# kspalaiologos/bzip3

Measured on AMD Instinct MI355X. Metric: MiB/s encode+decode round-trip, 8 MiB blocks, higher is better.
Workload: dtype u8

## Files before the change

bzip3_amd/__init__.py:

```python
import ctypes as C
import os

_HERE = os.path.dirname(os.path.abspath(__file__))
LIB_PATH = os.path.join(_HERE, "lib", "libbzip3.so")

BZ3_OK = 0
BZ3_ERR_OUT_OF_BOUNDS = -1
BZ3_ERR_BWT = -2
BZ3_ERR_CRC = -3
BZ3_ERR_MALFORMED_HEADER = -4
BZ3_ERR_TRUNCATED_DATA = -5
BZ3_ERR_DATA_TOO_BIG = -6
BZ3_ERR_INIT = -7
BZ3_ERR_DATA_SIZE_TOO_SMALL = -8

T_NAMES = ["crc", "rle", "lzp", "bwt", "cm", "copy", "_6", "_7"]

_lib = None


def _declare(L, strict=True):
    vp, i32, u32, sz = C.c_void_p, C.c_int32, C.c_uint32, C.c_size_t
    sig = {
        "bz3_version": (C.c_char_p, []),
        "bz3_last_error": (C.c_int8, [vp]),
        "bz3_strerror": (C.c_char_p, [vp]),
        "bz3_new": (vp, [i32]),
        "bz3_free": (None, [vp]),
        "bz3_bound": (sz, [sz]),
        "bz3_compress": (C.c_int, [u32, vp, vp, sz, C.POINTER(sz)]),
        "bz3_decompress": (C.c_int, [vp, vp, sz, C.POINTER(sz)]),
        "bz3_min_memory_needed": (sz, [i32]),
        "bz3_encode_block": (i32, [vp, vp, i32]),
        "bz3_decode_block": (i32, [vp, vp, sz, i32, i32]),
        "bz3_encode_blocks": (None, [vp, vp, vp, i32]),
        "bz3_decode_blocks": (None, [vp, vp, vp, vp, vp, i32]),
        "bz3_orig_size_sufficient_for_decode": (C.c_int, [vp, sz, i32]),
        "bz3_hip_device_count": (C.c_int, []),
        "bz3_hip_bind_device": (C.c_int, [C.c_int]),
        "bz3_hip_state_device": (C.c_int, [vp]),
        "bz3_hip_set_cm_mode": (C.c_int, [C.c_int]),
        "bz3_hip_cm_blocks_given_up": (C.c_uint, []),
        "bz3_hip_cm_blocks_routed_full": (C.c_uint, []),
        "bz3_hip_debug_bwt_big_rounds": (None, [C.c_int]),
        "bz3_hip_debug_set_unbwt_log_stride": (None, [C.c_int]),
        "bz3_hip_debug_peak_concurrent_groups": (C.c_int, [C.c_int]),
        "bz3_hip_debug_front_end_ring": (C.c_int, []),
        "bz3_hip_debug_arena_swap_buffers": (C.c_int, [C.c_int]),
        "bz3_hip_cm_variant_for": (C.c_int, [C.c_int, C.c_int, C.c_int]),
        "bz3_hip_set_lean_states": (C.c_int, [C.c_int]),
        "bz3_hip_release_cached_memory": (None, []),
        "bz3_hip_set_keep_workspace": (C.c_int, [C.c_int]),
        "bz3_hip_set_front_end_duo": (C.c_int, [C.c_int]),
        "bz3_hip_set_workspace_headroom": (None, [C.c_longlong]),
        "bz3_hip_workspace_headroom": (sz, []),
        "bz3_hip_debug_headroom_events": (C.c_uint, [C.c_int, C.POINTER(C.c_uint)]),
        "bz3_hip_debug_ring_contexts": (sz, [sz, sz, sz, sz, sz, sz, C.c_int, sz]),
        "bz3_hip_debug_arena_slack": (sz, [sz]),
        "bz3_hip_debug_cm_launches": (C.c_uint, [C.c_int]),
        "bz3_hip_debug_workspace_bytes": (sz, [sz, C.c_int]),
        "bz3_hip_debug_cached_bytes": (sz, [C.c_int]),
        "bz3_hip_encode_block_device": (i32, [vp, vp, i32]),
        "bz3_hip_decode_block_device": (i32, [vp, vp, sz, i32, i32]),
        "bz3_hip_encode_blocks_device": (None, [vp, vp, vp, i32]),
        "bz3_hip_decode_blocks_device": (None, [vp, vp, vp, vp, vp, i32]),
        "bz3_hip_compress_device": (C.c_int, [u32, vp, vp, sz, C.POINTER(sz)]),
        "bz3_hip_decompress_device": (C.c_int, [vp, vp, sz, C.POINTER(sz)]),
        "bz3_hip_frame_decoded_size_device": (C.c_int, [vp, sz, C.POINTER(sz)]),
        "bz3_hip_compress_device_many": (C.c_int, [u32, i32, C.POINTER(vp), C.POINTER(sz), C.POINTER(vp), C.POINTER(sz), C.POINTER(C.c_int)]),
        "bz3_hip_decompress_device_many": (C.c_int, [i32, C.POINTER(vp), C.POINTER(sz), C.POINTER(vp), C.POINTER(sz), C.POINTER(C.c_int)]),
        "bz3_hip_frame_decoded_sizes_device": (C.c_int, [i32, C.POINTER(vp), C.POINTER(sz), C.POINTER(sz), C.POINTER(C.c_int)]),
        "bz3_hip_debug_copy_segments": (i32, [vp, vp, C.POINTER(C.c_uint64), i32]),
        "bz3_hip_compress_device_planes": (C.c_int, [u32, u32, vp, vp, sz, C.POINTER(sz)]),
        "bz3_hip_decompress_device_planes": (C.c_int, [u32, vp, vp, sz, C.POINTER(sz)]),
        "bz3_hip_compress_device_planes_many": (C.c_int, [u32, i32, C.POINTER(u32), C.POINTER(vp), C.POINTER(sz), C.POINTER(vp), C.POINTER(sz), C.POINTER(C.c_int)]),
        "bz3_hip_decompress_device_planes_many": (C.c_int, [i32, C.POINTER(u32), C.POINTER(vp), C.POINTER(sz), C.POINTER(vp), C.POINTER(sz), C.POINTER(C.c_int)]),
        "bz3_hip_debug_planes": (i32, [vp, vp, C.POINTER(C.c_uint64), i32]),
        "bz3_hip_compress_device_delta": (C.c_int, [u32, u32, vp, vp, vp, sz, C.POINTER(sz)]),
        "bz3_hip_decompress_device_delta": (C.c_int, [u32, vp, vp, sz, vp, sz, C.POINTER(sz)]),
        "bz3_hip_compress_device_delta_many": (C.c_int, [u32, i32, C.POINTER(u32), C.POINTER(vp), C.POINTER(vp), C.POINTER(sz), C.POINTER(vp), C.POINTER(sz), C.POINTER(C.c_int)]),
        "bz3_hip_decompress_device_delta_many": (C.c_int, [i32, C.POINTER(u32), C.POINTER(vp), C.POINTER(sz), C.POINTER(vp), C.POINTER(sz), C.POINTER(vp), C.POINTER(sz), C.POINTER(C.c_int)]),
        "bz3_hip_crc32c_device": (C.c_int, [vp, sz, u32, C.POINTER(u32)]),
        "bz3_hip_crc32c_device_many": (C.c_int, [i32, C.POINTER(vp), C.POINTER(sz), C.POINTER(u32), C.POINTER(u32)]),
        "bz3_hip_debug_crc_launches": (C.c_uint, [C.c_int]),
        "bz3_hip_debug_delta": (i32, [vp, vp, vp, C.POINTER(C.c_uint64), i32]),
        "bz3_hip_decompress_device_range": (C.c_int, [u32, vp, sz, C.c_uint64, vp, sz, vp, C.POINTER(sz)]),
        "bz3_hip_decompress_device_range_many": (C.c_int, [i32, C.POINTER(u32), C.POINTER(vp), C.POINTER(sz), C.POINTER(C.c_uint64), C.POINTER(vp), C.POINTER(sz),
                                                           C.POINTER(vp), C.POINTER(sz), C.POINTER(C.c_int)]),
        "bz3_hip_debug_range": (i32, [vp, vp, vp, C.POINTER(C.c_uint64), i32]),
        "bz3_hip_decompress_device_strided": (C.c_int, [u32, vp, sz, C.c_uint64, C.c_uint64, C.c_uint64, C.c_uint64, vp, sz, vp, C.POINTER(sz)]),
        "bz3_hip_decompress_device_strided_many": (C.c_int, [i32, C.POINTER(u32), C.POINTER(vp), C.POINTER(sz), C.POINTER(C.c_uint64), C.POINTER(vp), C.POINTER(sz),
                                                             C.POINTER(vp), C.POINTER(sz), C.POINTER(C.c_int)]),
        "bz3_hip_debug_strided": (i32, [vp, vp, vp, C.POINTER(C.c_uint64), i32]),
        "bz3_hip_decompress_device_select": (C.c_int, [u32, vp, sz, C.c_uint64, C.c_uint64, C.c_uint64, C.c_uint64, C.POINTER(C.c_uint64), vp, sz, vp, C.POINTER(sz)]),
        "bz3_hip_decompress_device_select_many": (C.c_int, [i32, C.POINTER(u32), C.POINTER(vp), C.POINTER(sz), C.POINTER(C.c_uint64), C.POINTER(C.POINTER(C.c_uint64)),
                                                            C.POINTER(vp), C.POINTER(sz), C.POINTER(vp), C.POINTER(sz), C.POINTER(C.c_int)]),
        "bz3_hip_debug_select": (i32, [vp, vp, vp, C.POINTER(C.c_uint64), i32, C.POINTER(C.c_uint64), C.c_uint64]),
        "bz3_hip_update_device_range": (C.c_int, [u32, vp, sz, C.c_uint64, vp, sz, vp, vp, C.POINTER(sz)]),
        "bz3_hip_update_device_range_many": (C.c_int, [i32, C.POINTER(u32), C.POINTER(vp), C.POINTER(sz), C.POINTER(C.c_uint64), C.POINTER(vp), C.POINTER(sz), C.POINTER(vp),
                                                       C.POINTER(vp), C.POINTER(sz), C.POINTER(C.c_int)]),
        "bz3_hip_debug_patch": (i32, [vp, vp, vp, C.POINTER(C.c_uint64), i32]),
        "bz3_hip_last_timings": (None, [vp, C.POINTER(C.c_float)]),
        "bz3_hip_last_bwt_stats": (None, [vp, C.POINTER(i32), C.POINTER(i32), C.POINTER(C.c_uint64)]),
        "bz3_hip_stage_crc32c": (u32, [vp, sz, u32]),
        "bz3_hip_stage_mrle_encode": (i32, [vp, i32, vp]),
        "bz3_hip_stage_mrle_decode": (C.c_int, [vp, vp, i32, i32]),
        "bz3_hip_stage_lzp_encode": (i32, [vp, i32, vp]),
        "bz3_hip_stage_lzp_decode": (i32, [vp, i32, vp, i32]),
        "bz3_hip_stage_bwt": (i32, [vp, vp, i32]),
        "bz3_hip_stage_unbwt": (i32, [vp, vp, i32, i32]),
        "bz3_hip_stage_last_ms": (C.c_float, []),
        "bz3_hip_debug_sort_u32": (i32, [vp, u32, C.c_int, C.c_int, vp, vp]),
        "bz3_hip_debug_scan_u32": (i32, [vp, u32, vp]),
        "bz3_hip_debug_cu_masks": (i32, [C.c_int, C.c_int, vp, vp]),
        "bz3_hip_set_collect_window_us": (None, [C.c_int]),
        "bz3_hip_debug_collected_batches": (C.c_uint, [C.c_int, C.POINTER(C.c_uint)]),
        "bz3_hip_stage_cm_encode": (i32, [vp, i32, vp]),
        "bz3_hip_stage_cm_decode": (None, [vp, i32, vp, i32]),
        "bz3_hip_stage_cm_decode_many": (C.c_float, [vp, i32, vp, i32, i32, vp]),
        "bz3_hip_stage_cm_encode_many": (C.c_float, [vp, i32, vp, C.POINTER(i32), i32]),
        "bz3_hip_encode_stream": (C.c_int, [C.c_int, C.c_int, i32, i32]),
        "bz3_hip_decode_stream": (C.c_int, [C.c_int, C.c_int, i32]),
    }
    for name, (res, args) in sig.items():
        if not strict and not hasattr(L, name):
            continue
        fn = getattr(L, name)
        fn.restype = res
        fn.argtypes = args
    return L


EXPORTED_SYMBOLS = None


def _share_hip_runtime_with_torch():
    if os.environ.get("BZ3_HIP_SYSTEM_RUNTIME") == "1":
        return
    try:
        import importlib.util

        spec = importlib.util.find_spec("torch")
        if spec is None or not spec.origin:
            return
        cand = os.path.join(os.path.dirname(spec.origin), "lib", "libamdhip64.so")
        if os.path.exists(cand):
            C.CDLL(cand, mode=C.RTLD_GLOBAL)
    except Exception:
        pass


def load(path=None):
    global _lib
    if _lib is not None and path is None:
        return _lib
    if path is None:
        _share_hip_runtime_with_torch()
    p = path or LIB_PATH
    if not os.path.exists(p):
        raise RuntimeError(
            f"{p} is missing: the HIP extension has not been built (python -m bzip3_amd.build). "
            "bzip3_amd has no CPU or PyTorch fallback by design."
        )
    L = _declare(C.CDLL(p), strict=path is None)
    if path is None:
        _lib = L
    return L


def _cbuf(data, cap):
    cap = max(1, cap)
    if len(data) == cap:
        return (C.c_uint8 * cap).from_buffer_copy(data)
    buf = (C.c_uint8 * cap)()
    if len(data):
        C.memmove(buf, data if isinstance(data, bytes) else bytes(data), len(data))
    return buf


class StageApi:

    def __init__(self, lib=None):
        self.lib = lib or load()

    def crc32c(self, data, init=1):
        return self.lib.bz3_hip_stage_crc32c(_cbuf(data, len(data)), len(data), init)

    def mrle_encode(self, data):
        out = (C.c_uint8 * (len(data) + 64))()
        n = self.lib.bz3_hip_stage_mrle_encode(_cbuf(data, len(data)), len(data), out)
        return C.string_at(out, n)

    def mrle_decode(self, data, outlen, maxin=None):
        maxin = len(data) if maxin is None else maxin
        out = (C.c_uint8 * max(1, outlen))()
        rc = self.lib.bz3_hip_stage_mrle_decode(_cbuf(data, len(data)), out, outlen, maxin)
        return rc, C.string_at(out, outlen)

    def lzp_encode(self, data):
        out = (C.c_uint8 * (len(data) + 64))()
        n = self.lib.bz3_hip_stage_lzp_encode(_cbuf(data, len(data)), len(data), out)
        return n, (C.string_at(out, n) if n > 0 else b"")

    def lzp_decode(self, data, maxout):
        out = (C.c_uint8 * max(8, maxout))()
        n = self.lib.bz3_hip_stage_lzp_decode(_cbuf(data, len(data)), len(data), out, maxout)
        return n, (C.string_at(out, n) if n > 0 else b"")

    def bwt(self, data):
        out = (C.c_uint8 * max(1, len(data)))()
        idx = self.lib.bz3_hip_stage_bwt(_cbuf(data, len(data)), out, len(data))
        return idx, C.string_at(out, len(data))

    def unbwt(self, data, idx):
        out = (C.c_uint8 * max(1, len(data)))()
        rc = self.lib.bz3_hip_stage_unbwt(_cbuf(data, len(data)), out, len(data), idx)
        return rc, C.string_at(out, len(data))

    def cm_encode(self, data):
        out = (C.c_uint8 * (len(data) + len(data) // 50 + 64))()
        n = self.lib.bz3_hip_stage_cm_encode(_cbuf(data, len(data)), len(data), out)
        return C.string_at(out, n)

    def cm_decode(self, data, n):
        out = (C.c_uint8 * max(1, n))()
        self.lib.bz3_hip_stage_cm_decode(_cbuf(data, len(data)), len(data), out, n)
        return C.string_at(out, n)


class State:

    def __init__(self, block_size, lib=None):
        self.lib = lib or load()
        self.block_size = block_size
        self.ptr = self.lib.bz3_new(block_size)
        if not self.ptr:
            raise RuntimeError(f"bz3_new({block_size}) returned NULL (invalid size, no HIP device, or out of device memory)")

    def close(self):
        if self.ptr:
            self.lib.bz3_free(self.ptr)
            self.ptr = None

    def __del__(self):
        try:
            self.close()
        except Exception:
            pass

    def __enter__(self):
        return self

    def __exit__(self, *a):
        self.close()

    @property
    def last_error(self):
        return self.lib.bz3_last_error(self.ptr)

    def strerror(self):
        return self.lib.bz3_strerror(self.ptr).decode()

    def timings(self):
        t = (C.c_float * 8)()
        self.lib.bz3_hip_last_timings(self.ptr, t)
        return {T_NAMES[i]: t[i] for i in range(6)}

    def bwt_stats(self):
        r, p, e = C.c_int32(), C.c_int32(), C.c_uint64()
        self.lib.bz3_hip_last_bwt_stats(self.ptr, C.byref(r), C.byref(p), C.byref(e))
        return {"rounds": r.value, "radix_passes": p.value, "sorted_elements": e.value}

    def encode_block(self, data):
        cap = self.lib.bz3_bound(max(len(data), self.block_size)) + 64
        buf = _cbuf(data, cap)
        n = self.lib.bz3_encode_block(self.ptr, buf, len(data))
        return n, self.last_error, (C.string_at(buf, n) if n > 0 else b"")

    def decode_block(self, data, orig_size, buffer_size=None, comp_size=None):
        cap = self.lib.bz3_bound(self.block_size) + 64
        buffer_size = cap if buffer_size is None else buffer_size
        comp_size = len(data) if comp_size is None else comp_size
        buf = _cbuf(data, max(cap, buffer_size, len(data) + 1))
        n = self.lib.bz3_decode_block(self.ptr, buf, buffer_size, comp_size, orig_size)
        return n, self.last_error, (C.string_at(buf, n) if n > 0 else b"")


def encode_block(data, block_size, lib=None):
    with State(block_size, lib) as st:
        return st.encode_block(data)


def decode_block(data, orig_size, block_size, lib=None, **kw):
    with State(block_size, lib) as st:
        return st.decode_block(data, orig_size, **kw)


class Bz3Error(RuntimeError):

    def __init__(self, code, what, out=None, index=None, codes=None, outs=None):
        super().__init__(f"{what} failed with {code} ({_ERR_NAMES.get(code, 'unknown error')})" + ("" if index is None else f" at frame {index}"))
        self.code = code
        self.out = out
        self.index = index
        self.codes = codes
        self.outs = outs


_ERR_NAMES = {v: k for k, v in globals().items() if k.startswith("BZ3_ERR_")}


def _device_u8(x, what):
    import torch

    if not isinstance(x, torch.Tensor) or x.device.type != "cuda" or x.dtype != torch.uint8 or not x.is_contiguous():
        raise TypeError(f"{what} must be a contiguous torch.uint8 tensor on a GPU")
    return x


def _planes_arg(planes, n):
    ks = [int(planes)] * n if isinstance(planes, int) else [int(k) for k in planes]
    if len(ks) != n:
        raise ValueError(f"planes: {len(ks)} element sizes for {n} tensors")
    for k in ks:
        if k not in (1, 2, 4, 8):
            raise ValueError(f"planes must be 1, 2, 4 or 8, not {k}")
    return ks


def _base_u8(base, x, what, same_size=True):
    if base is None:
        return None
    base = _device_u8(base, what)
    if base.device != x.device:
        raise ValueError(f"{what} is on {base.device}, the tensor on {x.device}")
    if same_size and base.numel() != x.numel():
        raise ValueError(f"{what} holds {base.numel()} bytes, the tensor {x.numel()}")
    return base


def _bases_arg(bases, n):
    bases = [None] * n if bases is None else list(bases)
    if len(bases) != n:
        raise ValueError(f"bases: {len(bases)} entries for {n} tensors")
    return bases


def _ptrs_or_null(ts):
    return (C.c_void_p * len(ts))(*[None if t is None else t.data_ptr() for t in ts])


def compress_tensor(x, block_size=16 << 20, lib=None, planes=1, base=None):
    import torch

    x = _device_u8(x, "x")
    (k,) = _planes_arg(planes, 1)
    base = _base_u8(base, x, "base")
    L = lib or load()
    n = x.numel()
    out = torch.empty(L.bz3_bound(n), dtype=torch.uint8, device=x.device)
    size = C.c_size_t(out.numel())
    torch.cuda.synchronize(x.device)
    rc = L.bz3_hip_compress_device_delta(block_size, k, C.c_void_p(x.data_ptr()), None if base is None else C.c_void_p(base.data_ptr()),
                                         C.c_void_p(out.data_ptr()), n, C.byref(size))
    if rc != BZ3_OK:
        raise Bz3Error(rc, "bz3_hip_compress_device_delta")
    return out[: size.value]


def decompress_tensor(frame, out=None, lib=None, planes=1, base=None):
    import torch

    frame = _device_u8(frame, "frame")
    (k,) = _planes_arg(planes, 1)
    base = _base_u8(base, frame, "base", same_size=False)
    L = lib or load()
    torch.cuda.synchronize(frame.device)
    if out is None:
        need = C.c_size_t(0)
        L.bz3_hip_frame_decoded_size_device(C.c_void_p(frame.data_ptr()), frame.numel(), C.byref(need))
        out = torch.empty(need.value, dtype=torch.uint8, device=frame.device)
    else:
        out = _device_u8(out, "out")
    size = C.c_size_t(out.numel())
    rc = L.bz3_hip_decompress_device_delta(k, C.c_void_p(frame.data_ptr()), None if base is None else C.c_void_p(base.data_ptr()),
                                           0 if base is None else base.numel(), C.c_void_p(out.data_ptr()), frame.numel(), C.byref(size))
    if rc != BZ3_OK:
        raise Bz3Error(rc, "bz3_hip_decompress_device_delta", out[: size.value])
    return out[: size.value]


def _same_device(ts, what):
    dev = ts[0].device
    for t in ts:
        if t.device != dev:
            raise ValueError(f"{what}: all tensors must be on one GPU ({dev} and {t.device})")
    return dev


def _ptrs(ts):
    return (C.c_void_p * len(ts))(*[t.data_ptr() for t in ts])


def _carve(total, sizes, device):
    import torch

    offs, o = [], 0
    for n in sizes:
        offs.append(o)
        o += (n + 15) & ~15
    buf = torch.empty(max(o, 1), dtype=torch.uint8, device=device)
    return [buf[a : a + n] for a, n in zip(offs, sizes)]


def _compress_many(L, xs, block_sizes, ks, dev, slack=False, bases=None):
    import torch

    n = len(xs)
    bases = _bases_arg(bases, n)
    caps = [L.bz3_bound(x.numel()) + ((13 + 8 * (x.numel() // _KiB65 + 2) + 15) & ~15 if slack else 0) for x in xs]
    outs = _carve(sum(caps), caps, dev)
    frames, codes = [None] * n, [BZ3_OK] * n
    torch.cuda.synchronize(dev)
    for bs in sorted(set(block_sizes)):
        idx = [i for i in range(n) if block_sizes[i] == bs]
        g = len(idx)
        out_sizes = (C.c_size_t * g)(*[caps[i] for i in idx])
        rcs = (C.c_int * g)()
        L.bz3_hip_compress_device_delta_many(bs, g, (C.c_uint32 * g)(*[ks[i] for i in idx]), _ptrs([xs[i] for i in idx]), _ptrs_or_null([bases[i] for i in idx]),
                                             (C.c_size_t * g)(*[xs[i].numel() for i in idx]), _ptrs([outs[i] for i in idx]), out_sizes, rcs)
        for j, i in enumerate(idx):
            frames[i], codes[i] = outs[i][: out_sizes[j]], rcs[j]
    if any(c != BZ3_OK for c in codes):
        idx = next(i for i, c in enumerate(codes) if c != BZ3_OK)
        raise Bz3Error(codes[idx], "bz3_hip_compress_device_delta_many", index=idx, codes=codes, outs=frames)
    return frames


def compress_tensors(xs, block_size=16 << 20, lib=None, planes=1, bases=None):
    xs = [_device_u8(x, f"xs[{i}]") for i, x in enumerate(xs)]
    if not xs:
        return []
    ks = _planes_arg(planes, len(xs))
    bases = [_base_u8(b, x, f"bases[{i}]") for i, (b, x) in enumerate(zip(_bases_arg(bases, len(xs)), xs))]
    dev = _same_device(xs, "compress_tensors")
    return _compress_many(lib or load(), xs, [block_size] * len(xs), ks, dev, bases=bases)


def decompress_tensors(frames, outs=None, lib=None, planes=1, bases=None):
    import torch

    frames = [_device_u8(f, f"frames[{i}]") for i, f in enumerate(frames)]
    if not frames:
        return []
    ks = _planes_arg(planes, len(frames))
    bases = [_base_u8(b, f, f"bases[{i}]", same_size=False) for i, (b, f) in enumerate(zip(_bases_arg(bases, len(frames)), frames))]
    dev = _same_device(frames, "decompress_tensors")
    L = lib or load()
    n = len(frames)
    in_ptrs = _ptrs(frames)
    in_sizes = (C.c_size_t * n)(*[f.numel() for f in frames])
    torch.cuda.synchronize(dev)
    if outs is None:
        need = (C.c_size_t * n)()
        rcs = (C.c_int * n)()
        L.bz3_hip_frame_decoded_sizes_device(n, in_ptrs, in_sizes, need, rcs)
        outs = _carve(sum(need), list(need), dev)
    else:
        outs = [_device_u8(o, f"outs[{i}]") for i, o in enumerate(outs)]
        if len(outs) != n:
            raise ValueError(f"decompress_tensors: {n} frames and {len(outs)} outputs")
        _same_device(frames + outs, "decompress_tensors")
    out_sizes = (C.c_size_t * n)(*[o.numel() for o in outs])
    rcs = (C.c_int * n)()
    rc = L.bz3_hip_decompress_device_delta_many(n, (C.c_uint32 * n)(*ks), in_ptrs, in_sizes, _ptrs_or_null(bases),
                                                (C.c_size_t * n)(*[0 if b is None else b.numel() for b in bases]), _ptrs(outs), out_sizes, rcs)
    res = [o[: out_sizes[i]] for i, o in enumerate(outs)]
    if rc != BZ3_OK:
        codes = list(rcs)
        idx = next(i for i, c in enumerate(codes) if c != BZ3_OK)
        raise Bz3Error(rc, "bz3_hip_decompress_device_delta_many", index=idx, codes=codes, outs=res)
    return res


def _decompress_partial(name, frames, request, outs, planes, bases, lib):
    import torch

    frames = [_device_u8(f, f"frames[{i}]") for i, f in enumerate(frames)]
    n = len(frames)
    nbytes, entry, params = request(n)
    if not frames:
        return []
    ks = _planes_arg(planes, n)
    bases = [_base_u8(b, f, f"bases[{i}]", same_size=False) for i, (b, f) in enumerate(zip(_bases_arg(bases, n), frames))]
    dev = _same_device(frames, name)
    L = lib or load()
    if outs is None:
        outs = _carve(sum(nbytes), nbytes, dev)
    else:
        outs = [_device_u8(o, f"outs[{i}]") for i, o in enumerate(outs)]
        if len(outs) != n:
            raise ValueError(f"{name}: {n} frames and {len(outs)} outputs")
        _same_device(frames + outs, name)
    for i, (o, b, w) in enumerate(zip(outs, bases, nbytes)):
        if o.numel() < w or (b is not None and b.numel() < w):
            raise ValueError(f"{name}: outs[{i}] / bases[{i}] hold fewer than the {w} bytes asked for")
    torch.cuda.synchronize(dev)
    out_sizes = (C.c_size_t * n)(*nbytes)
    rcs = (C.c_int * n)()
    rc = getattr(L, entry)(n, (C.c_uint32 * n)(*ks), _ptrs(frames), (C.c_size_t * n)(*[f.numel() for f in frames]), *params, _ptrs_or_null(bases),
                           (C.c_size_t * n)(*[0 if b is None else w for b, w in zip(bases, nbytes)]), _ptrs(outs), out_sizes, rcs)
    res = [o[: out_sizes[i]] for i, o in enumerate(outs)]
    if rc != BZ3_OK:
        codes = list(rcs)
        idx = next(i for i, c in enumerate(codes) if c != BZ3_OK)
        raise Bz3Error(rc, entry, index=idx, codes=codes, outs=res)
    return res


def decompress_tensors_range(frames, offsets, nbytes, outs=None, planes=1, bases=None, lib=None):
    def request(n):
        offs, sizes = [int(o) for o in offsets], [int(w) for w in nbytes]
        if len(offs) != n or len(sizes) != n:
            raise ValueError(f"decompress_tensors_range: {n} frames, {len(offs)} offsets and {len(sizes)} sizes")
        if any(o < 0 for o in offs) or any(w < 0 for w in sizes):
            raise ValueError("decompress_tensors_range: offsets and sizes must not be negative")
        return sizes, "bz3_hip_decompress_device_range_many", [(C.c_uint64 * n)(*offs)]

    return _decompress_partial("decompress_tensors_range", frames, request, outs, planes, bases, lib)


def decompress_tensor_range(frame, offset, nbytes, out=None, planes=1, base=None, lib=None):
    try:
        return decompress_tensors_range([frame], [offset], [nbytes], None if out is None else [out], planes=planes, bases=None if base is None else [base], lib=lib)[0]
    except Bz3Error as e:
        raise Bz3Error(e.code, "bz3_hip_decompress_device_range", e.outs[0]) from None


def update_tensors_range(frames, offsets, datas, planes=1, bases=None, lib=None, block_sizes=None):
    import torch

    frames = [_device_u8(f, f"frames[{i}]") for i, f in enumerate(frames)]
    n = len(frames)
    offs = [int(o) for o in offsets]
    datas = [_device_u8(d, f"datas[{i}]") for i, d in enumerate(datas)]
    if len(offs) != n or len(datas) != n:
        raise ValueError(f"update_tensors_range: {n} frames, {len(offs)} offsets and {len(datas)} data tensors")
    if any(o < 0 for o in offs):
        raise ValueError("update_tensors_range: offsets must not be negative")
    if not frames:
        return []
    ks = _planes_arg(planes, n)
    bases = [_base_u8(b, d, f"bases[{i}]") for i, (b, d) in enumerate(zip(_bases_arg(bases, n), datas))]
    dev = _same_device(frames + datas, "update_tensors_range")
    L = lib or load()
    if block_sizes is None:
        heads = torch.stack([torch.nn.functional.pad(f[:13], (0, 13 - min(13, f.numel()))) for f in frames]).cpu().numpy()
        block_sizes = [int.from_bytes(bytes(h[5:9]), "little") for h in heads]
    bss = [min(max(int(b), _KiB65), _MiB511) for b in block_sizes]
    if len(bss) != n:
        raise ValueError(f"update_tensors_range: {n} frames and {len(bss)} block sizes")
    caps = [f.numel() + (d.numel() // bs + 2) * L.bz3_bound(bs) for f, d, bs in zip(frames, datas, bss)]
    outs = _carve(sum(caps), caps, dev)
    out_sizes = (C.c_size_t * n)(*caps)
    rcs = (C.c_int * n)()
    torch.cuda.synchronize(dev)
    rc = L.bz3_hip_update_device_range_many(n, (C.c_uint32 * n)(*ks), _ptrs(frames), (C.c_size_t * n)(*[f.numel() for f in frames]), (C.c_uint64 * n)(*offs), _ptrs(datas),
                                            (C.c_size_t * n)(*[d.numel() for d in datas]), _ptrs_or_null(bases), _ptrs(outs), out_sizes, rcs)
    res = [o[: out_sizes[i]] for i, o in enumerate(outs)]
    if rc != BZ3_OK:
        codes = list(rcs)
        idx = next(i for i, c in enumerate(codes) if c != BZ3_OK)
        raise Bz3Error(codes[idx], "bz3_hip_update_device_range_many", index=idx, codes=codes, outs=res)
    return res


def update_tensor_range(frame, offset, data, planes=1, base=None, lib=None, block_size=None):
    try:
        return update_tensors_range([frame], [offset], [data], planes=planes, bases=None if base is None else [base], lib=lib,
                                    block_sizes=None if block_size is None else [block_size])[0]
    except Bz3Error as e:
        raise Bz3Error(e.code, "bz3_hip_update_device_range") from None


def decompress_tensors_strided(frames, offsets, runs, strides, counts, outs=None, planes=1, bases=None, lib=None):
    def request(n):
        cols = [[int(v) for v in col] for col in (offsets, runs, strides, counts)]
        if any(len(col) != n for col in cols):
            raise ValueError(f"decompress_tensors_strided: {n} frames and {[len(col) for col in cols]} offsets, runs, strides and counts")
        params = list(zip(*cols))
        for i, (o, r, s, c) in enumerate(params):
            if min(o, r, s, c) < 0:
                raise ValueError("decompress_tensors_strided: offsets, runs, strides and counts must not be negative")
            if r and c and ((c > 1 and s < r) or c * r >= 1 << 64 or o + (c - 1) * s + r >= 1 << 64):
                raise ValueError(f"decompress_tensors_strided: ({o}, {r}, {s}, {c}) of frame {i} is no strided range")
        return [r * c for _, r, _, c in params], "bz3_hip_decompress_device_strided_many", [(C.c_uint64 * (4 * n))(*[v for p in params for v in p])]

    return _decompress_partial("decompress_tensors_strided", frames, request, outs, planes, bases, lib)


def decompress_tensor_strided(frame, offset, run, stride, count, out=None, planes=1, base=None, lib=None):
    try:
        return decompress_tensors_strided([frame], [offset], [run], [stride], [count], None if out is None else [out], planes=planes, bases=None if base is None else [base],
                                          lib=lib)[0]
    except Bz3Error as e:
        raise Bz3Error(e.code, "bz3_hip_decompress_device_strided", e.outs[0]) from None


def decompress_tensors_select(frames, offsets, strides, counts, pieces, outs=None, planes=1, bases=None, lib=None):
    def request(n):
        cols = [[int(v) for v in col] for col in (offsets, strides, counts)]
        lists = [[(int(a), int(l)) for a, l in pl] for pl in pieces]
        if any(len(col) != n for col in cols) or len(lists) != n:
            raise ValueError(f"decompress_tensors_select: {n} frames and {[len(col) for col in cols]} offsets, strides and counts, {len(lists)} piece lists")
        params = list(zip(*cols))
        nbytes = []
        for i, ((o, s, c), pl) in enumerate(zip(params, lists)):
            if min(o, s, c) < 0 or any(a < 0 or l < 0 for a, l in pl):
                raise ValueError("decompress_tensors_select: offsets, strides, counts and pieces must not be negative")
            if any(a + l >= 1 << 64 for a, l in pl) or any(a + l > b for (a, l), (b, _) in zip(pl, pl[1:])):
                raise ValueError(f"decompress_tensors_select: the pieces of frame {i} do not ascend")
            L, end = sum(l for _, l in pl), pl[-1][0] + pl[-1][1] if pl else 0
            if L and c and ((c > 1 and s < end) or c * L >= 1 << 64 or o + (c - 1) * s + end >= 1 << 64):
                raise ValueError(f"decompress_tensors_select: ({o}, {s}, {c}) and the pieces of frame {i} are no index set")
            nbytes.append(c * L)
        arrs = [(C.c_uint64 * max(1, 2 * len(pl)))(*[v for p in pl for v in p]) for pl in lists]
        ptrs = (C.POINTER(C.c_uint64) * n)(*[C.cast(a, C.POINTER(C.c_uint64)) for a in arrs])
        ptrs.arrays = arrs
        return nbytes, "bz3_hip_decompress_device_select_many", [(C.c_uint64 * (4 * n))(*[v for p, pl in zip(params, lists) for v in (*p, len(pl))]), ptrs]

    return _decompress_partial("decompress_tensors_select", frames, request, outs, planes, bases, lib)


def decompress_tensor_select(frame, offset, stride, count, pieces, out=None, planes=1, base=None, lib=None):
    try:
        return decompress_tensors_select([frame], [offset], [stride], [count], [pieces], None if out is None else [out], planes=planes, bases=None if base is None else [base],
                                         lib=lib)[0]
    except Bz3Error as e:
        raise Bz3Error(e.code, "bz3_hip_decompress_device_select", e.outs[0]) from None


DEFAULT_PLANES = {
    "float32": 4,
    "float64": 8,
    "int64": 8,
    "complex64": 4,
    "complex128": 8,
    "bfloat16": 1,
    "float16": 1,
    "int32": 1,
    "int16": 1,
    "int8": 1,
    "uint8": 1,
    "bool": 1,
}
DELTA_PLANES = {"float64": 8}
_KiB65, _MiB511 = 65 * 1024, 511 << 20


def default_planes(dtype):
    return DEFAULT_PLANES.get(str(dtype).replace("torch.", ""), 1)


def delta_default_planes(dtype):
    return DELTA_PLANES.get(str(dtype).replace("torch.", ""), 1)


def _lossless_block_size(nbytes, block_size, planes):
    if planes not in (1, 2, 4, 8):
        raise ValueError(f"planes must be 1, 2, 4 or 8, not {planes}")

    def ok(bs):
        eff = max(_KiB65, bs if bs <= nbytes else nbytes + nbytes // 50 + 32)
        return eff <= _MiB511 and (nbytes == 0 or bs > nbytes or nbytes % bs != 0)

    start = min(max(int(block_size), _KiB65), _MiB511)
    start -= start % planes
    bs = start
    if bs > nbytes > 0 and not ok(bs):
        bs = nbytes - nbytes % planes
    while bs >= _KiB65:
        if ok(bs):
            return bs
        bs -= planes
    bs = start + planes
    while not ok(bs):
        bs += planes
    return bs


class PackedTensor:

    __slots__ = ("frame", "dtype", "shape", "planes", "block_size", "nbytes", "delta", "base_crc", "crc")

    def __init__(self, frame, dtype, shape, planes, block_size, nbytes, delta=False, base_crc=None, crc=None):
        self.frame, self.dtype, self.shape, self.planes, self.block_size, self.nbytes = frame, dtype, shape, planes, block_size, nbytes
        self.delta, self.base_crc, self.crc = delta, base_crc, crc

    def __repr__(self):
        d = f", delta against a base of crc {self.base_crc:#010x}" if self.delta and self.base_crc is not None else (", delta" if self.delta else "")
        return f"PackedTensor({self.dtype}, {tuple(self.shape)}, planes={self.planes}, block_size={self.block_size}{d}, {self.frame.numel()} of {self.nbytes} bytes)"


def _as_bytes(x, what):
    import torch

    if not isinstance(x, torch.Tensor) or x.device.type != "cuda":
        raise TypeError(f"{what} must be a torch tensor on a GPU")
    x = x.detach().contiguous()
    if x.is_complex():
        x = torch.view_as_real(x)
    return x.reshape(-1).view(torch.uint8)


def _from_bytes(raw, dtype, shape):
    import torch

    if dtype.is_complex:
        return torch.view_as_complex(raw.view(torch.empty(0, dtype=dtype).real.dtype).reshape(tuple(shape) + (2,)))
    return raw.view(dtype).reshape(shape)


def _base_bytes(base, nbytes, device, what):
    if base is None:
        return None
    b = _as_bytes(base, what)
    if b.device != device:
        raise ValueError(f"{what} is on {b.device}, the tensor on {device}")
    if b.numel() != nbytes:
        raise ValueError(f"{what} holds {b.numel()} bytes, the tensor {nbytes}")
    return b


def base_crc(raw, lib=None):
    import torch

    raw = _device_u8(raw, "raw")
    torch.cuda.synchronize(raw.device)
    crc = C.c_uint32(0)
    rc = (lib or load()).bz3_hip_crc32c_device(C.c_void_p(raw.data_ptr()), raw.numel(), 1, C.byref(crc))
    if rc != BZ3_OK:
        raise Bz3Error(rc, "bz3_hip_crc32c_device")
    return crc.value


def crc32c_tensors(ts, inits=None, lib=None):
    import torch

    ts = [_device_u8(t, f"ts[{i}]") for i, t in enumerate(ts)]
    if not ts:
        return []
    n = len(ts)
    if inits is not None:
        inits = [int(v) for v in inits]
        if len(inits) != n:
            raise ValueError(f"crc32c_tensors: {len(inits)} start states for {n} tensors")
    dev = _same_device(ts, "crc32c_tensors")
    torch.cuda.synchronize(dev)
    crcs = (C.c_uint32 * n)()
    rc = (lib or load()).bz3_hip_crc32c_device_many(n, (C.c_void_p * n)(*[t.data_ptr() if t.numel() else None for t in ts]), (C.c_size_t * n)(*[t.numel() for t in ts]),
                                                    None if inits is None else (C.c_uint32 * n)(*inits), crcs)
    if rc != BZ3_OK:
        raise Bz3Error(rc, "bz3_hip_crc32c_device_many")
    return list(crcs)


def _crcs_where(ts, lib):
    idx = [i for i, t in enumerate(ts) if t is not None]
    out = [None] * len(ts)
    for i, c in zip(idx, crc32c_tensors([ts[i] for i in idx], lib=lib)):
        out[i] = c
    return out


def _pack_many(xs, block_size, planes, lib, bases=None, checksum=True):
    raws = [_as_bytes(x, f"tensor {i}") for i, x in enumerate(xs)]
    braws = [_base_bytes(b, r.numel(), r.device, f"base {i}") for i, (b, r) in enumerate(zip(_bases_arg(bases, len(xs)), raws))]
    ks = [default_planes(x.dtype) if b is None else delta_default_planes(x.dtype) for x, b in zip(xs, braws)] if planes is None else _planes_arg(planes, len(xs))
    bss = [_lossless_block_size(r.numel(), block_size, k) for r, k in zip(raws, ks)]
    if any(bs % k for bs, k in zip(bss, ks)):
        raise AssertionError("a lossless block size must be a multiple of the element size")
    dev = _same_device(raws, "pack")
    L = lib or load()
    frames = _compress_many(L, raws, bss, ks, dev, slack=True, bases=braws)
    crcs = _crcs_where(braws + (raws if checksum else []), L)
    own = crcs[len(xs) :] if checksum else [None] * len(xs)
    return [PackedTensor(f, x.dtype, x.shape, k, bs, r.numel(), b is not None, c, o) for f, x, k, bs, r, b, c, o in zip(frames, xs, ks, bss, raws, braws, crcs, own)]


def _check_bases(ps, braws, labels, lib):
    got = _crcs_where([b if b is not None and p.base_crc is not None else None for p, b in zip(ps, braws)], lib)
    for p, g, label in zip(ps, got, labels):
        if g is not None and g != p.base_crc:
            raise ValueError(f"unpack: base {label} is not the tensor this frame was packed against (its checksum differs)")


def _unpack_many(ps, outs, lib, bases=None, check_base=True, verify=False, names=None):
    import torch

    for p in ps:
        if not isinstance(p, PackedTensor):
            raise TypeError("unpack: a PackedTensor is expected")
    bases = _bases_arg(bases, len(ps))
    braws = []
    for i, (p, b) in enumerate(zip(ps, bases)):
        if p.delta and b is None:
            raise ValueError(f"unpack: tensor {i} was packed against a base, which is needed to restore it")
        if not p.delta:
            b = None
        braws.append(_base_bytes(b, p.nbytes, p.frame.device, f"base {i}"))
    L = lib or load()
    if check_base:
        _check_bases(ps, braws, range(len(ps)), L)
    if outs is None:
        dev = _same_device([p.frame for p in ps], "unpack")
        raws = _carve(0, [p.nbytes for p in ps], dev)
        res = None
    else:
        res = outs
        raws = []
        for p, o in zip(ps, outs):
            if not isinstance(o, torch.Tensor) or o.dtype != p.dtype or o.shape != p.shape or not o.is_contiguous():
                raise TypeError("unpack: `out` must be a contiguous tensor of the packed dtype and shape")
            raws.append(_as_bytes(o, "out"))
    got = decompress_tensors([p.frame for p in ps], raws, lib=lib, planes=[p.planes for p in ps], bases=braws)
    for p, g in zip(ps, got):
        if g.numel() != p.nbytes:
            raise ValueError(f"unpack: the frame decodes to {g.numel()} bytes, the tensor has {p.nbytes}")
    if verify:
        got = _crcs_where([r if p.crc is not None else None for p, r in zip(ps, raws)], L)
        for i, (p, g) in enumerate(zip(ps, got)):
            if g is not None and g != p.crc:
                raise ValueError(f"unpack: the decoded bytes of tensor {i if names is None else repr(names[i])} do not have the checksum recorded when it was packed")
    return res if res is not None else [_from_bytes(r, p.dtype, p.shape) for r, p in zip(raws, ps)]


def pack_tensor(x, block_size=16 << 20, planes=None, lib=None, base=None, checksum=True):
    return _pack_many([x], block_size, None if planes is None else [planes], lib, [base], checksum)[0]


def unpack_tensor(p, out=None, lib=None, base=None, check_base=True, verify=False):
    return _unpack_many([p], None if out is None else [out], lib, [base], check_base, verify)[0]


def _row_bytes(p, what):
    if not isinstance(p, PackedTensor):
        raise TypeError("unpack: a PackedTensor is expected")
    if len(p.shape) == 0:
        raise ValueError(f"{what}: a 0-d tensor has no rows")
    return p.nbytes // p.shape[0] if p.shape[0] else 0


def _unpack_rows_many(ps, rows, outs, lib, bases):
    shapes, spans = [], []
    for i, (p, r) in enumerate(zip(ps, rows)):
        if not isinstance(p, PackedTensor):
            raise TypeError("unpack: a PackedTensor is expected")
        if r is None:
            shapes.append(tuple(p.shape))
            spans.append((0, p.nbytes))
            continue
        rb = _row_bytes(p, f"tensor {i}")
        start, stop = int(r[0]), int(r[1])
        if not 0 <= start <= stop <= p.shape[0]:
            raise ValueError(f"rows ({start}, {stop}) of a tensor of {p.shape[0]} rows")
        shapes.append((stop - start, *p.shape[1:]))
        spans.append((start * rb, (stop - start) * rb))
    frames, planes, sizes = [p.frame for p in ps], [p.planes for p in ps], [w for _, w in spans]
    return _unpack_parts_many(ps, shapes, sizes, [], outs, lib, bases, "rows",
                              lambda raws, braws: decompress_tensors_range(frames, [o for o, _ in spans], sizes, raws, planes=planes, bases=braws, lib=lib))



def unpack_tensor_rows(p, start, stop, out=None, base=None, lib=None):
    return _unpack_rows_many([p], [(start, stop)], None if out is None else [out], lib, [base])[0]


def _update_rows_many(ps, rows, bases, lib):
    import torch

    offs, raws, braws = [], [], []
    for i, (p, (start, values), b) in enumerate(zip(ps, rows, _bases_arg(bases, len(ps)))):
        rb = _row_bytes(p, f"tensor {i}")
        start = int(start)
        if not isinstance(values, torch.Tensor) or values.device.type != "cuda":
            raise TypeError(f"update: the rows of tensor {i} must be a torch tensor on a GPU")
        if values.dtype != p.dtype or values.dim() != len(p.shape) or tuple(values.shape[1:]) != tuple(p.shape[1:]):
            raise TypeError(f"update: the rows of tensor {i} must be {p.dtype} of shape (rows, {', '.join(map(str, p.shape[1:]))})")
        if not 0 <= start <= start + values.shape[0] <= p.shape[0]:
            raise ValueError(f"update: rows ({start}, {start + values.shape[0]}) of a tensor of {p.shape[0]} rows")
        if p.delta and b is None:
            raise ValueError(f"update: tensor {i} was packed against a base, whose rows are needed to code the new ones")
        if not p.delta:
            b = None
        elif not isinstance(b, torch.Tensor) or b.dtype != p.dtype or tuple(b.shape) != tuple(values.shape):
            raise ValueError(f"update: base {i} must hold the same rows of the base: {p.dtype} {tuple(values.shape)}")
        raw = _as_bytes(values, f"rows {i}")
        offs.append(start * rb)
        raws.append(raw)
        braws.append(_base_bytes(b, raw.numel(), p.frame.device, f"base {i}"))
    frames = update_tensors_range([p.frame for p in ps], offs, raws, planes=[p.planes for p in ps], bases=braws, lib=lib, block_sizes=[p.block_size for p in ps])
    return [PackedTensor(f, p.dtype, p.shape, p.planes, p.block_size, p.nbytes, p.delta, p.base_crc, None) for f, p in zip(frames, ps)]


def update_tensor_rows(p, start, values, base=None, lib=None):
    return _update_rows_many([p], [(start, values)], [base], lib)[0]


def _slice_of(p, sl, what):
    if not isinstance(p, PackedTensor):
        raise TypeError("unpack: a PackedTensor is expected")
    shape = tuple(p.shape)
    if sl is None:
        return shape, (0, p.nbytes, p.nbytes, 1)
    dim, start, stop = (int(v) for v in sl)
    if not shape:
        raise ValueError(f"{what}: a 0-d tensor has no dimension to slice")
    if not -len(shape) <= dim < len(shape):
        raise ValueError(f"{what}: dimension {dim} of a tensor of {len(shape)} dimensions")
    dim %= len(shape)
    if not 0 <= start <= stop <= shape[dim]:
        raise ValueError(f"{what}: ({start}, {stop}) of a dimension of {shape[dim]}")
    numel, inner, count = 1, 1, 1
    for d, v in enumerate(shape):
        numel *= v
        if d > dim:
            inner *= v
        if d < dim:
            count *= v
    inner *= p.nbytes // numel if numel else 0
    return shape[:dim] + (stop - start,) + shape[dim + 1 :], (start * inner, (stop - start) * inner, shape[dim] * inner, count)


def _unpack_parts_many(ps, shapes, sizes, whole, outs, lib, bases, what, decode):
    import torch

    bases = _bases_arg(bases, len(ps))
    braws = []
    for i, (p, b, w, shape) in enumerate(zip(ps, bases, sizes, shapes)):
        if p.delta and b is None:
            raise ValueError(f"unpack: tensor {i} was packed against a base, which is needed to restore it")
        if not p.delta:
            b = None
        elif not isinstance(b, torch.Tensor) or b.dtype != p.dtype or tuple(b.shape) != shape:
            raise ValueError(f"unpack: base {i} must hold the same {what} of the base: {p.dtype} {shape}")
        braws.append(_base_bytes(b, w, p.frame.device, f"base {i}"))
    dev = _same_device([p.frame for p in ps], "unpack")
    if outs is None:
        raws = _carve(0, sizes, dev)
    else:
        raws = []
        for p, o, shape in zip(ps, outs, shapes):
            if not isinstance(o, torch.Tensor) or o.dtype != p.dtype or tuple(o.shape) != shape or not o.is_contiguous():
                raise TypeError(f"unpack: `out` must be a contiguous tensor of the packed dtype and of the {what}'{'' if what.endswith('s') else 's'} shape")
            raws.append(_as_bytes(o, "out"))
    got = decode(raws, braws)
    for i, (g, w) in enumerate(zip(got, sizes)):
        if g.numel() != w:
            raise Bz3Error(BZ3_ERR_TRUNCATED_DATA, f"unpack: the frame of tensor {i} holds {g.numel()} of the {w} bytes of its {what};", g)
    if whole:
        n = len(whole)
        need, rcs = (C.c_size_t * n)(), (C.c_int * n)()
        (lib or load()).bz3_hip_frame_decoded_sizes_device(n, _ptrs([ps[i].frame for i in whole]), (C.c_size_t * n)(*[ps[i].frame.numel() for i in whole]), need, rcs)
        for i, d in zip(whole, need):
            if d != ps[i].nbytes:
                raise Bz3Error(BZ3_ERR_DATA_TOO_BIG if d > ps[i].nbytes else BZ3_ERR_TRUNCATED_DATA, f"unpack: the frame of tensor {i} decodes to {d} bytes, the tensor has {ps[i].nbytes};")
    return list(outs) if outs is not None else [_from_bytes(r, p.dtype, shape) for r, p, shape in zip(raws, ps, shapes)]


def _unpack_slices_many(ps, slices, outs, lib, bases):
    shapes, params = [], []
    for i, (p, sl) in enumerate(zip(ps, slices)):
        shape, q = _slice_of(p, sl, f"tensor {i}")
        shapes.append(shape)
        params.append(q)
    frames, planes = [p.frame for p in ps], [p.planes for p in ps]
    return _unpack_parts_many(ps, shapes, [q[1] * q[3] for q in params], [i for i, sl in enumerate(slices) if sl is None], outs, lib, bases, "slice",
                              lambda raws, braws: decompress_tensors_strided(frames, *zip(*params), raws, planes=planes, bases=braws, lib=lib))


def unpack_tensor_slice(p, dim, start, stop, out=None, base=None, lib=None):
    return _unpack_slices_many([p], [(dim, start, stop)], None if out is None else [out], lib, [base])[0]


def _index_list(index, what):
    if hasattr(index, "detach") and hasattr(index, "cpu"):
        if index.dim() != 1 or index.is_floating_point() or index.is_complex() or str(index.dtype) == "torch.bool":
            raise ValueError(f"{what}: the index must be a 1-D integer tensor")
        return [int(v) for v in index.detach().cpu().tolist()]
    if hasattr(index, "ndim") and hasattr(index, "tolist"):
        if index.ndim != 1 or index.dtype.kind not in "iu":
            raise ValueError(f"{what}: the index must be a 1-D integer array")
        return [int(v) for v in index.tolist()]
    out = []
    for v in index:
        if isinstance(v, bool) or int(v) != v:
            raise ValueError(f"{what}: the index must hold integers")
        out.append(int(v))
    return out


def _index_of(p, sel, what):
    if sel is None or len(sel) == 3:
        shape, (o, r, s, c) = _slice_of(p, sel, what)
        return shape, (o, s, c, [(0, r)]), None
    shape, (_, _, stride, count) = _slice_of(p, (sel[0], 0, 0), what)
    dim = int(sel[0]) % len(p.shape)
    size = p.shape[dim]
    inner = stride // size if size else 0
    idx = _index_list(sel[1], what)
    if any(not 0 <= i < size for i in idx):
        raise ValueError(f"{what}: index out of range for a dimension of {size}")
    if any(a >= b for a, b in zip(idx, idx[1:])):
        raise ValueError(f"{what}: the index must be strictly increasing here")
    pieces = []
    for i in idx:
        if pieces and pieces[-1][0] + pieces[-1][1] == i * inner:
            pieces[-1] = (pieces[-1][0], pieces[-1][1] + inner)
        else:
            pieces.append((i * inner, inner))
    return tuple(p.shape[:dim]) + (len(idx),) + tuple(p.shape[dim + 1 :]), (0, stride, count if idx else 0, pieces), idx


def _unpack_index_many(ps, sels, outs, lib, bases):
    shapes, reqs = [], []
    for i, (p, sel) in enumerate(zip(ps, sels)):
        shape, q, _ = _index_of(p, sel, f"tensor {i}")
        shapes.append(shape)
        reqs.append(q)
    frames, planes = [p.frame for p in ps], [p.planes for p in ps]
    return _unpack_parts_many(ps, shapes, [q[2] * sum(l for _, l in q[3]) for q in reqs], [i for i, sel in enumerate(sels) if sel is None], outs, lib, bases, "part",
                              lambda raws, braws: decompress_tensors_select(frames, *zip(*reqs), raws, planes=planes, bases=braws, lib=lib))


def _sorted_unique(index, what):
    idx = _index_list(index, what)
    if all(a < b for a, b in zip(idx, idx[1:])):
        return idx, idx, None
    uniq = sorted(set(idx))
    where = {v: j for j, v in enumerate(uniq)}
    return idx, uniq, [where[v] for v in idx]


def unpack_tensor_index(p, dim, index, out=None, base=None, lib=None):
    import torch

    idx, uniq, where = _sorted_unique(index, "unpack_tensor_index")
    if where is None:
        return _unpack_index_many([p], [(dim, idx)], None if out is None else [out], lib, [base])[0]
    if isinstance(p, PackedTensor) and p.delta:
        raise ValueError("unpack_tensor_index: a tensor packed against a base takes a strictly increasing index (its base is given in the index's order)")
    part = _unpack_index_many([p], [(dim, uniq)], None, lib, [None])[0]
    d = int(dim) % len(p.shape)
    shape = tuple(p.shape[:d]) + (len(idx),) + tuple(p.shape[d + 1 :])
    if out is not None and (not isinstance(out, torch.Tensor) or out.dtype != p.dtype or tuple(out.shape) != shape or not out.is_contiguous()):
        raise TypeError("unpack: `out` must be a contiguous tensor of the packed dtype and of the result's shape")
    order = torch.tensor(where, dtype=torch.int64, device=part.device)
    if out is None:
        return torch.index_select(part, d, order)
    torch.index_select(part, d, order, out=out)
    return out


def pack_state_dict(sd, block_size=16 << 20, planes=None, lib=None, base=None, checksum=True):
    names = list(sd)
    if isinstance(planes, dict):
        planes = [planes[k] for k in names]
    if not names:
        return {}
    bases = None
    if base is not None:
        bases = [base.get(k) for k in names]
        bases = [b if b is not None and getattr(b, "dtype", None) == sd[k].dtype and getattr(b, "shape", None) == sd[k].shape else None for k, b in zip(names, bases)]
    return dict(zip(names, _pack_many([sd[k] for k in names], block_size, planes, lib, bases, checksum)))


def unpack_state_dict(packed, lib=None, base=None, inplace=False, check_base=True, rows=None, verify=False, slices=None, index=None):
    names = list(packed)
    if index is not None or slices is not None or rows is not None:
        arg, part = ("index", "a part of") if index is not None else ("slices", "a slice of") if slices is not None else ("rows", "rows for")
        if verify:
            raise ValueError(f"unpack_state_dict: verify=True and {arg} do not go together (the checksum covers the whole tensor)")
        if inplace:
            raise ValueError(f"unpack_state_dict: {arg} and inplace=True do not go together")
        want = {k: (0, int(r[0]), int(r[1])) for k, r in (rows or {}).items()}
        for k, sl in (slices or {}).items():
            if k in want:
                raise ValueError(f"unpack_state_dict: {k!r} is in both rows and slices")
            want[k] = tuple(sl)
        order = {}
        for k, (dim, idx) in (index or {}).items():
            if k in want:
                raise ValueError(f"unpack_state_dict: {k!r} is in index and in rows or slices")
            if k in packed:
                _, uniq, order[k] = _sorted_unique(idx, repr(k))
                want[k] = (dim, uniq)
            else:
                want[k] = (dim, idx)
        unknown = [k for k in want if k not in packed]
        if unknown:
            raise ValueError(f"unpack_state_dict: {part} {unknown[0]!r}, which is not in the dict")
        if not names:
            return {}
        import torch

        ps = [packed[k] for k in names]
        sels = [want.get(k) for k in names]
        for k, p, sel in zip(names, ps, sels):
            if arg != "rows":
                _index_of(p, sel, repr(k))
            if order.get(k) is not None and p.delta:
                raise ValueError(f"unpack_state_dict: {k!r} was packed against a base and takes a strictly increasing index")
        bases, whole = [], []
        L = lib or load()
        for k, p, sel in zip(names, ps, sels):
            b = base.get(k) if base is not None and p.delta else None
            fits = isinstance(b, torch.Tensor) and b.dtype == p.dtype and tuple(b.shape) == tuple(p.shape)
            whole.append(_base_bytes(b, p.nbytes, p.frame.device, f"base {k!r}") if check_base and fits and p.base_crc is not None else None)
            if fits and sel is not None and len(sel) == 3:
                if arg != "rows" or (len(p.shape) and 0 <= sel[1] <= sel[2] <= p.shape[0]):
                    b = b.narrow(int(sel[0]) % len(p.shape), int(sel[1]), int(sel[2]) - int(sel[1]))
            elif fits and sel is not None:
                b = b.index_select(int(sel[0]) % len(p.shape), torch.tensor(sel[1], dtype=torch.int64, device=b.device))
            bases.append(b)
        _check_bases(ps, whole, [repr(k) for k in names], L)
        if arg == "index":
            parts = _unpack_index_many(ps, sels, None, lib, bases)
        elif arg == "slices":
            parts = _unpack_slices_many(ps, sels, None, lib, bases)
        else:
            parts = _unpack_rows_many(ps, [None if sel is None else sel[1:] for sel in sels], None, lib, bases)
        got = dict(zip(names, parts))
        for k, where in order.items():
            if where is not None:
                got[k] = torch.index_select(got[k], int(index[k][0]) % len(packed[k].shape), torch.tensor(where, dtype=torch.int64, device=got[k].device))
        return got
    if not names:
        return {}
    ps = [packed[k] for k in names]
    bases = [base.get(k) if base is not None and p.delta else None for k, p in zip(names, ps)]
    if not inplace or not any(p.delta for p in ps):
        return dict(zip(names, _unpack_many(ps, None, lib, bases, check_base, verify, names)))
    import torch

    fresh = _carve(0, [0 if p.delta else p.nbytes for p in ps], _same_device([p.frame for p in ps], "unpack"))
    outs = []
    for k, p, b, f in zip(names, ps, bases, fresh):
        if not p.delta:
            outs.append(_from_bytes(f, p.dtype, p.shape))
        elif not isinstance(b, torch.Tensor) or b.dtype != p.dtype or b.shape != p.shape:
            raise ValueError(f"unpack: {k} was packed against a base of {p.dtype} {tuple(p.shape)}, which is needed to restore it")
        else:
            outs.append(b)
    return dict(zip(names, _unpack_many(ps, outs, lib, bases, check_base, verify, names)))


def update_state_dict_rows(packed, rows, base=None, lib=None):
    unknown = [k for k in rows if k not in packed]
    if unknown:
        raise ValueError(f"update_state_dict_rows: rows for {unknown[0]!r}, which is not in the dict")
    names = list(rows)
    out = dict(packed)
    if names:
        out.update(zip(names, _update_rows_many([packed[k] for k in names], [rows[k] for k in names], [None if base is None else base.get(k) for k in names], lib)))
    return out


def check_chain(steps):
    unchecked = []
    for t, step in enumerate(steps):
        for name, p in step.items():
            if not isinstance(p, PackedTensor):
                raise TypeError(f"check_chain: step {t}: {name!r} is not a PackedTensor")
            if not p.delta:
                continue
            if t == 0:
                raise ValueError(f"check_chain: step 0: {name!r} is a delta tensor, and there is no step before it")
            q = steps[t - 1].get(name)
            if q is None:
                raise ValueError(f"check_chain: step {t}: {name!r} is a delta tensor, and step {t - 1} does not hold that name")
            if q.dtype != p.dtype or tuple(q.shape) != tuple(p.shape) or q.nbytes != p.nbytes:
                raise ValueError(f"check_chain: step {t}: {name!r} is {p.dtype} {tuple(p.shape)} of {p.nbytes} bytes, in step {t - 1} it is {q.dtype} {tuple(q.shape)} of {q.nbytes}")
            if p.base_crc is None or q.crc is None:
                unchecked.append((t - 1, name))
            elif p.base_crc != q.crc:
                raise ValueError(f"check_chain: step {t}: {name!r} was packed against a base of checksum {p.base_crc:#010x}, in step {t - 1} it has {q.crc:#010x}")
    return unchecked


def unpack_chain(steps, verify=True, lib=None):
    steps = list(steps)
    if not steps:
        raise ValueError("unpack_chain: no steps")
    check_chain(steps)
    last = len(steps) - 1
    current = unpack_state_dict(steps[0], lib=lib, verify=verify and last == 0)
    for t in range(1, len(steps)):
        current = unpack_state_dict(steps[t], lib=lib, base=current, inplace=True, check_base=False, verify=verify and t == last)
    return current


PACKED_MAGIC = b"BZ3TNSR1"
_ENTRY_KEYS = ("dtype", "shape", "planes", "block_size", "nbytes", "delta", "base_crc", "crc", "offset", "size")


def _opt_int(v):
    return None if v is None else int(v)


def save_packed(path, packed, metadata=None):
    import json

    import torch

    names = list(packed)
    entries, offs, o = {}, [], 0
    for k in names:
        p = packed[k]
        if not isinstance(k, str) or not isinstance(p, PackedTensor):
            raise TypeError("save_packed: a dict of str -> PackedTensor is expected")
        if not isinstance(p.frame, torch.Tensor) or p.frame.dtype != torch.uint8 or p.frame.dim() != 1:
            raise TypeError(f"save_packed: the frame of {k!r} must be a one-dimensional torch.uint8 tensor")
        size = p.frame.numel()
        entries[k] = {"dtype": str(p.dtype).replace("torch.", ""), "shape": [int(d) for d in p.shape], "planes": int(p.planes), "block_size": int(p.block_size),
                      "nbytes": int(p.nbytes), "delta": bool(p.delta), "base_crc": _opt_int(p.base_crc), "crc": _opt_int(p.crc), "offset": o, "size": size}
        offs.append(o)
        o += (size + 15) & ~15
    head = json.dumps({"version": 1, "metadata": {} if metadata is None else metadata, "tensors": entries}, ensure_ascii=False).encode("utf-8")
    head += b" " * ((0 - (16 + len(head))) % 64)
    host = {}
    for dev in {packed[k].frame.device for k in names}:
        mine = [k for k in names if packed[k].frame.device == dev]
        if dev.type == "cpu":
            host.update({k: packed[k].frame.contiguous() for k in mine})
        else:
            parts = torch.cat([packed[k].frame for k in mine]).cpu().split([packed[k].frame.numel() for k in mine])
            host.update(dict(zip(mine, parts)))
    tmp = path + ".tmp"
    try:
        with open(tmp, "wb") as f:
            f.write(PACKED_MAGIC + len(head).to_bytes(8, "little") + head)
            at = 0
            for k, off in zip(names, offs):
                f.write(b"\0" * (off - at))
                f.write(memoryview(host[k].numpy()))
                at = off + host[k].numel()
        os.replace(tmp, path)
    except BaseException:
        if os.path.exists(tmp):
            os.remove(tmp)
        raise


def _read_packed_header(f, path):
    import json
    import math

    import torch

    size = os.fstat(f.fileno()).st_size
    fixed = f.read(16)
    if len(fixed) < 16 or fixed[:8] != PACKED_MAGIC:
        raise ValueError(f"{path}: not a packed tensor file (it does not start with {PACKED_MAGIC!r})")
    hlen = int.from_bytes(fixed[8:], "little")
    if 16 + hlen > size:
        raise ValueError(f"{path}: the header of {hlen} bytes runs past the end of the file")
    try:
        head = json.loads(f.read(hlen).decode("utf-8"))
    except ValueError as e:
        raise ValueError(f"{path}: the header is not JSON: {e}") from None
    if not isinstance(head, dict) or head.get("version") != 1:
        raise ValueError(f"{path}: version {head.get('version') if isinstance(head, dict) else None!r} of the format, this code reads version 1")
    entries, metadata = head.get("tensors"), head.get("metadata", {})
    if not isinstance(entries, dict):
        raise ValueError(f"{path}: the header holds no tensors")
    for k, e in entries.items():
        if not isinstance(e, dict) or any(key not in e for key in _ENTRY_KEYS):
            raise ValueError(f"{path}: the entry of {k!r} is incomplete")
        dtype = getattr(torch, e["dtype"], None) if isinstance(e["dtype"], str) else None
        if not isinstance(dtype, torch.dtype):
            raise ValueError(f"{path}: {k!r} has the unknown dtype {e['dtype']!r}")
        if e["planes"] not in (1, 2, 4, 8):
            raise ValueError(f"{path}: {k!r} has planes = {e['planes']!r}, which must be 1, 2, 4 or 8")
        if not isinstance(e["shape"], list) or any(not isinstance(d, int) or d < 0 for d in e["shape"]):
            raise ValueError(f"{path}: {k!r} has the shape {e['shape']!r}")
        if e["nbytes"] != math.prod(e["shape"]) * torch.empty(0, dtype=dtype).element_size():
            raise ValueError(f"{path}: {k!r} has nbytes = {e['nbytes']!r}, which is not what {e['dtype']} {e['shape']} holds")
        if any(not isinstance(e[key], int) or isinstance(e[key], bool) or e[key] < 0 for key in ("offset", "size", "block_size")):
            raise ValueError(f"{path}: {k!r} has a bad offset, size or block size")
    return entries, metadata, 16 + hlen, size


def packed_index(path):
    with open(path, "rb") as f:
        entries, metadata, _, _ = _read_packed_header(f, path)
    return entries, metadata


def load_packed(path, device, names=None):
    import torch

    with open(path, "rb") as f:
        entries, _, data_at, size = _read_packed_header(f, path)
        names = list(entries) if names is None else list(names)
        for k in names:
            if k not in entries:
                raise KeyError(k)
            if data_at + entries[k]["offset"] + entries[k]["size"] > size:
                raise ValueError(f"{path}: the frame of {k!r} runs past the end of the file")
        offs, o = [], 0
        for k in names:
            offs.append(o)
            o += (entries[k]["size"] + 15) & ~15
        host = torch.zeros(max(o, 1), dtype=torch.uint8)
        view = memoryview(host.numpy())
        for k, a in zip(names, offs):
            f.seek(data_at + entries[k]["offset"])
            if f.readinto(view[a : a + entries[k]["size"]]) != entries[k]["size"]:
                raise ValueError(f"{path}: the frame of {k!r} could not be read whole")
    buf = host.to(device)
    out = {}
    for k, a in zip(names, offs):
        e = entries[k]
        out[k] = PackedTensor(buf[a : a + e["size"]], getattr(torch, e["dtype"]), torch.Size(e["shape"]), e["planes"], e["block_size"], e["nbytes"], bool(e["delta"]),
                              e["base_crc"], e["crc"])
    return out


def shard_blocks(n_blocks, world_size, rank):
    return [k for k in range(n_blocks) if k % world_size == rank]
```

bzip3_amd/csrc/api_decode.hip:

```cpp
#include "api_internal.hpp"

using namespace bz3;
using namespace bz3::api;

namespace {

__global__ void __launch_bounds__(128) k_unstore_small(u8 * __restrict__ b, u32 n) {
    const u32 t = threadIdx.x;
    const u8 v = t < n ? b[8 + t] : (u8)0;
    __syncthreads();
    if (t < n) b[t] = v;
}

void decode_front(bz3_state * st, u8 * buf, size_t buffer_size, s32 compressed_size, s32 orig_size, const u8 * hdr) {
    st->pending = bz3_state::FAILED;
    st->result = -1;
    if (st->skip) return;
    if (buffer_size < 9 || buffer_size < (size_t)compressed_size) {
        st->last_error = BZ3_ERR_DATA_SIZE_TOO_SMALL;
        return;
    }
    const u32 crc = rd_le32(hdr);
    const s32 bwt_idx = (s32)rd_le32(hdr + 4);
    const size_t bound = bz3_bound((size_t)st->block_size);
    if (compressed_size < 0 || (size_t)compressed_size > bound) {
        st->last_error = BZ3_ERR_MALFORMED_HEADER;
        return;
    }
    hipStream_t s = st->xs;
    for (float & x : st->t) x = 0.f;
    st->user = buf;
    st->buffer_size = buffer_size;
    st->crc = crc;
    if (bwt_idx == -1) {
        if (compressed_size - 8 > 64 || compressed_size < 8) {
            st->last_error = BZ3_ERR_MALFORMED_HEADER;
            return;
        }
        if ((size_t)(compressed_size - 8) > buffer_size) {
            st->last_error = BZ3_ERR_DATA_SIZE_TOO_SMALL;
            return;
        }
        st->size = compressed_size - 8;
        launch(k_unstore_small, dim3(1), dim3(128), 0, s, buf, (u32)st->size);
        crc32c_device(buf, (u64)st->size, 1u, st->ctx->d_crc, st->d_words, s);
        st->pending = bz3_state::DEC_STORED;
        return;
    }
    const s32 model = (s8)hdr[8];
    const size_t need = 9 + (size_t)((model & 2) * 4) + (size_t)((model & 4) * 4);
    if (buffer_size < need) {
        st->last_error = BZ3_ERR_DATA_SIZE_TOO_SMALL;
        return;
    }
    s32 lzp_size = -1, rle_size = -1, p = 0;
    if (model & 2) lzp_size = (s32)rd_le32(hdr + 9 + 4 * p++);
    if (model & 4) rle_size = (s32)rd_le32(hdr + 9 + 4 * p++);
    p += 2;
    compressed_size -= p * 4 + 1;
    if (((model & 2) && (lzp_size < 0 || (size_t)lzp_size > bound)) || ((model & 4) && (rle_size < 0 || (size_t)rle_size > bound))) {
        st->last_error = BZ3_ERR_MALFORMED_HEADER;
        return;
    }
    if (orig_size < 0 || (size_t)orig_size > bound) {
        st->last_error = BZ3_ERR_MALFORMED_HEADER;
        return;
    }
    const s32 size_before_bwt = (model & 2) ? lzp_size : (model & 4) ? rle_size : orig_size;
    if (!sizes_fit(buffer_size, lzp_size, rle_size, orig_size)) {
        st->last_error = BZ3_ERR_DATA_SIZE_TOO_SMALL;
        return;
    }
    st->bwt_idx = bwt_idx;
    st->model = model;
    st->lzp_size = lzp_size;
    st->rle_size = rle_size;
    st->orig_size = orig_size;
    st->size_before_bwt = size_before_bwt;
    st->cm_in = buf + p * 4 + 1;
    st->cm_in_size = (u32)(compressed_size < 0 ? 0 : compressed_size);
    st->pending = bz3_state::DEC_CODED;
}

bool decode_unbwt(bz3_state * st, Arena & arena, float cm_ms, u32 lanes) {
    hipStream_t s = st->xs;
    st->t[BZ3_HIP_T_CM] = cm_ms;
    const s32 n = st->size_before_bwt;
    if (st->bwt_idx > n) {
        st->last_error = BZ3_ERR_MALFORMED_HEADER;
        return false;
    }
    u8 *b1 = st->d_swap, *b2 = st->user;
    if (st->lean) {
        b1 = st->user;
        b2 = st->d_swap;
    }
    const double t0 = now_ms();
    if (n <= 1) {
        if (st->bwt_idx != n) { st->last_error = BZ3_ERR_BWT; return false; }
        if (n == 1) HIP_CHECK(hipMemcpyAsync(b2, b1, 1, hipMemcpyDeviceToDevice, s));
    } else {
        if (st->bwt_idx <= 0) { st->last_error = BZ3_ERR_BWT; return false; }
        bwt_inverse(b1, (u32)n, (u32)st->bwt_idx, b2, arena, s, lanes);
        HIP_CHECK(hipStreamSynchronize(s));
    }
    st->b1 = b2;
    st->b2 = b1;
    st->size_src = n;
    st->t[BZ3_HIP_T_BWT] = (float)(now_ms() - t0);
    return true;
}

void decode_finish(bz3_state * st, Arena & arena) {
    hipStream_t s = st->xs;
    const size_t bound = bz3_bound((size_t)st->block_size);
    (void)bound;
    u8 *b1 = st->b1, *b2 = st->b2;
    s32 size_src = st->size_src;
    if (st->model & 2) {
        size_src = (s32)read_word(s, st->d_words + 5);
        if (size_src == -1) { st->last_error = BZ3_ERR_CRC; return; }
        if ((size_t)size_src > st->buffer_size) { st->last_error = BZ3_ERR_DATA_SIZE_TOO_SMALL; return; }
        u8 * tmp = b1; b1 = b2; b2 = tmp;
    }
    if (st->model & 4) {
        const double t0 = now_ms();
        bool bad = size_src < 32;
        if (!bad) {
            mrle_decode(b1, (u32)size_src, b2, (u32)st->orig_size, st->d_words + 4, arena, s);
            bad = read_word(s, st->d_words + 4) != (u32)st->orig_size;
        }
        st->t[BZ3_HIP_T_RLE] = (float)(now_ms() - t0);
        if (bad) { st->last_error = BZ3_ERR_CRC; return; }
        size_src = st->orig_size;
        u8 * tmp = b1; b1 = b2; b2 = tmp;
    }
    st->last_error = BZ3_OK;
    if (size_src > st->block_size || size_src < 0) {
        st->last_error = BZ3_ERR_MALFORMED_HEADER;
        return;
    }
    if (b1 != st->user) {
        const double t0 = now_ms();
        HIP_CHECK(hipMemcpyAsync(st->user, b1, (size_t)size_src, hipMemcpyDeviceToDevice, s));
        HIP_CHECK(hipStreamSynchronize(s));
        st->t[BZ3_HIP_T_COPY] += (float)(now_ms() - t0);
    }
    const double t0 = now_ms();
    crc32c_device(st->user, (u64)size_src, 1u, st->ctx->d_crc, st->d_words, s);
    const u32 got = read_word(s, st->d_words + 1);
    st->t[BZ3_HIP_T_CRC] = (float)(now_ms() - t0);
    if (got != st->crc) {
        st->last_error = BZ3_ERR_CRC;
        return;
    }
    st->result = size_src;
}

}

namespace bz3 {
namespace api {

void decode_group(bz3_state ** sts, u8 ** bufs, const size_t * buffer_sizes, const s32 * sizes, const s32 * orig_sizes, const u8 * hdrs, s32 n) {
    if (n <= 0) return;
    bz3_state * lead = sts[0];
    DeviceGuard g(lead->device);
    std::lock_guard<std::mutex> lk(lead->ctx->mu);
    hipStream_t s = lead->stream;
    for (s32 i = 0; i < n; i++) sts[i]->xs = s;
    size_t need = 0;
    bool any_lean = false;
    for (s32 i = 0; i < n; i++) {
        const size_t w = workspace_bytes_for(bz3_bound((size_t)sts[i]->block_size) + 64);
        if (w > need) need = w;
        any_lean = any_lean || sts[i]->lean;
    }
    std::vector<s32> coded;
    for (s32 i = 0; i < n; i++) {
        decode_front(sts[i], bufs[i], buffer_sizes[i], sizes[i], orig_sizes[i], hdrs + 17 * (size_t)i);
        if (sts[i]->pending == bz3_state::DEC_CODED) coded.push_back(i);
    }
    auto stage_bytes = [&](s32 i) { return sts[i]->lean ? (((size_t)sts[i]->cm_in_size + 64 + 255) & ~(size_t)255) : (size_t)0; };
    size_t stage_budget = (size_t)48 << 30;
    {
        size_t free_b = 0, total_b = 0;
        if (any_lean && hipMemGetInfo(&free_b, &total_b) == hipSuccess) {
            const size_t have = lead->ctx->ws_cap;
            const size_t aside = need + ws_headroom() + ((size_t)577 << 20);
            const size_t room = free_b + have > aside ? free_b + have - aside : 0;
            stage_budget = room - room / 4;
        }
    }
    std::vector<size_t> round_end;
    size_t max_round = 0;
    for (size_t k = 0; k < coded.size();) {
        size_t bytes = 0, e = k;
        while (e < coded.size() && (e == k || bytes + stage_bytes(coded[e]) <= stage_budget)) bytes += stage_bytes(coded[e++]);
        round_end.push_back(e);
        if (bytes > max_round) max_round = bytes;
        k = e;
    }
    s32 tail_slots = n >= 128 ? 4 : 2;
    s32 tail_window = tail_slots == 4 ? 16 : 32;
    if (tail_slots == 4) {
        size_t cap_max = 0;
        for (s32 i = 0; i < n; i++)
            if (sts[i]->lean && sts[i]->cap > cap_max) cap_max = sts[i]->cap;
        const size_t cap_al = (cap_max + 255) & ~(size_t)255;
        size_t free_b = 0, total_b = 0;
        const bool have_info = hipMemGetInfo(&free_b, &total_b) == hipSuccess;
        for (s32 w : {30, 25, 20}) {
            if (n < 4 * w || lead->ctx->reserved_cus_wanted() < 64) continue;
            const size_t bufs = (size_t)4 * (size_t)w;
            const bool from_arena = keep_workspace() && any_lean && lead->ctx->ws_cap >= need + need / 16 + bufs * cap_al + ((size_t)64 << 20);
            if (!any_lean || from_arena || (have_info && free_b >= bufs * cap_max + ws_headroom() + ((size_t)2 << 30) + max_round)) {
                tail_window = w;
                break;
            }
        }
    }
    lead->ctx->ensure_aux();
    if (const char * e = getenv("BZ3_HIP_TAIL_PIPE")) {
        int w = 0, q = 0;
        if (sscanf(e, "%d,%d", &w, &q) == 2 && w >= 1 && q >= 2 && q <= DeviceCtx::AUX) {
            tail_window = w;
            tail_slots = q;
        }
    }
    if (tail_window > n) tail_window = n;
    size_t lzp_in_window = 0;
    for (s32 w0 = 0; w0 < n; w0 += tail_window) {
        size_t c = 0;
        for (s32 i = w0; i < n && i < w0 + tail_window; i++)
            if (sts[i]->pending == bz3_state::DEC_CODED && (sts[i]->model & 2)) c++;
        if (c > lzp_in_window) lzp_in_window = c;
    }
    Arena arena = lead->ctx->arena_for(need + (size_t)tail_slots * lzp_in_window * (LZP_LUT_WORDS * 4 + sizeof(LzpDecodeJob) + 256) + (size_t)n * 256 + cm_scratch_bytes(coded.size()) + max_round + 65536);
    float cm_ms = 0.f;
    for (size_t r = 0, k0 = 0; r < round_end.size(); k0 = round_end[r++]) {
        const size_t mk = arena.mark();
        std::vector<CmDecodeJob> cm_jobs;
        std::vector<char> to_full;
        for (size_t k = k0; k < round_end[r]; k++) {
            bz3_state * st = sts[coded[k]];
            to_full.push_back((u64)st->cm_in_size * 10u >= (u64)(u32)st->size_before_bwt * 9u ? 1 : 0);
            const u8 * in = st->cm_in;
            if (st->lean) {
                u8 * stage = arena.take<u8>(stage_bytes(coded[k]));
                if (st->cm_in_size) HIP_CHECK(hipMemcpyAsync(stage, st->cm_in, st->cm_in_size, hipMemcpyDeviceToDevice, s));
                in = stage;
            }
            cm_jobs.push_back(CmDecodeJob{dev_addr(in), dev_addr(st->lean ? st->user : st->d_swap), st->cm_in_size, (u32)st->size_before_bwt, 0u, 0u});
        }
        CmDecodeJob * d_jobs = arena.take<CmDecodeJob>(cm_jobs.size());
        cm_ms += run_cm_jobs(lead->ctx, arena, cm_jobs, d_jobs, s, lead->ev0, lead->ev1,
                             [](const CmDecodeJob * j, u32 nj, hipStream_t st, int variant) { cm_decode_batch(j, nj, st, variant); }, &to_full);
        arena.release(mk);
    }
    struct TailWindow {
        s32 w0 = 0, w1 = 0;
        std::vector<LzpDecodeJob> lz_jobs;
        std::vector<s32> lz_owner;
        std::vector<char> alive;
        LzpDecodeJob * d_lz = nullptr;
        u32 * luts = nullptr;
    } tw[DeviceCtx::AUX];
    for (int k = 0; k < tail_slots; k++) {
        tw[k].d_lz = lzp_in_window ? arena.take<LzpDecodeJob>(lzp_in_window) : nullptr;
        tw[k].luts = lzp_in_window ? arena.take<u32>(lzp_in_window * LZP_LUT_WORDS) : nullptr;
    }
    std::vector<u8 *> arena_swaps;
    size_t swap_cap = 0;
    if (keep_workspace() && any_lean) {
        for (s32 i = 0; i < n; i++)
            if (sts[i]->lean && sts[i]->cap > swap_cap) swap_cap = sts[i]->cap;
        const size_t want = (size_t)tail_slots * (size_t)tail_window;
        const size_t step = (swap_cap + 255) & ~(size_t)255;
        const size_t keep_free = need + need / 32 + 65536;
        while (swap_cap && arena_swaps.size() < want && arena.cap - arena.used >= keep_free + step) arena_swaps.push_back(arena.take<u8>(swap_cap));
    }
    std::vector<char> from_arena((size_t)n, 0);
    auto borrow = [&](s32 i) {
        bz3_state * st = sts[i];
        if (st->lean && !st->d_swap && !arena_swaps.empty() && st->cap <= swap_cap) {
            st->d_swap = arena_swaps.back();
            arena_swaps.pop_back();
            from_arena[(size_t)i] = 1;
            g_arena_swaps.fetch_add(1);
        } else {
            lean_borrow(st);
        }
    };
    auto give_back = [&](s32 i) {
        bz3_state * st = sts[i];
        if (from_arena[(size_t)i]) {
            if (st->d_swap) arena_swaps.push_back(st->d_swap);
            st->d_swap = nullptr;
            from_arena[(size_t)i] = 0;
        } else {
            lean_return(st);
        }
    };
    lead->ctx->ensure_aux();
    DrainOnUnwind drain{s, lead->ctx->aux, DeviceCtx::AUX};
    hipStream_t s_cm = s;
    hipStream_t * side_streams = lead->ctx->aux;
    static const s32 part_min = [] { const char * e = getenv("BZ3_HIP_CU_PARTITION_MIN_BLOCKS"); return e && atoi(e) > 0 ? (s32)atoi(e) : (s32)128; }();
    if (lead->ctx->rest && n >= part_min && tail_slots <= DeviceCtx::RING_SLOTS) {
        side_streams = lead->ctx->aux_m;
        HIP_CHECK(hipStreamSynchronize(s));
        s = lead->ctx->rest;
        for (s32 i = 0; i < n; i++) sts[i]->xs = s;
    }
    const u32 unbwt_lanes = s != s_cm && lead->ctx->real_cus > lead->ctx->reserved_cus ? (u32)(lead->ctx->real_cus - lead->ctx->reserved_cus) * UNBWT_LANES_PER_CU : 0u;
    DrainOnUnwind drain_rest{s == s_cm ? nullptr : s, side_streams == lead->ctx->aux ? nullptr : side_streams, side_streams == lead->ctx->aux ? 0 : DeviceCtx::AUX};
    const s32 nwin = (n + tail_window - 1) / tail_window;
    const s32 lag = tail_slots - 1;
    static const bool trace_rings = getenv("BZ3_HIP_TRACE_RINGS") != nullptr;
    double tr_unbwt = 0, tr_wait = 0, tr_finish = 0, tr_t0 = now_ms();
    for (s32 k = 0; k < nwin + lag; k++) {
        const double tr_a = now_ms();
        if (k < nwin) {
            const int q = (int)(k % tail_slots);
            hipStream_t s2 = side_streams[q];
            TailWindow & w = tw[q];
            w.w0 = k * tail_window;
            w.w1 = (w.w0 + tail_window < n) ? w.w0 + tail_window : n;
            w.lz_jobs.clear();
            w.lz_owner.clear();
            w.alive.assign((size_t)(w.w1 - w.w0), 0);
            for (s32 i = w.w0; i < w.w1; i++) {
                bz3_state * st = sts[i];
                if (st->pending == bz3_state::DEC_STORED) {
                    HIP_CHECK(hipStreamSynchronize(st->xs));
                    if (read_word(st->xs, st->d_words + 1) != st->crc) st->last_error = BZ3_ERR_CRC;
                    else st->result = st->size;
                    continue;
                }
                if (st->pending != bz3_state::DEC_CODED) continue;
                borrow(i);
                if (!decode_unbwt(st, arena, cm_ms, unbwt_lanes)) continue;
                w.alive[(size_t)(i - w.w0)] = 1;
                if (st->model & 2) {
                    if (st->lzp_size < 4) {
                        st->last_error = BZ3_ERR_CRC;
                        w.alive[(size_t)(i - w.w0)] = 0;
                        continue;
                    }
                    const size_t bound = bz3_bound((size_t)st->block_size);
                    const size_t room = st->lean && st->buffer_size < bound ? st->buffer_size : bound;
                    w.lz_jobs.push_back(LzpDecodeJob{dev_addr(st->b1), dev_addr(st->b2), dev_addr(w.luts + w.lz_jobs.size() * LZP_LUT_WORDS), dev_addr(st->d_words + 5),
                                                     (u32)st->lzp_size, (u32)room});
                    w.lz_owner.push_back(i);
                }
            }
            if (!w.lz_jobs.empty()) {
                HIP_CHECK(hipEventRecord(lead->ctx->ev_prep, s));
                HIP_CHECK(hipStreamWaitEvent(s2, lead->ctx->ev_prep, 0));
                HIP_CHECK(hipEventRecord(lead->ctx->ev_d0[q], s2));
                lzp_decode_batch(w.lz_jobs.data(), w.d_lz, (u32)w.lz_jobs.size(), s2);
                HIP_CHECK(hipEventRecord(lead->ctx->ev_d1[q], s2));
            }
        }
        const double tr_b = now_ms();
        tr_unbwt += tr_b - tr_a;
        if (k >= lag) {
            const int q = (int)((k - lag) % tail_slots);
            TailWindow & w = tw[q];
            if (!w.lz_jobs.empty()) {
                HIP_CHECK(hipEventSynchronize(lead->ctx->ev_d1[q]));
                tr_wait += now_ms() - tr_b;
                float ms = 0.f;
                (void)hipEventElapsedTime(&ms, lead->ctx->ev_d0[q], lead->ctx->ev_d1[q]);
                for (s32 i : w.lz_owner) sts[i]->t[BZ3_HIP_T_LZP] = ms;
                for (size_t j = 0; j < w.lz_jobs.size(); j++) {
                    bz3_state * st = sts[w.lz_owner[j]];
                    const size_t bound = bz3_bound((size_t)st->block_size);
                    if (!st->lean || st->buffer_size >= bound || read_word(s, st->d_words + 5) != w.lz_jobs[j].max_out) continue;
                    u8 * big = st->ctx->temp_get(st->cap);
                    LzpDecodeJob again = w.lz_jobs[j];
                    again.out = dev_addr(big);
                    again.max_out = (u32)bound;
                    again.lut = dev_addr(w.luts);
                    lzp_decode_batch(&again, w.d_lz, 1u, s);
                    HIP_CHECK(hipStreamSynchronize(s));
                    st->ctx->temp_put(big);
                }
            }
            for (s32 i = w.w0; i < w.w1; i++) {
                if (w.alive[(size_t)(i - w.w0)]) decode_finish(sts[i], arena);
                give_back(i);
            }
        }
        tr_finish += now_ms() - tr_b;
    }
    if (trace_rings)
        fprintf(stderr, "[bz3 rings] decode tail: %d blocks, %d windows of %d x %d slots: %.1f ms = inverse BWTs + LZP launches %.1f + waiting for a window's LZP decoders %.1f + mRLE / CRC / hand-back %.1f\n",
                (int)n, (int)nwin, (int)tail_window, (int)tail_slots, now_ms() - tr_t0, tr_unbwt, tr_wait, tr_finish - tr_wait);
    for (s32 i = 0; i < n; i++) sts[i]->pending = bz3_state::NONE;
    if (s != s_cm) (void)hipStreamSynchronize(s);
    enforce_headroom(lead->ctx, s_cm);
}

}
}
```

bzip3_amd/csrc/api_hooks.hip:

```cpp
#include "api_internal.hpp"

using namespace bz3;
using namespace bz3::api;

namespace {

struct StageEnv {
    DeviceCtx * ctx = nullptr;
    hipStream_t s = nullptr;
    std::vector<void *> allocs;
    std::unique_lock<std::mutex> lock;
    StageEnv() {
        int dev = pick_device();
        if (dev < 0) {
            fprintf(stderr, "bzip3_amd: no HIP device available -- this library has no CPU code path\n");
            abort();
        }
        ctx = get_ctx(dev);
        HIP_CHECK(hipSetDevice(dev));
        HIP_CHECK(hipStreamCreateWithFlags(&s, hipStreamNonBlocking));
        lock = std::unique_lock<std::mutex>(ctx->mu);
    }
    ~StageEnv() {
        (void)hipStreamSynchronize(s);
        for (void * p : allocs) (void)hipFree(p);
        (void)hipStreamDestroy(s);
    }
    u8 * dev(size_t bytes, const void * init = nullptr, size_t init_bytes = 0) {
        void * p = nullptr;
        HIP_CHECK(hipMalloc(&p, bytes + 4096));
        allocs.push_back(p);
        if (init && init_bytes) HIP_CHECK(hipMemcpy(p, init, init_bytes, hipMemcpyHostToDevice));
        return (u8 *)p;
    }
    void down(void * host, const void * d, size_t bytes) {
        HIP_CHECK(hipStreamSynchronize(s));
        if (bytes) HIP_CHECK(hipMemcpy(host, d, bytes, hipMemcpyDeviceToHost));
    }
    u32 word(const u32 * d) {
        u32 v = 0;
        down(&v, d, 4);
        return v;
    }
};

template <typename F>
auto stage_guard(F && f) -> decltype(f()) {
    try {
        return f();
    } catch (const HipError & e) {
        fprintf(stderr, "bzip3_amd: HIP failure '%s' at %s:%d\n", e.what, e.file, e.line);
        abort();
    }
}

}

extern "C" {

BZIP3_API uint32_t bz3_hip_stage_crc32c(const uint8_t * data, size_t n, uint32_t init) {
    return stage_guard([&]() -> u32 {
        StageEnv e;
        u8 * d = e.dev(n + 16, data, n);
        u32 * w = (u32 *)e.dev(64);
        crc32c_device(d, n, init, e.ctx->d_crc, w, e.s);
        return e.word(w + 1);
    });
}

BZIP3_API int32_t bz3_hip_stage_mrle_encode(const uint8_t * in, int32_t n, uint8_t * out) {
    return stage_guard([&]() -> s32 {
        StageEnv e;
        u8 * d = e.dev((size_t)n + 16, in, (size_t)n);
        u8 * o = e.dev((size_t)n + 64);
        Arena a = e.ctx->arena_for(workspace_bytes_for((u64)n + 64));
        MrleEncScratch sc;
        mrle_encode_size(d, (u32)n, sc, a, e.s);
        const s32 size = (s32)(32u + e.word(sc.total));
        mrle_encode_write(d, (u32)n, sc, o, e.s);
        e.down(out, o, (size_t)size);
        return size;
    });
}

BZIP3_API int bz3_hip_stage_mrle_decode(const uint8_t * in, uint8_t * out, int32_t outlen, int32_t maxin) {
    return stage_guard([&]() -> int {
        if (maxin < 32) return 1;
        StageEnv e;
        u8 * d = e.dev((size_t)maxin + 16, in, (size_t)maxin);
        u8 * o = e.dev((size_t)outlen + 64);
        u32 * w = (u32 *)e.dev(64);
        Arena a = e.ctx->arena_for(workspace_bytes_for((u64)maxin + 64));
        mrle_decode(d, (u32)maxin, o, (u32)outlen, w, a, e.s);
        const u32 got = e.word(w);
        e.down(out, o, (size_t)(got < (u32)outlen ? got : (u32)outlen));
        return got != (u32)outlen;
    });
}

BZIP3_API int32_t bz3_hip_stage_lzp_encode(const uint8_t * in, int32_t n, uint8_t * out) {
    return stage_guard([&]() -> s32 {
        StageEnv e;
        u8 * d = e.dev((size_t)n + 64, in, (size_t)n);
        u8 * o = e.dev((size_t)n + 64);
        Arena a = e.ctx->arena_for(workspace_bytes_for((u64)n + 64));
        const s32 r = lzp_encode(d, (u32)n, o, a, e.s);
        if (r > 0) e.down(out, o, (size_t)r);
        return r;
    });
}

BZIP3_API int32_t bz3_hip_stage_lzp_decode(const uint8_t * in, int32_t n, uint8_t * out, int32_t max) {
    return stage_guard([&]() -> s32 {
        StageEnv e;
        u8 * d = e.dev((size_t)n + 64, in, (size_t)n);
        u8 * o = e.dev((size_t)max + 64);
        Arena a = e.ctx->arena_for(workspace_bytes_for((u64)n + 64));
        if (n < 4) return -1;
        u32 * d_result = a.take<u32>(4);
        LzpDecodeJob job{dev_addr(d), dev_addr(o), dev_addr(a.take<u32>(LZP_LUT_WORDS)), dev_addr(d_result), (u32)n, (u32)max};
        LzpDecodeJob * d_job = a.take<LzpDecodeJob>(1);
        lzp_decode_batch(&job, d_job, 1, e.s);
        const s32 r = (s32)e.word(d_result);
        if (r > 0) e.down(out, o, (size_t)r);
        return r;
    });
}

static std::atomic<float> g_stage_ms{0.f};
BZIP3_API float bz3_hip_stage_last_ms(void) { return g_stage_ms.load(); }

BZIP3_API int32_t bz3_hip_stage_bwt(const uint8_t * in, uint8_t * out, int32_t n) {
    return stage_guard([&]() -> s32 {
        StageEnv e;
        u8 * d = e.dev((size_t)n + 64, in, (size_t)n);
        u8 * o = e.dev((size_t)n + 64);
        Arena a = e.ctx->arena_for(workspace_bytes_for((u64)n + 64));
        HIP_CHECK(hipStreamSynchronize(e.s));
        const auto t0 = std::chrono::steady_clock::now();
        const s32 idx = bwt_forward(d, (u32)n, o, a, e.s, nullptr);
        g_stage_ms.store(std::chrono::duration<float, std::milli>(std::chrono::steady_clock::now() - t0).count());
        e.down(out, o, (size_t)n);
        return idx;
    });
}

BZIP3_API int32_t bz3_hip_stage_unbwt(const uint8_t * in, uint8_t * out, int32_t n, int32_t idx) {
    return stage_guard([&]() -> s32 {
        if (n < 0) return -1;
        if (n <= 1) {
            if (idx != n) return -1;
            if (n == 1) out[0] = in[0];
            return 0;
        }
        if (idx <= 0 || idx > n) return -1;
        StageEnv e;
        u8 * d = e.dev((size_t)n + 64, in, (size_t)n);
        u8 * o = e.dev((size_t)n + 64);
        Arena a = e.ctx->arena_for(workspace_bytes_for((u64)n + 64));
        HIP_CHECK(hipStreamSynchronize(e.s));
        const auto t0 = std::chrono::steady_clock::now();
        bwt_inverse(d, (u32)n, (u32)idx, o, a, e.s);
        HIP_CHECK(hipStreamSynchronize(e.s));
        g_stage_ms.store(std::chrono::duration<float, std::milli>(std::chrono::steady_clock::now() - t0).count());
        e.down(out, o, (size_t)n);
        return 0;
    });
}

BZIP3_API int32_t bz3_hip_debug_cu_masks(int cus, int reserve, uint32_t * side, uint32_t * rest) {
    if (cus < 32 || cus > 1024 || reserve < 8 || !side || !rest) return -1;
    std::vector<uint32_t> a, b;
    DeviceCtx::cu_masks(cus, reserve, a, b);
    for (size_t k = 0; k < a.size(); k++) {
        side[k] = a[k];
        rest[k] = b[k];
    }
    return (int32_t)a.size();
}

BZIP3_API int32_t bz3_hip_debug_scan_u32(uint32_t * data, uint32_t n, uint32_t * total) {
    return stage_guard([&]() -> s32 {
        if (n == 0) return -1;
        StageEnv e;
        u32 * d = (u32 *)e.dev((size_t)n * 4 + 64, data, (size_t)n * 4);
        u32 * t = (u32 *)e.dev(64);
        Arena a = e.ctx->arena_for(scan_temp_words(n) * 4 + (1u << 20));
        exclusive_scan_u32(d, n, t, a, e.s);
        e.down(data, d, (size_t)n * 4);
        if (total) *total = e.word(t);
        return 0;
    });
}

BZIP3_API int32_t bz3_hip_debug_sort_u32(const uint32_t * keys, uint32_t n, int key_bits, int digit_bits, uint32_t * sorted_keys, uint32_t * sorted_index) {
    return stage_guard([&]() -> s32 {
        if ((digit_bits != 8 && digit_bits != 9) || key_bits < 1 || key_bits > 32 || n == 0) return -1;
        StageEnv e;
        u32 * k[2] = {(u32 *)e.dev((size_t)n * 4 + 64, keys, (size_t)n * 4), (u32 *)e.dev((size_t)n * 4 + 64)};
        u32 * v[2] = {(u32 *)e.dev((size_t)n * 4 + 64), (u32 *)e.dev((size_t)n * 4 + 64)};
        Arena a = e.ctx->arena_for(radix_temp_bytes(n, digit_bits) + (1u << 20));
        int cur = 0, passes = 0;
        for (int shift = 0; shift < key_bits; shift += digit_bits, passes++) {
            const u32 * vin = passes ? v[cur] : nullptr;
            if (digit_bits == 9) radix_pass_bits<u32, 9>(k[cur], k[cur ^ 1], vin, v[cur ^ 1], n, shift, 0xFFFFFFFFu, 0u, a, e.s);
            else radix_pass<u32>(k[cur], k[cur ^ 1], vin, v[cur ^ 1], n, shift, 0xFFFFFFFFu, 0u, a, e.s);
            cur ^= 1;
        }
        e.down(sorted_keys, k[cur], (size_t)n * 4);
        e.down(sorted_index, v[cur], (size_t)n * 4);
        return passes;
    });
}

extern "C++" template <class Job, class Launch>
void stage_cm_job(StageEnv & e, Job job, Launch && go) {
    const int variant = cm_variant_for(e.ctx, 1, std::is_same<Job, CmEncodeJob>::value);
    u32 * status = nullptr;
    if (cm_variant_has_rows(variant)) {
        job.spill = dev_addr(e.dev(CM_SPILL_BYTES));
        status = (u32 *)e.dev(64);
        HIP_CHECK(hipMemsetAsync(status, 0, 64, e.s));
        job.status = dev_addr(status);
        job.miss_base = cm_variant_is_test(variant) ? 64u : CM_MISS_BASE;
        job.miss_shift = cm_variant_is_test(variant) ? 3u : CM_MISS_SHIFT;
    }
    Job * d_job = (Job *)e.dev(sizeof job, &job, sizeof job);
    go(d_job, 1u, e.s, variant);
    if (cm_variant_has_rows(variant) && e.word(status) != 0u) {
        g_cm_given_up.fetch_add(1u);
        go(d_job, 1u, e.s, (int)CM_VARIANT_FULL);
    }
}

BZIP3_API int32_t bz3_hip_stage_cm_encode(const uint8_t * in, int32_t n, uint8_t * out) {
    return stage_guard([&]() -> s32 {
        StageEnv e;
        u8 * d = e.dev((size_t)n + 64, in, (size_t)n);
        u8 * o = e.dev(bz3_bound((size_t)n) + 64);
        u32 * w = (u32 *)e.dev(64);
        const char * dbg = getenv("BZ3_CM_DEBUG");
        CmEncodeJob job{dev_addr(d), dev_addr(o), dev_addr(w), (u32)n, dbg ? (u32)atoi(dbg) : 0u};
        const char * tg = getenv("BZ3_CM_TEST_GAP");
        u8 * side = nullptr;
        if (tg) {
            const size_t g = (size_t)atol(tg);
            const char * ts = getenv("BZ3_CM_TEST_SIDE");
            const size_t side_cap = ts ? (size_t)atol(ts) : CM_SIDE_BYTES;
            u8 * both = e.dev(g + (size_t)n + 64);
            HIP_CHECK(hipMemcpy(both + g, d, (size_t)n, hipMemcpyDeviceToDevice));
            side = e.dev(side_cap + 64);
            o = both;
            job.in = dev_addr(both + g);
            job.out = dev_addr(both);
            job.gap = (u32)g;
            job.side = dev_addr(side);
            job.side_cap = (u32)side_cap;
        }
        stage_cm_job(e, job, [](const CmEncodeJob * j, u32 nj, hipStream_t st, int variant) { cm_encode_batch(j, nj, st, variant); });
        const u32 coded = e.word(w), sw = e.word(w + 1);
        if (coded == 0xFFFFFFFFu) return -1;
        const u32 head = (tg && sw < coded) ? sw : coded;
        e.down(out, o, (size_t)head);
        if (head < coded) e.down(out + head, side, (size_t)(coded - head));
        return (s32)coded;
    });
}

BZIP3_API void bz3_hip_stage_cm_decode(const uint8_t * in, int32_t in_size, uint8_t * out, int32_t n) {
    stage_guard([&]() -> int {
        StageEnv e;
        u8 * d = e.dev((size_t)in_size + 64, in, (size_t)in_size);
        u8 * o = e.dev((size_t)n + 64);
        const char * dbg = getenv("BZ3_CM_DEBUG");
        CmDecodeJob job{dev_addr(d), dev_addr(o), (u32)in_size, (u32)n, dbg ? (u32)atoi(dbg) : 0u, 0u};
        stage_cm_job(e, job, [](const CmDecodeJob * j, u32 nj, hipStream_t st, int variant) { cm_decode_batch(j, nj, st, variant); });
        e.down(out, o, (size_t)n);
        return 0;
    });
}

BZIP3_API float bz3_hip_stage_cm_decode_many(const uint8_t * in, int32_t in_size, uint8_t * out, int32_t n, int32_t copies, uint64_t * counters) {
    return stage_guard([&]() -> float {
        StageEnv e;
        if (copies < 1 || n < 256) return -1.f;
        u8 * d = e.dev((size_t)in_size + 64, in, (size_t)in_size);
        const size_t stride = ((size_t)n + 64 + 255) & ~(size_t)255;
        u8 * o = e.dev(stride * (size_t)copies);
        const char * dbg = getenv("BZ3_CM_DEBUG");
        const u32 debug = dbg ? (u32)atoi(dbg) : 0u;
        const int variant = cm_variant_for(e.ctx, (size_t)copies, false);
        u8 * spill = cm_variant_has_rows(variant) ? e.dev(CM_SPILL_BYTES * (size_t)copies) : nullptr;
        u32 * status = (u32 *)e.dev(4 * (size_t)copies + 64);
        HIP_CHECK(hipMemsetAsync(status, 0, 4 * (size_t)copies, e.s));
        std::vector<CmDecodeJob> jobs;
        for (int32_t k = 0; k < copies; k++) {
            CmDecodeJob j{dev_addr(d), dev_addr(o + stride * (size_t)k), (u32)in_size, (u32)n, debug, 0u};
            if (spill) {
                j.spill = dev_addr(spill + CM_SPILL_BYTES * (size_t)k);
                j.status = dev_addr(status + k);
                j.miss_base = CM_MISS_BASE;
                j.miss_shift = CM_MISS_SHIFT;
            }
            jobs.push_back(j);
        }
        CmDecodeJob * d_jobs = (CmDecodeJob *)e.dev(sizeof(CmDecodeJob) * jobs.size(), jobs.data(), sizeof(CmDecodeJob) * jobs.size());
        hipEvent_t e0, e1;
        HIP_CHECK(hipEventCreate(&e0));
        HIP_CHECK(hipEventCreate(&e1));
        HIP_CHECK(hipEventRecord(e0, e.s));
        cm_decode_batch(d_jobs, (u32)copies, e.s, variant, (debug & 15u) == 3u);
        HIP_CHECK(hipEventRecord(e1, e.s));
        HIP_CHECK(hipStreamSynchronize(e.s));
        float ms = 0.f;
        (void)hipEventElapsedTime(&ms, e0, e1);
        (void)hipEventDestroy(e0);
        (void)hipEventDestroy(e1);
        e.down(out, o, (size_t)n);
        if (counters)
            for (int32_t k = 0; k < copies; k++) e.down(counters + 16 * (size_t)k, o + stride * (size_t)k, 128);
        if (getenv("BZ3_CM_MANY_CHECK")) {
            std::vector<u8> other((size_t)n);
            for (int32_t k = 1; k < copies; k++) {
                e.down(other.data(), o + stride * (size_t)k, (size_t)n);
                if (memcmp(other.data(), out, (size_t)n) != 0) return -2.f;
            }
        }
        return ms;
    });
}

BZIP3_API float bz3_hip_stage_cm_encode_many(const uint8_t * in, int32_t n, uint8_t * out, int32_t * coded, int32_t copies) {
    return stage_guard([&]() -> float {
        StageEnv e;
        if (copies < 1 || n < 1) return -1.f;
        u8 * d = e.dev((size_t)n + 64, in, (size_t)n);
        const size_t stride = (bz3_bound((size_t)n) + 64 + 255) & ~(size_t)255;
        u8 * o = e.dev(stride * (size_t)copies);
        u32 * w = (u32 *)e.dev(16 * (size_t)copies + 64);
        const char * dbg = getenv("BZ3_CM_DEBUG");
        const u32 debug = dbg ? (u32)atoi(dbg) : 0u;
        const int variant = cm_variant_for(e.ctx, (size_t)copies, true);
        u8 * spill = cm_variant_has_rows(variant) ? e.dev(CM_SPILL_BYTES * (size_t)copies) : nullptr;
        u32 * status = (u32 *)e.dev(4 * (size_t)copies + 64);
        HIP_CHECK(hipMemsetAsync(status, 0, 4 * (size_t)copies, e.s));
        u32 * claim = getenv("BZ3_CM_NO_CLAIM") ? nullptr : (u32 *)e.dev(CM_CLAIM_WORDS * 4);
        if (claim) HIP_CHECK(hipMemsetAsync(claim, 0, CM_CLAIM_WORDS * 4, e.s));
        std::vector<CmEncodeJob> jobs;
        for (int32_t k = 0; k < copies; k++) {
            CmEncodeJob j{dev_addr(d), dev_addr(o + stride * (size_t)k), dev_addr(w + 4 * (size_t)k), (u32)n, debug};
            j.claim = claim ? dev_addr(claim) : 0;
            if (spill) {
                j.spill = dev_addr(spill + CM_SPILL_BYTES * (size_t)k);
                j.status = dev_addr(status + k);
                j.miss_base = CM_MISS_BASE;
                j.miss_shift = CM_MISS_SHIFT;
            }
            jobs.push_back(j);
        }
        CmEncodeJob * d_jobs = (CmEncodeJob *)e.dev(sizeof(CmEncodeJob) * jobs.size(), jobs.data(), sizeof(CmEncodeJob) * jobs.size());
        hipEvent_t e0, e1;
        HIP_CHECK(hipEventCreate(&e0));
        HIP_CHECK(hipEventCreate(&e1));
        HIP_CHECK(hipEventRecord(e0, e.s));
        cm_encode_batch(d_jobs, (u32)copies, e.s, variant);
        HIP_CHECK(hipEventRecord(e1, e.s));
        HIP_CHECK(hipStreamSynchronize(e.s));
        float ms = 0.f;
        (void)hipEventElapsedTime(&ms, e0, e1);
        (void)hipEventDestroy(e0);
        (void)hipEventDestroy(e1);
        const u32 got = e.word(w);
        if (coded) *coded = (int32_t)got;
        if (got != 0xFFFFFFFFu && got <= bz3_bound((size_t)n) && !(debug & 15u)) {
            e.down(out, o, (size_t)got);
            if (getenv("BZ3_CM_MANY_CHECK")) {
                std::vector<u8> other((size_t)got);
                for (int32_t k = 1; k < copies; k++) {
                    if (e.word(w + 4 * (size_t)k) != got) return -2.f;
                    e.down(other.data(), o + stride * (size_t)k, (size_t)got);
                    if (memcmp(other.data(), out, (size_t)got) != 0) return -2.f;
                }
            }
        }
        return ms;
    });
}

}
```

bzip3_amd/csrc/sort.hip:

```cpp
#include "prims.hpp"
#include "sort.hpp"

namespace bz3 {

constexpr int SC_BLOCK = 256;
constexpr int SC_ITEMS = 8;
constexpr int SC_TILE = SC_BLOCK * SC_ITEMS;

__device__ __forceinline__ void scan_load_items(const u32 * __restrict__ data, u64 n, u64 base, u32 (&v)[SC_ITEMS]) {
    static_assert(SC_ITEMS == 8, "two uint4 per thread");
    if (base + SC_ITEMS <= n && (reinterpret_cast<uintptr_t>(data) & 15u) == 0) {
        const uint4 a = *reinterpret_cast<const uint4 *>(data + base);
        const uint4 b = *reinterpret_cast<const uint4 *>(data + base + 4);
        v[0] = a.x; v[1] = a.y; v[2] = a.z; v[3] = a.w;
        v[4] = b.x; v[5] = b.y; v[6] = b.z; v[7] = b.w;
    } else {
        const u64 last = n - 1;
#pragma unroll
        for (int k = 0; k < SC_ITEMS; k++) v[k] = data[base + k < n ? base + k : last];
#pragma unroll
        for (int k = 0; k < SC_ITEMS; k++) v[k] = base + k < n ? v[k] : 0u;
    }
}

__global__ void __launch_bounds__(SC_BLOCK) k_scan_reduce(const u32 * __restrict__ data, u64 n, u32 * __restrict__ sums) {
    __shared__ u32 lds[SC_BLOCK / WAVE + 1];
    const u64 base = (u64)blockIdx.x * SC_TILE + (u64)threadIdx.x * SC_ITEMS;
    u32 v[SC_ITEMS];
    scan_load_items(data, n, base, v);
    u32 acc = 0;
#pragma unroll
    for (int k = 0; k < SC_ITEMS; k++) acc += v[k];
    u32 tot = block_sum<SC_BLOCK>(acc, lds);
    if (threadIdx.x == 0) sums[blockIdx.x] = tot;
}

__global__ void __launch_bounds__(SC_BLOCK) k_scan_apply(u32 * __restrict__ data, u64 n, const u32 * __restrict__ sums,
                                                         u32 * __restrict__ total_out) {
    __shared__ u32 lds[SC_BLOCK / WAVE + 1];
    const u64 base = (u64)blockIdx.x * SC_TILE + (u64)threadIdx.x * SC_ITEMS;
    u32 v[SC_ITEMS];
    scan_load_items(data, n, base, v);
    u32 acc = 0;
#pragma unroll
    for (int k = 0; k < SC_ITEMS; k++) acc += v[k];
    u32 tot;
    u32 pre = block_excl_add<SC_BLOCK>(acc, lds, tot);
    if (sums) pre += sums[blockIdx.x];
    if (base + SC_ITEMS <= n && (reinterpret_cast<uintptr_t>(data) & 15u) == 0) {
        uint4 a, b;
        a.x = pre; a.y = a.x + v[0]; a.z = a.y + v[1]; a.w = a.z + v[2];
        b.x = a.w + v[3]; b.y = b.x + v[4]; b.z = b.y + v[5]; b.w = b.z + v[6];
        *reinterpret_cast<uint4 *>(data + base) = a;
        *reinterpret_cast<uint4 *>(data + base + 4) = b;
    } else {
#pragma unroll
        for (int k = 0; k < SC_ITEMS; k++) {
            if (base + k < n) data[base + k] = pre;
            pre += v[k];
        }
    }
    if (total_out && gridDim.x == 1 && threadIdx.x == 0) *total_out = tot;
}

__global__ void k_add_last(const u32 * __restrict__ sums_excl, const u32 * __restrict__ last_tile_total, u32 * out) {
    *out = *sums_excl + *last_tile_total;
}

constexpr int SC1_BLOCK = 1024;
constexpr u64 SC1_MAX = 262144;
__global__ void __launch_bounds__(SC1_BLOCK) k_scan_single(u32 * __restrict__ data, u64 n, u32 * __restrict__ total_out) {
    __shared__ u32 lds[SC1_BLOCK / WAVE + 1];
    const u64 quads = (n + 3) / 4;
    const u64 per = (quads + SC1_BLOCK - 1) / SC1_BLOCK;
    const u64 q0 = (u64)threadIdx.x * per, q1 = q0 + per < quads ? q0 + per : quads;
    const bool vec = (reinterpret_cast<uintptr_t>(data) & 15u) == 0;
    auto load4 = [&](u64 q, u32 (&v)[4]) {
        if (vec && 4 * q + 4 <= n) {
            const uint4 a = *reinterpret_cast<const uint4 *>(data + 4 * q);
            v[0] = a.x; v[1] = a.y; v[2] = a.z; v[3] = a.w;
        } else {
#pragma unroll
            for (int k = 0; k < 4; k++) v[k] = 4 * q + k < n ? data[4 * q + k] : 0u;
        }
    };
    u32 acc = 0;
    for (u64 q = q0; q < q1; q++) {
        u32 v[4];
        load4(q, v);
        acc += v[0] + v[1] + v[2] + v[3];
    }
    u32 tot;
    u32 run = block_excl_add<SC1_BLOCK>(acc, lds, tot);
    for (u64 q = q0; q < q1; q++) {
        u32 v[4];
        load4(q, v);
        u32 o[4];
        o[0] = run; o[1] = o[0] + v[0]; o[2] = o[1] + v[1]; o[3] = o[2] + v[2];
        run = o[3] + v[3];
        if (vec && 4 * q + 4 <= n) {
            *reinterpret_cast<uint4 *>(data + 4 * q) = make_uint4(o[0], o[1], o[2], o[3]);
        } else {
#pragma unroll
            for (int k = 0; k < 4; k++)
                if (4 * q + k < n) data[4 * q + k] = o[k];
        }
    }
    if (total_out && threadIdx.x == 0) *total_out = tot;
}

static void scan_rec(u32 * d, u64 n, u32 * d_total, Arena & tmp, hipStream_t s) {
    if (n == 0) {
        if (d_total) HIP_CHECK(hipMemsetAsync(d_total, 0, 4, s));
        return;
    }
    if (n <= SC_TILE) {
        launch(k_scan_apply, dim3(1), dim3(SC_BLOCK), 0, s, d, n, (const u32 *)nullptr, d_total);
        return;
    }
    static const bool no_single = getenv("BZ3_SCAN_NO_SINGLE") != nullptr;
    if (n <= SC1_MAX && !no_single) {
        launch(k_scan_single, dim3(1), dim3(SC1_BLOCK), 0, s, d, n, d_total);
        return;
    }
    const u64 tiles = (n + SC_TILE - 1) / SC_TILE;
    size_t m = tmp.mark();
    u32 * sums = tmp.take<u32>(tiles + 1);
    launch(k_scan_reduce, dim3((u32)tiles), dim3(SC_BLOCK), 0, s, (const u32 *)d, n, sums);
    scan_rec(sums, tiles, d_total, tmp, s);
    launch(k_scan_apply, dim3((u32)tiles), dim3(SC_BLOCK), 0, s, d, n, (const u32 *)sums, (u32 *)nullptr);
    tmp.release(m);
}

void exclusive_scan_u32(u32 * d_data, u64 n, u32 * d_total, Arena & tmp, hipStream_t s) { scan_rec(d_data, n, d_total, tmp, s); }

constexpr int RS_WAVES = RS_BLOCK / WAVE;
constexpr int RS_ROUNDS = RS_TILE / RS_BLOCK;
constexpr int RS_WAVE_SPAN = RS_TILE / RS_WAVES;

__device__ __forceinline__ u32 rs_tile_of_block(u32 b, u32 tiles, bool xcd) {
    if (!xcd) return b;
    const u32 per = (tiles + 7u) / 8u;
    return (b & 7u) * per + (b >> 3);
}
inline u32 rs_grid(u32 tiles, bool xcd) { return xcd ? 8u * ((tiles + 7u) / 8u) : tiles; }

template <typename K, int BITS>
__device__ __forceinline__ u32 rs_digit(K key, int shift) {
    return (u32)(key >> shift) & ((1u << BITS) - 1u);
}

template <typename K, int BITS>
__global__ void __launch_bounds__(RS_BLOCK) k_rs_hist(const K * __restrict__ keys, u64 n, int shift, u32 * __restrict__ hist, u32 tiles, u32 xcd) {
    constexpr int RADIX = 1 << BITS;
    __shared__ u32 bins[RADIX];
    const u32 tile = rs_tile_of_block(blockIdx.x, tiles, xcd != 0u);
    if (tile >= tiles) return;
#pragma unroll
    for (int d = threadIdx.x; d < RADIX; d += RS_BLOCK) bins[d] = 0;
    __syncthreads();
    const u64 tile_base = (u64)tile * RS_TILE;
    const u64 wbase = tile_base + (u64)wave_id() * RS_WAVE_SPAN + lane_id();
    const u64 last = n - 1;
    K key[RS_ROUNDS];
#pragma unroll
    for (int r = 0; r < RS_ROUNDS; r++) {
        const u64 i = wbase + (u64)r * WAVE;
        key[r] = keys[i < n ? i : last];
    }
#pragma unroll
    for (int r = 0; r < RS_ROUNDS; r++) {
        const u64 i = wbase + (u64)r * WAVE;
        if (i < n) atomicAdd(&bins[rs_digit<K, BITS>(key[r], shift)], 1u);
    }
    __syncthreads();
#pragma unroll
    for (int d = threadIdx.x; d < RADIX; d += RS_BLOCK) hist[(u64)d * tiles + tile] = bins[d];
}

template <typename K, bool IOTA, bool WKEYS, int BITS, bool RAW>
__global__ void __launch_bounds__(RS_BLOCK) k_rs_scatter(const K * __restrict__ kin, K * __restrict__ kout, const u32 * __restrict__ vin,
                                                               u32 * __restrict__ vout, u64 n, int shift, const u32 * __restrict__ offs, u32 tiles,
                                                               u32 iota_split, u32 out_base, u32 xcd) {
    constexpr int RADIX = 1 << BITS;
    constexpr int DPT = RADIX / RS_BLOCK;
    static_assert(RADIX % RS_BLOCK == 0 && DPT >= 1, "a thread owns whole digits");
    __shared__ u32 cnt[RS_WAVES][RADIX];
    __shared__ u32 dstart[RADIX];
    __shared__ u32 gdelta[RADIX];
    __shared__ u32 scan_lds[RS_BLOCK / WAVE + 1];
    __shared__ K skey[RS_TILE];
    __shared__ u32 sval[RS_TILE];
    const u32 tile = rs_tile_of_block(blockIdx.x, tiles, xcd != 0u);
    if (tile >= tiles) return;
    const int w = wave_id(), l = lane_id();
#pragma unroll
    for (int k = 0; k < RS_WAVES; k++)
#pragma unroll
        for (int d = threadIdx.x; d < RADIX; d += RS_BLOCK) cnt[k][d] = 0;
    __syncthreads();

    const u64 tile_base = (u64)tile * RS_TILE;
    const u64 wbase = tile_base + (u64)w * RS_WAVE_SPAN + l;
    K key[RS_ROUNDS];
    u32 local[RS_ROUNDS];
    const u64 lt = lanemask_lt();
    const u64 last = n - 1;
#pragma unroll
    for (int r = 0; r < RS_ROUNDS; r++) {
        const u64 i = wbase + (u64)r * WAVE;
        key[r] = kin[i < n ? i : last];
    }
    u32 row_total[DPT], row_before[DPT];
    if (RAW) {
#pragma unroll
        for (int j = 0; j < DPT; j++) {
            const u32 * __restrict__ row = offs + (u64)(DPT * threadIdx.x + j) * tiles;
            u32 tot = 0, bef = 0;
#pragma unroll 4
            for (u32 t = 0; t < tiles; t++) {
                const u32 c = row[t];
                tot += c;
                bef += t < tile ? c : 0u;
            }
            row_total[j] = tot;
            row_before[j] = bef;
        }
    }
#pragma unroll
    for (int r = 0; r < RS_ROUNDS; r++) {
        const u64 i = wbase + (u64)r * WAVE;
        const bool valid = i < n;
        const u32 d = rs_digit<K, BITS>(key[r], shift);
        u64 peers = __ballot(valid);
#pragma unroll
        for (int b = 0; b < BITS; b++) {
            const bool bit = (d >> b) & 1u;
            const u64 bal = __ballot(bit);
            peers &= bit ? bal : ~bal;
        }
        const u32 below = (u32)__popcll(peers & lt);
        const u32 pre = valid ? cnt[w][d] : 0u;
        wave_sync();
        if (valid && below == 0) cnt[w][d] = pre + (u32)__popcll(peers);
        wave_sync();
        local[r] = pre + below;
    }
    u32 val[RS_ROUNDS];
#pragma unroll
    for (int r = 0; r < RS_ROUNDS; r++) {
        const u64 i = wbase + (u64)r * WAVE;
        val[r] = IOTA ? (u32)i + ((u32)i >= iota_split ? 1u : 0u) : vin[i < n ? i : last];
    }
    __syncthreads();
    {
        u32 run[DPT];
        u32 mine = 0;
#pragma unroll
        for (int j = 0; j < DPT; j++) {
            const u32 d = DPT * threadIdx.x + j;
            u32 acc = 0;
#pragma unroll
            for (int k = 0; k < RS_WAVES; k++) {
                u32 c = cnt[k][d];
                cnt[k][d] = acc;
                acc += c;
            }
            run[j] = acc;
            mine += acc;
        }
        u32 total;
        u32 start = block_excl_add<RS_BLOCK>(mine, scan_lds, total);
        u32 gbase = 0;
        if (RAW) {
            u32 rt = 0;
#pragma unroll
            for (int j = 0; j < DPT; j++) rt += row_total[j];
            u32 all;
            gbase = block_excl_add<RS_BLOCK>(rt, scan_lds, all);
        }
#pragma unroll
        for (int j = 0; j < DPT; j++) {
            const u32 d = DPT * threadIdx.x + j;
            dstart[d] = start;
            if (RAW) {
                gdelta[d] = gbase + row_before[j] + out_base - start;
                gbase += row_total[j];
            } else {
                gdelta[d] = offs[(u64)d * tiles + tile] + out_base - start;
            }
            start += run[j];
        }
    }
    __syncthreads();
#pragma unroll
    for (int r = 0; r < RS_ROUNDS; r++) {
        const u32 d = rs_digit<K, BITS>(key[r], shift);
        local[r] += dstart[d] + cnt[w][d];
    }
#pragma unroll
    for (int r = 0; r < RS_ROUNDS; r++) {
        const u64 i = wbase + (u64)r * WAVE;
        if (i < n) {
            skey[local[r]] = key[r];
            sval[local[r]] = val[r];
        }
    }
    __syncthreads();
    const u64 left = n - tile_base;
    const u32 count = left < (u64)RS_TILE ? (u32)left : (u32)RS_TILE;
#pragma unroll
    for (int q = 0; q < RS_ROUNDS; q++) {
        const u32 j = (u32)q * RS_BLOCK + threadIdx.x;
        if (j < count) {
            const K k = skey[j];
            const u32 pos = gdelta[rs_digit<K, BITS>(k, shift)] + j;
            if (WKEYS) kout[pos] = k;
            vout[pos] = sval[j];
        }
    }
}

constexpr u32 RS_RAW_TILES = 128;

template <typename K, int BITS>
void radix_pass_bits(const K * kin, K * kout, const u32 * vin, u32 * vout, u64 n, int shift, u32 iota_split, u32 out_base, Arena & tmp,
                     hipStream_t s) {
    if (n == 0) return;
    constexpr int RADIX = 1 << BITS;
    const u32 tiles = (u32)((n + RS_TILE - 1) / RS_TILE);
    size_t m = tmp.mark();
    u32 * hist = tmp.take<u32>((size_t)tiles * RADIX);
    const u32 xcd = 1u;
    const dim3 sgrid(rs_grid(tiles, xcd != 0u));
    launch(k_rs_hist<K, BITS>, sgrid, dim3(RS_BLOCK), 0, s, kin, n, shift, hist, tiles, xcd);
    static const bool no_raw = getenv("BZ3_RS_NO_RAW") != nullptr;
    const bool raw = tiles <= RS_RAW_TILES && !no_raw;
    if (!raw) exclusive_scan_u32(hist, (u64)tiles * RADIX, nullptr, tmp, s);
    const bool iota = vin == nullptr, wkeys = kout != nullptr;
#define BZ3_RS_LAUNCH(I, W, R) \
    launch(k_rs_scatter<K, I, W, BITS, R>, sgrid, dim3(RS_BLOCK), 0, s, kin, kout, vin, vout, n, shift, (const u32 *)hist, tiles, iota_split, out_base, xcd)
#define BZ3_RS_DISPATCH(R)                                   \
    do {                                                     \
        if (iota && wkeys) BZ3_RS_LAUNCH(true, true, R);     \
        else if (iota) BZ3_RS_LAUNCH(true, false, R);        \
        else if (wkeys) BZ3_RS_LAUNCH(false, true, R);       \
        else BZ3_RS_LAUNCH(false, false, R);                 \
    } while (0)
    if (raw) BZ3_RS_DISPATCH(true);
    else BZ3_RS_DISPATCH(false);
#undef BZ3_RS_DISPATCH
#undef BZ3_RS_LAUNCH
    tmp.release(m);
}

void radix_hist_bits9(const u32 * keys, u64 n, int shift, u32 * hist, u32 tiles, hipStream_t s) {
    launch(k_rs_hist<u32, 9>, dim3(rs_grid(tiles, true)), dim3(RS_BLOCK), 0, s, keys, n, shift, hist, tiles, 1u);
}

template <typename K>
void radix_pass(const K * kin, K * kout, const u32 * vin, u32 * vout, u64 n, int shift, u32 iota_split, u32 out_base, Arena & tmp,
                hipStream_t s) {
    radix_pass_bits<K, 8>(kin, kout, vin, vout, n, shift, iota_split, out_base, tmp, s);
}

template <typename K>
int radix_sort_pairs(K * k0, K * k1, u32 * v0, u32 * v1, u64 n, int bit_lo, int bit_hi, Arena & tmp, hipStream_t s) {
    int cur = 0;
    for (int shift = bit_lo; shift < bit_hi; shift += 8) {
        if (cur == 0)
            radix_pass<K>(k0, k1, v0, v1, n, shift, 0xFFFFFFFFu, 0u, tmp, s);
        else
            radix_pass<K>(k1, k0, v1, v0, n, shift, 0xFFFFFFFFu, 0u, tmp, s);
        cur ^= 1;
    }
    return cur;
}

template void radix_pass<u8>(const u8 *, u8 *, const u32 *, u32 *, u64, int, u32, u32, Arena &, hipStream_t);
template void radix_pass<u32>(const u32 *, u32 *, const u32 *, u32 *, u64, int, u32, u32, Arena &, hipStream_t);
template void radix_pass<u64>(const u64 *, u64 *, const u32 *, u32 *, u64, int, u32, u32, Arena &, hipStream_t);
template void radix_pass_bits<u32, 9>(const u32 *, u32 *, const u32 *, u32 *, u64, int, u32, u32, Arena &, hipStream_t);
template int radix_sort_pairs<u32>(u32 *, u32 *, u32 *, u32 *, u64, int, int, Arena &, hipStream_t);
template int radix_sort_pairs<u64>(u64 *, u64 *, u32 *, u32 *, u64, int, int, Arena &, hipStream_t);

}
```

bzip3_amd/csrc/sort.hpp:

```cpp
#pragma once
#include "hipx.hpp"

namespace bz3 {

struct Arena {
    char * base = nullptr;
    size_t cap = 0, used = 0;
    template <typename T>
    T * take(size_t count) {
        size_t bytes = (count * sizeof(T) + 255) & ~(size_t)255;
        if (used + bytes > cap) throw HipError{hipErrorUnknown, "device workspace exhausted", __FILE__, __LINE__};
        T * p = reinterpret_cast<T *>(base + used);
        used += bytes;
        return p;
    }
    size_t mark() const { return used; }
    void release(size_t m) { used = m; }
};

constexpr int RS_TILE = 4096;
constexpr int RS_BLOCK = 256;
constexpr int RS_RADIX = 256;

inline size_t scan_temp_words(u64 n) {
    size_t w = 0;
    while (n > 2048) {
        n = (n + 2047) / 2048;
        w += ((n + 63) & ~(u64)63);
    }
    return w + 64;
}
inline size_t radix_temp_bytes(u64 n, int bits = 8) {
    u64 tiles = (n + RS_TILE - 1) / RS_TILE;
    u64 hist = tiles << bits;
    return (hist + scan_temp_words(hist) + 256) * 4 + 4096;
}

void exclusive_scan_u32(u32 * d_data, u64 n, u32 * d_total, Arena & tmp, hipStream_t s);

template <typename K>
void radix_pass(const K * kin, K * kout, const u32 * vin, u32 * vout, u64 n, int shift, u32 iota_split, u32 out_base,
                Arena & tmp, hipStream_t s);

template <typename K, int BITS>
void radix_pass_bits(const K * kin, K * kout, const u32 * vin, u32 * vout, u64 n, int shift, u32 iota_split, u32 out_base,
                     Arena & tmp, hipStream_t s);

void radix_hist_bits9(const u32 * keys, u64 n, int shift, u32 * hist, u32 tiles, hipStream_t s);

template <typename K>
int radix_sort_pairs(K * k0, K * k1, u32 * v0, u32 * v1, u64 n, int bit_lo, int bit_hi, Arena & tmp, hipStream_t s);

}
```

bzip3_amd/csrc/stages.hpp:

```cpp
#pragma once
#include "hipx.hpp"
#include "sort.hpp"

namespace bz3 {

struct CrcTables {
    u32 pow2[64];
    u32 lane[64];
    u32 row;
    u32 pad[3];
};
void crc_build_tables(CrcTables & t);
void crc32c_device(const u8 * d_data, u64 n, u32 init, const CrcTables * d_tables, u32 * d_scratch, hipStream_t s);
struct CrcBuf {
    u64 ptr;
    u64 size;
    u32 init;
    u32 first_seg;
};
u64 crc_many_segments(const void * ptr, u64 size);
unsigned crc32c_device_many(const CrcBuf * d_bufs, u32 n, u32 total_seg, const CrcTables * d_tables, u32 * d_crcs, hipStream_t s);

struct MrleEncScratch {
    u32 tiles = 0;
    u32 * carry = nullptr;
    u32 * tile_sum = nullptr;
    s32 * gain = nullptr;
    u32 * total = nullptr;
};
void mrle_encode_size(const u8 * d_in, u32 n, MrleEncScratch & sc, Arena & tmp, hipStream_t s);
void mrle_encode_write(const u8 * d_in, u32 n, const MrleEncScratch & sc, u8 * d_out, hipStream_t s);
void mrle_decode(const u8 * d_enc, u32 m, u8 * d_out, u32 outlen, u32 * d_total, Arena & tmp, hipStream_t s);

struct LzDriverOut {
    u32 end_pos;
    u32 n_matches;
    u32 iterations;
    u32 evaluated;
};
struct LzpEncodeCtx {
    bool active = false;
    const u8 * in = nullptr;
    u32 n = 0, nwords = 0;
    u32 *prev = nullptr, *next = nullptr, *skip = nullptr, *mstart = nullptr, *cand_bits = nullptr, *mpos = nullptr, *mlen = nullptr;
    LzDriverOut * d_res = nullptr;
};
struct LzpDriverJob {
    u64 in;
    u64 prev, next, cand_bits, skip, mstart, mpos, mlen;
    u64 result;
    u32 n, nwords;
};
size_t lzp_encode_ctx_bytes(u64 n);
void lzp_encode_prepare(const u8 * d_in, u32 n, LzpEncodeCtx & c, Arena & tmp, hipStream_t s);
void lzp_encode_prepare(const u8 * d_in, u32 n, LzpEncodeCtx & c, Arena & ctx, Arena & tmp, hipStream_t s);
LzpDriverJob lzp_driver_job(const LzpEncodeCtx & c);
void lzp_driver_batch(const LzpDriverJob * h_jobs, LzpDriverJob * d_jobs, u32 njobs, hipStream_t s);
s32 lzp_encode_finish(const LzpEncodeCtx & c, u8 * d_out, Arena & tmp, hipStream_t s);
s32 lzp_encode(const u8 * d_in, u32 n, u8 * d_out, Arena & tmp, hipStream_t s);
struct LzpDecodeJob {
    u64 in;
    u64 out;
    u64 lut;
    u64 result;
    u32 n, max_out;
};
constexpr size_t LZP_LUT_WORDS = (size_t)1 << 18;
void lzp_decode_batch(const LzpDecodeJob * h_jobs, LzpDecodeJob * d_jobs, u32 njobs, hipStream_t s);

struct BwtStats {
    int rounds = 0;
    u64 sorted_elements = 0;
    int radix_passes = 0;
};
constexpr int BWT_ROUTE_KEEP = 40;
s32 bwt_forward(const u8 * d_in, u32 n, u8 * d_out, Arena & tmp, hipStream_t s, BwtStats * stats, u32 * d_idx = nullptr, u32 * d_outside = nullptr);
size_t bwt_workspace_bytes(u64 n);
void bwt_set_big_rounds(int k);

constexpr u32 UNBWT_LANES_PER_CU = 2048;
void bwt_inverse(const u8 * d_in, u32 n, u32 idx, u8 * d_out, Arena & tmp, hipStream_t s, u32 lanes = 0);
size_t unbwt_workspace_bytes(u64 n);
int unbwt_log_stride(u32 rows, u32 lanes);
void unbwt_set_log_stride(int v);

constexpr u32 CM_NO_GAP = 0xFFFFFFFFu;
struct CmEncodeJob {
    u64 in;
    u64 out;
    u64 out_size;
    u32 n;
    u32 debug;
    u64 spill = 0;
    u64 status = 0;
    u32 miss_base = 0, miss_shift = 0;
    u32 gap = CM_NO_GAP, side_cap = 0;
    u64 side = 0;
    u64 claim = 0;
};
constexpr u32 CM_CLAIM_WORDS = 4096;
struct CmDecodeJob {
    u64 in;
    u64 out;
    u32 in_size;
    u32 n;
    u32 debug;
    u32 pad;
    u64 spill = 0, status = 0;
    u32 miss_base = 0, miss_shift = 0;
};
enum { CM_VARIANT_FULL = 0, CM_VARIANT_ROWS = 1, CM_VARIANT_ROWS3 = 2, CM_VARIANT_ROWS_TEST = 9  };
inline bool cm_variant_has_rows(int v) { return v != CM_VARIANT_FULL; }
inline bool cm_variant_is_test(int v) { return v == CM_VARIANT_ROWS_TEST; }
constexpr size_t CM_SPILL_BYTES = 256 * 256 * 2;
constexpr u32 CM_MISS_BASE = 1024, CM_MISS_SHIFT = 5;
void cm_encode_batch(const CmEncodeJob * d_jobs, u32 njobs, hipStream_t s, int variant = CM_VARIANT_FULL);
void cm_decode_batch(const CmDecodeJob * d_jobs, u32 njobs, hipStream_t s, int variant = CM_VARIANT_FULL, bool prof = false);

}
```

bzip3_amd/csrc/unbwt.hip:

```cpp
#include "prims.hpp"
#include "sort.hpp"
#include "stages.hpp"

#include <atomic>

namespace bz3 {

constexpr int UB_BLOCK = 256;
constexpr u32 UB_EVERY_ROW = 1u << 17;
constexpr int UB_MIN_LOG_STRIDE = 3, UB_MAX_LOG_STRIDE = 8;

__device__ __forceinline__ bool ub_is_splitter(u32 row, u32 idx, int log_stride) {
    if (row == 0 || row == idx || log_stride == 0) return true;
    return ((row * 0x9E3779B1u) >> (32 - log_stride)) == 0u;
}

constexpr u32 UB_BOUND_MARGIN = 64;
static inline u32 ub_split_bound(u32 rows, int log_stride) {
    if (log_stride == 0) return rows;
    const u64 b = ((u64)rows >> log_stride) + 2 + UB_BOUND_MARGIN;
    return b < rows ? (u32)b : rows;
}
__device__ __forceinline__ u32 ub_count(const u32 * __restrict__ d_total, u32 bound) {
    const u32 t = *d_total;
    return t < bound ? t : bound;
}
__device__ __forceinline__ u32 ub_sid(const u32 * __restrict__ sid, u32 row, u32 bound) {
    const u32 v = sid[row];
    return v < bound ? v : bound - 1;
}

__global__ void __launch_bounds__(UB_BLOCK) k_ub_hist(const u8 * __restrict__ in, u32 n, u32 * __restrict__ hist) {
    __shared__ u32 bins[256];
    bins[threadIdx.x] = 0;
    __syncthreads();
    const u64 base = (u64)blockIdx.x * (UB_BLOCK * 64);
    const u64 last = (u64)n - 1;
    for (u32 g = 0; g < 4; g++) {
        u8 c[16];
#pragma unroll
        for (u32 k = 0; k < 16; k++) {
            const u64 i = base + (u64)(g * 16 + k) * UB_BLOCK + threadIdx.x;
            c[k] = in[i < n ? i : last];
        }
#pragma unroll
        for (u32 k = 0; k < 16; k++) {
            const u64 i = base + (u64)(g * 16 + k) * UB_BLOCK + threadIdx.x;
            if (i < n) atomicAdd(&bins[c[k]], 1u);
        }
    }
    __syncthreads();
    if (bins[threadIdx.x]) atomicAdd(&hist[threadIdx.x], bins[threadIdx.x]);
}

__global__ void __launch_bounds__(256) k_ub_cum(const u32 * __restrict__ hist, u32 * __restrict__ cum, u32 * __restrict__ psi, u32 idx) {
    __shared__ u32 lds[256 / WAVE + 1];
    u32 tot;
    u32 pre = block_excl_add<256>(hist[threadIdx.x], lds, tot);
    cum[threadIdx.x] = pre + 1;
    if (threadIdx.x == 0) {
        cum[256] = tot + 1;
        psi[0] = idx;
    }
}

__global__ void __launch_bounds__(UB_BLOCK) k_ub_flags(u32 rows, u32 idx, int log_stride, u32 * __restrict__ flags) {
    const u32 r = blockIdx.x * UB_BLOCK + threadIdx.x;
    if (r < rows) flags[r] = ub_is_splitter(r, idx, log_stride) ? 1u : 0u;
}

__global__ void __launch_bounds__(UB_BLOCK) k_ub_collect(u32 rows, u32 idx, int log_stride, const u32 * __restrict__ sid, u32 bound, u32 * __restrict__ split_row) {
    const u32 r = blockIdx.x * UB_BLOCK + threadIdx.x;
    if (r < rows && ub_is_splitter(r, idx, log_stride)) {
        const u32 j = sid[r];
        if (j < bound) split_row[j] = r;
    }
}

__device__ __forceinline__ u32 ub_symbol_lds(const u32 * c, u32 r) {
    u32 lo = 0, hi = 256;
#pragma unroll
    for (int b = 0; b < 8; b++) {
        const u32 mid = (lo + hi) >> 1;
        if (c[mid] <= r) lo = mid; else hi = mid;
    }
    return lo;
}

__global__ void __launch_bounds__(UB_BLOCK) k_ub_walk(const u32 * __restrict__ psi, const u32 * __restrict__ sid, const u32 * __restrict__ split_row,
                                                     const u32 * __restrict__ d_total, u32 bound, u32 idx, int log_stride, u32 rows, const u32 * __restrict__ cum,
                                                     u32 cap, u32 * __restrict__ succ, u32 * __restrict__ dist, u32 * __restrict__ seg_len, u8 * __restrict__ slab,
                                                     u32 * __restrict__ resume) {
    __shared__ u32 c[257];
    for (int k = threadIdx.x; k < 257; k += UB_BLOCK) c[k] = cum[k];
    __syncthreads();
    const u32 j = blockIdx.x * UB_BLOCK + threadIdx.x;
    if (j >= ub_count(d_total, bound)) return;
    u32 r = split_row[j];
    if (r == 0) {
        succ[j] = j;
        dist[j] = 0;
        seg_len[j] = 0;
        return;
    }
    u32 * __restrict__ mine = reinterpret_cast<u32 *>(slab + (size_t)j * cap);
    u32 len = 0, word = 0;
    do {
        const u32 nr = psi[r];
        if (len < cap) {
            word |= ub_symbol_lds(c, r) << (8u * (len & 3u));
            if ((len & 3u) == 3u) {
                mine[len >> 2] = word;
                word = 0;
            }
        } else if (len == cap) {
            resume[j] = r;
        }
        r = nr;
        len++;
    } while (!ub_is_splitter(r, idx, log_stride) && len <= rows);
    if (len < cap && (len & 3u)) mine[len >> 2] = word;
    succ[j] = ub_sid(sid, r, bound);
    dist[j] = len;
    seg_len[j] = len;
}

__global__ void __launch_bounds__(UB_BLOCK) k_ub_jump(const u32 * __restrict__ succ_in, const u32 * __restrict__ dist_in, const u32 * __restrict__ d_total, u32 bound,
                                                     u32 * __restrict__ succ_out, u32 * __restrict__ dist_out) {
    const u32 j = blockIdx.x * UB_BLOCK + threadIdx.x;
    if (j >= ub_count(d_total, bound)) return;
    const u32 sj = succ_in[j];
    u64 d = (u64)dist_in[j] + dist_in[sj];
    dist_out[j] = d > 0xFFFFFFFFull ? 0xFFFFFFFFu : (u32)d;
    succ_out[j] = succ_in[sj];
}

__global__ void __launch_bounds__(UB_BLOCK) k_ub_place(const u8 * __restrict__ slab, const u32 * __restrict__ seg_len, const u32 * __restrict__ dist,
                                                      const u32 * __restrict__ succ, const u32 * __restrict__ sid, u32 idx, u32 cap,
                                                      const u32 * __restrict__ d_total, u32 bound, u32 n, u8 * __restrict__ out) {
    const u32 t = blockIdx.x * UB_BLOCK + threadIdx.x;
    const u32 j = t >> 4, part = t & 15u;
    if (j >= ub_count(d_total, bound)) return;
    if (succ[j] != sid[0]) return;
    const u32 D = dist[ub_sid(sid, idx, bound)];
    const u32 d = dist[j];
    if (d > D) return;
    const u32 len = seg_len[j];
    const u32 m = len < cap ? len : cap;
    const u32 limit = n & ~1u;
    const u64 pos0 = (u64)D - d;
    const u8 * __restrict__ src = slab + (size_t)j * cap;
    for (u32 o = part * 16u; o < m; o += 256u) {
        if (o + 16u <= m && pos0 + o + 16u <= limit) {
            const uint4 q = *reinterpret_cast<const uint4 *>(src + o);
            PackedU128 w;
            w.v[0] = q.x; w.v[1] = q.y; w.v[2] = q.z; w.v[3] = q.w;
            *reinterpret_cast<PackedU128 *>(out + pos0 + o) = w;
        } else {
            for (u32 k = o; k < m && k < o + 16u; k++)
                if (pos0 + k < limit) out[pos0 + k] = src[k];
        }
    }
}

__global__ void __launch_bounds__(UB_BLOCK) k_ub_walk_long(const u32 * __restrict__ psi, const u32 * __restrict__ resume, const u32 * __restrict__ seg_len,
                                                          const u32 * __restrict__ dist, const u32 * __restrict__ succ, const u32 * __restrict__ sid, u32 idx,
                                                          const u32 * __restrict__ cum, u32 cap, const u32 * __restrict__ d_total, u32 bound, u32 n,
                                                          u8 * __restrict__ out) {
    __shared__ u32 c[257];
    for (int k = threadIdx.x; k < 257; k += UB_BLOCK) c[k] = cum[k];
    __syncthreads();
    const u32 j = blockIdx.x * UB_BLOCK + threadIdx.x;
    if (j >= ub_count(d_total, bound)) return;
    const u32 len = seg_len[j];
    if (len <= cap) return;
    if (succ[j] != sid[0]) return;
    const u32 D = dist[ub_sid(sid, idx, bound)];
    const u32 d = dist[j];
    if (d > D) return;
    const u32 limit = n & ~1u;
    u32 r = resume[j];
    u64 pos = (u64)D - d + cap;
    for (u32 t = cap; t < len; t++) {
        const u32 nr = psi[r];
        const u32 sym = ub_symbol_lds(c, r);
        if (pos < limit) out[pos] = (u8)sym;
        pos++;
        r = nr;
    }
}

__device__ __forceinline__ u32 ub_first_symbol(const u32 * __restrict__ cum, u32 r) {
    u32 lo = 0, hi = 256;
    for (int b = 0; b < 8; b++) {
        const u32 mid = (lo + hi) >> 1;
        if (cum[mid] <= r) lo = mid; else hi = mid;
    }
    return lo;
}

__global__ void __launch_bounds__(UB_BLOCK) k_ub_tail(const u8 * __restrict__ in, const u32 * __restrict__ psi, const u32 * __restrict__ cum,
                                                     const u32 * __restrict__ dist, const u32 * __restrict__ sid, u32 idx, u32 bound, u32 n, u8 * __restrict__ out) {
    const u32 D = dist[ub_sid(sid, idx, bound)];
    const u32 limit = n & ~1u;
    const u32 lastc = in[0];
    const u32 E = cum[lastc];
    const u32 gid = blockIdx.x * UB_BLOCK + threadIdx.x;
    u32 start = D;
    if (D < limit && (D & 1u)) {
        int shift = 0;
        while ((n >> shift) > (1u << 17)) shift++;
        const bool same_group = E >= 2 && ((E - 1) >> shift) == (E >> shift);
        if (gid == 0) {
            if (same_group || E + 1 > n) {
                out[D] = 0;
            } else {
                out[D - 1] = (u8)ub_first_symbol(cum, E + 1);
                out[D] = (u8)ub_first_symbol(cum, psi[E + 1]);
            }
        }
        start = D + 1;
    }
    if (start < limit) {
        const u32 q0 = (E == 1) ? 2u : 1u;
        const u32 hi = ub_first_symbol(cum, q0), lo = ub_first_symbol(cum, psi[q0]);
        for (u64 j = (u64)start + gid; j < limit; j += (u64)gridDim.x * UB_BLOCK)
            if (j != n - 1) out[j] = (u8)((j & 1u) ? lo : hi);
    }
    if (gid == 0) out[n - 1] = (u8)lastc;
}

size_t unbwt_workspace_bytes(u64 n) {
    const u64 rows = n + 1;
    const u64 splitters = rows < UB_EVERY_ROW ? rows : (rows >> UB_MIN_LOG_STRIDE) + 2 + UB_BOUND_MARGIN;
    return (n + 64) * 8 + radix_temp_bytes(n) + scan_temp_words(n + 1) * 4 + (splitters + 4096) * 32 + (n + (n >> 3)) * 4 + (1u << 20);
}

static std::atomic<int> g_ub_force_log_stride{-1};
void unbwt_set_log_stride(int v) { g_ub_force_log_stride.store(v >= 0 && v <= UB_MAX_LOG_STRIDE ? v : -1); }

static u32 ub_device_lanes() {
    static std::atomic<u32> cached[64];
    int dev = 0;
    if (hipGetDevice(&dev) != hipSuccess || dev < 0 || dev >= 64) dev = 0;
    u32 v = cached[dev].load();
    if (v == 0) {
        int cus = 0;
#ifndef BZ3_EMU
        if (hipDeviceGetAttribute(&cus, hipDeviceAttributeMultiprocessorCount, dev) != hipSuccess) cus = 0;
#endif
        if (cus <= 0) cus = 256;
        v = (u32)cus * UNBWT_LANES_PER_CU;
        cached[dev].store(v);
    }
    return v;
}

int unbwt_log_stride(u32 rows, u32 lanes) {
    const int forced = g_ub_force_log_stride.load();
    if (forced >= 0) return forced;
    if (rows < UB_EVERY_ROW) return 0;
    int log_stride = UB_MIN_LOG_STRIDE;
    while (log_stride < UB_MAX_LOG_STRIDE && ((u64)rows >> log_stride) > lanes) log_stride++;
    return log_stride;
}

void bwt_inverse(const u8 * d_in, u32 n, u32 idx, u8 * d_out, Arena & tmp, hipStream_t s, u32 lanes) {
    if (n == 0) return;
    if (n == 1) {
        HIP_CHECK(hipMemcpyAsync(d_out, d_in, 1, hipMemcpyDeviceToDevice, s));
        return;
    }
    const size_t mk = tmp.mark();
    const u32 rows = n + 1;
    u32 * psi = tmp.take<u32>(rows);
    u32 * sid = tmp.take<u32>(rows);
    u32 * hist = tmp.take<u32>(256);
    u32 * cum = tmp.take<u32>(257);
    u32 * d_total = tmp.take<u32>(1);

    HIP_CHECK(hipMemsetAsync(hist, 0, 256 * 4, s));
    launch(k_ub_hist, dim3((u32)(((u64)n + UB_BLOCK * 64 - 1) / (UB_BLOCK * 64))), dim3(UB_BLOCK), 0, s, d_in, n, hist);
    launch(k_ub_cum, dim3(1), dim3(256), 0, s, (const u32 *)hist, cum, psi, idx);
    radix_pass<u8>(d_in, (u8 *)nullptr, (const u32 *)nullptr, psi, n, 0, idx, 1u, tmp, s);

    const int log_stride = unbwt_log_stride(rows, lanes ? lanes : ub_device_lanes());
    const u32 bound = ub_split_bound(rows, log_stride);
    const dim3 grows((rows + UB_BLOCK - 1) / UB_BLOCK);
    launch(k_ub_flags, grows, dim3(UB_BLOCK), 0, s, rows, idx, log_stride, sid);
    exclusive_scan_u32(sid, rows, d_total, tmp, s);
    u32 * split_row = tmp.take<u32>(bound);
    u32 * seg_len = tmp.take<u32>(bound);
    u32 * resume = tmp.take<u32>(bound);
    u32 * succ[2] = {tmp.take<u32>(bound), tmp.take<u32>(bound)};
    u32 * dist[2] = {tmp.take<u32>(bound), tmp.take<u32>(bound)};
    const u32 cap = 4u << log_stride;
    u8 * slab = tmp.take<u8>((size_t)bound * cap + 64);
    const dim3 gs((bound + UB_BLOCK - 1) / UB_BLOCK);
    launch(k_ub_collect, grows, dim3(UB_BLOCK), 0, s, rows, idx, log_stride, (const u32 *)sid, bound, split_row);
    launch(k_ub_walk, gs, dim3(UB_BLOCK), 0, s, (const u32 *)psi, (const u32 *)sid, (const u32 *)split_row, (const u32 *)d_total, bound, idx, log_stride, rows,
           (const u32 *)cum, cap, succ[0], dist[0], seg_len, slab, resume);

    int cur = 0;
    for (u64 span = 1; span < bound; span <<= 1) {
        launch(k_ub_jump, gs, dim3(UB_BLOCK), 0, s, (const u32 *)succ[cur], (const u32 *)dist[cur], (const u32 *)d_total, bound, succ[cur ^ 1], dist[cur ^ 1]);
        cur ^= 1;
    }
    launch(k_ub_place, dim3((u32)(((u64)bound * 16 + UB_BLOCK - 1) / UB_BLOCK)), dim3(UB_BLOCK), 0, s, (const u8 *)slab, (const u32 *)seg_len, (const u32 *)dist[cur],
           (const u32 *)succ[cur], (const u32 *)sid, idx, cap, (const u32 *)d_total, bound, n, d_out);
    launch(k_ub_walk_long, gs, dim3(UB_BLOCK), 0, s, (const u32 *)psi, (const u32 *)resume, (const u32 *)seg_len, (const u32 *)dist[cur], (const u32 *)succ[cur],
           (const u32 *)sid, idx, (const u32 *)cum, cap, (const u32 *)d_total, bound, n, d_out);
    launch(k_ub_tail, dim3(256), dim3(UB_BLOCK), 0, s, d_in, (const u32 *)psi, (const u32 *)cum, (const u32 *)dist[cur], (const u32 *)sid, idx, bound, n, d_out);
    tmp.release(mk);
}

}
```

include/bz3_hip.h:

```cpp
#ifndef BZ3_HIP_H
#define BZ3_HIP_H
#include <stddef.h>
#include <stdint.h>
#include "libbz3.h"
#define BZ3_HIP 1

#ifdef __cplusplus
extern "C" {
#endif

BZIP3_API int bz3_hip_device_count(void);
BZIP3_API int bz3_hip_bind_device(int device);
BZIP3_API int bz3_hip_state_device(struct bz3_state * state);

BZIP3_API int bz3_hip_set_cm_mode(int mode);
BZIP3_API void bz3_hip_debug_bwt_big_rounds(int k);
BZIP3_API void bz3_hip_debug_set_unbwt_log_stride(int log_stride);
BZIP3_API unsigned bz3_hip_cm_blocks_given_up(void);
BZIP3_API unsigned bz3_hip_cm_blocks_routed_full(void);

BZIP3_API int bz3_hip_cm_variant_for(int device, int blocks, int encode);

BZIP3_API int bz3_hip_debug_peak_concurrent_groups(int reset);

BZIP3_API int bz3_hip_debug_front_end_ring(void);
BZIP3_API int bz3_hip_set_keep_workspace(int on);
BZIP3_API int bz3_hip_set_front_end_duo(int on);
BZIP3_API void bz3_hip_set_workspace_headroom(long long bytes);
BZIP3_API size_t bz3_hip_workspace_headroom(void);
BZIP3_API unsigned bz3_hip_debug_headroom_events(int reset, unsigned * releases);
BZIP3_API size_t bz3_hip_debug_ring_contexts(size_t free_bytes, size_t have, size_t need, size_t fixed, size_t ctx_bytes, size_t cap, int lean, size_t headroom);
BZIP3_API size_t bz3_hip_debug_arena_slack(size_t bytes);
BZIP3_API unsigned bz3_hip_debug_cm_launches(int reset);
BZIP3_API size_t bz3_hip_debug_workspace_bytes(size_t block_bytes, int which);
BZIP3_API size_t bz3_hip_debug_cached_bytes(int device);
BZIP3_API int bz3_hip_debug_arena_swap_buffers(int reset);

BZIP3_API int bz3_hip_set_lean_states(int on);
BZIP3_API void bz3_hip_release_cached_memory(void);

BZIP3_API int32_t bz3_hip_encode_block_device(struct bz3_state * state, void * buffer, int32_t size);
BZIP3_API int32_t bz3_hip_decode_block_device(struct bz3_state * state, void * buffer, size_t buffer_size, int32_t compressed_size,
                                              int32_t orig_size);
BZIP3_API void bz3_hip_encode_blocks_device(struct bz3_state * states[], void * buffers[], int32_t sizes[], int32_t n);
BZIP3_API void bz3_hip_decode_blocks_device(struct bz3_state * states[], void * buffers[], size_t buffer_sizes[], int32_t sizes[],
                                            int32_t orig_sizes[], int32_t n);

BZIP3_API int bz3_hip_compress_device(uint32_t block_size, const void * in, void * out, size_t in_size, size_t * out_size);
BZIP3_API int bz3_hip_decompress_device(const void * in, void * out, size_t in_size, size_t * out_size);
BZIP3_API int bz3_hip_frame_decoded_size_device(const void * in, size_t in_size, size_t * decoded_size);
BZIP3_API int bz3_hip_compress_device_many(uint32_t block_size, int32_t n, const void * const ins[], const size_t in_sizes[],
                                           void * const outs[], size_t out_sizes[], int rcs[]);
BZIP3_API int bz3_hip_decompress_device_many(int32_t n, const void * const ins[], const size_t in_sizes[],
                                             void * const outs[], size_t out_sizes[], int rcs[]);
BZIP3_API int bz3_hip_frame_decoded_sizes_device(int32_t n, const void * const ins[], const size_t in_sizes[],
                                                 size_t decoded_sizes[], int rcs[]);
BZIP3_API int32_t bz3_hip_debug_copy_segments(const void * src, void * dst, const uint64_t * segs, int32_t n);

BZIP3_API int bz3_hip_compress_device_planes(uint32_t block_size, uint32_t elem_size, const void * in, void * out, size_t in_size,
                                             size_t * out_size);
BZIP3_API int bz3_hip_decompress_device_planes(uint32_t elem_size, const void * in, void * out, size_t in_size, size_t * out_size);
BZIP3_API int bz3_hip_compress_device_planes_many(uint32_t block_size, int32_t n, const uint32_t elem_sizes[], const void * const ins[],
                                                  const size_t in_sizes[], void * const outs[], size_t out_sizes[], int rcs[]);
BZIP3_API int bz3_hip_decompress_device_planes_many(int32_t n, const uint32_t elem_sizes[], const void * const ins[],
                                                    const size_t in_sizes[], void * const outs[], size_t out_sizes[], int rcs[]);
BZIP3_API int32_t bz3_hip_debug_planes(const void * src, void * dst, const uint64_t * segs, int32_t n);

BZIP3_API int bz3_hip_compress_device_delta(uint32_t block_size, uint32_t elem_size, const void * in, const void * base, void * out,
                                            size_t in_size, size_t * out_size);
BZIP3_API int bz3_hip_decompress_device_delta(uint32_t elem_size, const void * in, const void * base, size_t base_size, void * out,
                                              size_t in_size, size_t * out_size);
BZIP3_API int bz3_hip_compress_device_delta_many(uint32_t block_size, int32_t n, const uint32_t elem_sizes[], const void * const ins[],
                                                 const void * const bases[], const size_t in_sizes[], void * const outs[],
                                                 size_t out_sizes[], int rcs[]);
BZIP3_API int bz3_hip_decompress_device_delta_many(int32_t n, const uint32_t elem_sizes[], const void * const ins[],
                                                   const size_t in_sizes[], const void * const bases[], const size_t base_sizes[],
                                                   void * const outs[], size_t out_sizes[], int rcs[]);
BZIP3_API int bz3_hip_crc32c_device(const void * p, size_t n, uint32_t init, uint32_t * crc);
BZIP3_API int bz3_hip_crc32c_device_many(int32_t n, const void * const * ptrs, const size_t * sizes, const uint32_t * inits, uint32_t * crcs);
BZIP3_API unsigned bz3_hip_debug_crc_launches(int reset);
BZIP3_API int32_t bz3_hip_debug_delta(const void * src, const void * base, void * dst, const uint64_t * segs, int32_t n);

BZIP3_API int bz3_hip_decompress_device_range(uint32_t elem_size, const void * in, size_t in_size, uint64_t offset, const void * base,
                                              size_t base_size, void * out, size_t * out_size);
BZIP3_API int bz3_hip_decompress_device_range_many(int32_t n, const uint32_t elem_sizes[], const void * const ins[], const size_t in_sizes[],
                                                   const uint64_t offsets[], const void * const bases[], const size_t base_sizes[],
                                                   void * const outs[], size_t out_sizes[], int rcs[]);
BZIP3_API int32_t bz3_hip_debug_range(const void * src, const void * base, void * dst, const uint64_t * segs, int32_t n);

BZIP3_API int bz3_hip_decompress_device_strided(uint32_t elem_size, const void * in, size_t in_size, uint64_t offset, uint64_t run,
                                                uint64_t stride, uint64_t count, const void * base, size_t base_size, void * out,
                                                size_t * out_size);
BZIP3_API int bz3_hip_decompress_device_strided_many(int32_t n, const uint32_t elem_sizes[], const void * const ins[], const size_t in_sizes[],
                                                     const uint64_t params[], const void * const bases[], const size_t base_sizes[],
                                                     void * const outs[], size_t out_sizes[], int rcs[]);
BZIP3_API int32_t bz3_hip_debug_strided(const void * src, const void * base, void * dst, const uint64_t * segs, int32_t n);

BZIP3_API int bz3_hip_decompress_device_select(uint32_t elem_size, const void * in, size_t in_size, uint64_t offset, uint64_t stride,
                                               uint64_t count, uint64_t m, const uint64_t * pieces, const void * base, size_t base_size,
                                               void * out, size_t * out_size);
BZIP3_API int bz3_hip_decompress_device_select_many(int32_t n, const uint32_t elem_sizes[], const void * const ins[], const size_t in_sizes[],
                                                    const uint64_t params[], const uint64_t * const pieces[], const void * const bases[],
                                                    const size_t base_sizes[], void * const outs[], size_t out_sizes[], int rcs[]);
BZIP3_API int32_t bz3_hip_debug_select(const void * src, const void * base, void * dst, const uint64_t * segs, int32_t n,
                                       const uint64_t * pieces, uint64_t n_pieces);

BZIP3_API int bz3_hip_update_device_range(uint32_t elem_size, const void * in, size_t in_size, uint64_t offset, const void * data, size_t w,
                                          const void * base, void * out, size_t * out_size);
BZIP3_API int bz3_hip_update_device_range_many(int32_t n, const uint32_t elem_sizes[], const void * const ins[], const size_t in_sizes[],
                                               const uint64_t offsets[], const void * const datas[], const size_t ws[],
                                               const void * const bases[], void * const outs[], size_t out_sizes[], int rcs[]);
BZIP3_API int32_t bz3_hip_debug_patch(const void * src, const void * base, void * dst, const uint64_t * segs, int32_t n);

enum {
    BZ3_HIP_T_CRC = 0,
    BZ3_HIP_T_RLE = 1,
    BZ3_HIP_T_LZP = 2,
    BZ3_HIP_T_BWT = 3,
    BZ3_HIP_T_CM = 4,
    BZ3_HIP_T_COPY = 5,
    BZ3_HIP_T_COUNT = 8
};
BZIP3_API void bz3_hip_last_timings(struct bz3_state * state, float ms[BZ3_HIP_T_COUNT]);
BZIP3_API void bz3_hip_last_bwt_stats(struct bz3_state * state, int32_t * rounds, int32_t * radix_passes, uint64_t * sorted_elements);

BZIP3_API void bz3_hip_set_collect_window_us(int us);
BZIP3_API unsigned bz3_hip_debug_collected_batches(int reset, unsigned * largest);

BZIP3_API uint32_t bz3_hip_stage_crc32c(const uint8_t * data, size_t n, uint32_t init);
BZIP3_API int32_t bz3_hip_stage_mrle_encode(const uint8_t * in, int32_t n, uint8_t * out);
BZIP3_API int bz3_hip_stage_mrle_decode(const uint8_t * in, uint8_t * out, int32_t outlen, int32_t maxin);
BZIP3_API int32_t bz3_hip_stage_lzp_encode(const uint8_t * in, int32_t n, uint8_t * out);
BZIP3_API int32_t bz3_hip_stage_lzp_decode(const uint8_t * in, int32_t n, uint8_t * out, int32_t max);
BZIP3_API int32_t bz3_hip_stage_bwt(const uint8_t * in, uint8_t * out, int32_t n);
BZIP3_API int32_t bz3_hip_stage_unbwt(const uint8_t * in, uint8_t * out, int32_t n, int32_t idx);
BZIP3_API int32_t bz3_hip_debug_cu_masks(int cus, int reserve, uint32_t * side, uint32_t * rest);
BZIP3_API int32_t bz3_hip_debug_scan_u32(uint32_t * data, uint32_t n, uint32_t * total);
BZIP3_API int32_t bz3_hip_debug_sort_u32(const uint32_t * keys, uint32_t n, int key_bits, int digit_bits, uint32_t * sorted_keys, uint32_t * sorted_index);
BZIP3_API float bz3_hip_stage_last_ms(void);
BZIP3_API int32_t bz3_hip_stage_cm_encode(const uint8_t * in, int32_t n, uint8_t * out);
BZIP3_API void bz3_hip_stage_cm_decode(const uint8_t * in, int32_t in_size, uint8_t * out, int32_t n);

#define BZ3_HIP_ERR_IO (-100)
BZIP3_API int bz3_hip_encode_stream(int in_fd, int out_fd, int32_t block_size, int32_t blocks_per_batch);
BZIP3_API int bz3_hip_decode_stream(int in_fd, int out_fd, int32_t blocks_per_batch);

BZIP3_API float bz3_hip_stage_cm_decode_many(const uint8_t * in, int32_t in_size, uint8_t * out, int32_t n, int32_t copies, uint64_t * counters);

BZIP3_API float bz3_hip_stage_cm_encode_many(const uint8_t * in, int32_t n, uint8_t * out, int32_t * coded, int32_t copies);

#ifdef __cplusplus
}
#endif
#endif
```

Before: 643.2.

## Batch inverse BWT across blocks in a decode window into shared launches

Decoding no longer runs the inverse BWT one block at a time with a sync after each. Blocks in a window are now gathered and processed together, with every unbwt kernel, the radix pass and the scan taking a second grid dimension indexed by job. This is meant to cut launch and sync overhead and fill the GPU when single 8 MiB blocks underuse it. In exchange, the batch needs workspace for each block and the batch size is limited by free arena space and available lanes, so per-block timing becomes an average.

```diff
diff --git a/bzip3_amd/__init__.py b/bzip3_amd/__init__.py
--- a/bzip3_amd/__init__.py
+++ b/bzip3_amd/__init__.py
@@ -109,6 +109,7 @@
         "bz3_hip_stage_lzp_decode": (i32, [vp, i32, vp, i32]),
         "bz3_hip_stage_bwt": (i32, [vp, vp, i32]),
         "bz3_hip_stage_unbwt": (i32, [vp, vp, i32, i32]),
+        "bz3_hip_debug_unbwt_many": (i32, [vp, vp, vp, vp, i32]),
         "bz3_hip_stage_last_ms": (C.c_float, []),
         "bz3_hip_debug_sort_u32": (i32, [vp, u32, C.c_int, C.c_int, vp, vp]),
         "bz3_hip_debug_scan_u32": (i32, [vp, u32, vp]),
@@ -216,6 +217,17 @@
         out = (C.c_uint8 * max(1, len(data)))()
         rc = self.lib.bz3_hip_stage_unbwt(_cbuf(data, len(data)), out, len(data), idx)
         return rc, C.string_at(out, len(data))
+
+    def unbwt_many(self, jobs):
+        k = len(jobs)
+        ins = [_cbuf(d, len(d)) for d, _ in jobs]
+        outs = [(C.c_uint8 * max(1, len(d)))() for d, _ in jobs]
+        inp = (C.c_void_p * max(1, k))(*[C.cast(b, C.c_void_p) for b in ins])
+        outp = (C.c_void_p * max(1, k))(*[C.cast(b, C.c_void_p) for b in outs])
+        n = (C.c_int32 * max(1, k))(*[len(d) for d, _ in jobs])
+        idx = (C.c_int32 * max(1, k))(*[i for _, i in jobs])
+        rc = self.lib.bz3_hip_debug_unbwt_many(inp, outp, n, idx, k)
+        return rc, [C.string_at(o, len(d)) for o, (d, _) in zip(outs, jobs)]
 
     def cm_encode(self, data):
         out = (C.c_uint8 * (len(data) + len(data) // 50 + 64))()
diff --git a/bzip3_amd/csrc/api_decode.hip b/bzip3_amd/csrc/api_decode.hip
--- a/bzip3_amd/csrc/api_decode.hip
+++ b/bzip3_amd/csrc/api_decode.hip
@@ -82,13 +82,13 @@
     st->pending = bz3_state::DEC_CODED;
 }
 
-bool decode_unbwt(bz3_state * st, Arena & arena, float cm_ms, u32 lanes) {
+int decode_unbwt_check(bz3_state * st, float cm_ms, UbBatchItem & item) {
     hipStream_t s = st->xs;
     st->t[BZ3_HIP_T_CM] = cm_ms;
     const s32 n = st->size_before_bwt;
     if (st->bwt_idx > n) {
         st->last_error = BZ3_ERR_MALFORMED_HEADER;
-        return false;
+        return -1;
     }
     u8 *b1 = st->d_swap, *b2 = st->user;
     if (st->lean) {
@@ -96,19 +96,20 @@
         b2 = st->d_swap;
     }
     const double t0 = now_ms();
+    int queued = 0;
     if (n <= 1) {
-        if (st->bwt_idx != n) { st->last_error = BZ3_ERR_BWT; return false; }
+        if (st->bwt_idx != n) { st->last_error = BZ3_ERR_BWT; return -1; }
         if (n == 1) HIP_CHECK(hipMemcpyAsync(b2, b1, 1, hipMemcpyDeviceToDevice, s));
     } else {
-        if (st->bwt_idx <= 0) { st->last_error = BZ3_ERR_BWT; return false; }
-        bwt_inverse(b1, (u32)n, (u32)st->bwt_idx, b2, arena, s, lanes);
-        HIP_CHECK(hipStreamSynchronize(s));
+        if (st->bwt_idx <= 0) { st->last_error = BZ3_ERR_BWT; return -1; }
+        item = UbBatchItem{b1, b2, (u32)n, (u32)st->bwt_idx};
+        queued = 1;
     }
     st->b1 = b2;
     st->b2 = b1;
     st->size_src = n;
     st->t[BZ3_HIP_T_BWT] = (float)(now_ms() - t0);
-    return true;
+    return queued;
 }
 
 void decode_finish(bz3_state * st, Arena & arena) {
@@ -315,6 +316,9 @@
     }
     const u32 unbwt_lanes = s != s_cm && lead->ctx->real_cus > lead->ctx->reserved_cus ? (u32)(lead->ctx->real_cus - lead->ctx->reserved_cus) * UNBWT_LANES_PER_CU : 0u;
     DrainOnUnwind drain_rest{s == s_cm ? nullptr : s, side_streams == lead->ctx->aux ? nullptr : side_streams, side_streams == lead->ctx->aux ? 0 : DeviceCtx::AUX};
+    std::vector<UbBatchItem> ub_items;
+    std::vector<u32> ub_sizes;
+    std::vector<s32> ub_owner;
     const s32 nwin = (n + tail_window - 1) / tail_window;
     const s32 lag = tail_slots - 1;
     static const bool trace_rings = getenv("BZ3_HIP_TRACE_RINGS") != nullptr;
@@ -330,6 +334,9 @@
             w.lz_jobs.clear();
             w.lz_owner.clear();
             w.alive.assign((size_t)(w.w1 - w.w0), 0);
+            ub_items.clear();
+            ub_sizes.clear();
+            ub_owner.clear();
             for (s32 i = w.w0; i < w.w1; i++) {
                 bz3_state * st = sts[i];
                 if (st->pending == bz3_state::DEC_STORED) {
@@ -340,8 +347,28 @@
                 }
                 if (st->pending != bz3_state::DEC_CODED) continue;
                 borrow(i);
-                if (!decode_unbwt(st, arena, cm_ms, unbwt_lanes)) continue;
+                UbBatchItem item{};
+                const int r = decode_unbwt_check(st, cm_ms, item);
+                if (r < 0) continue;
                 w.alive[(size_t)(i - w.w0)] = 1;
+                if (r > 0) {
+                    ub_items.push_back(item);
+                    ub_sizes.push_back(item.n);
+                    ub_owner.push_back(i);
+                }
+            }
+            for (size_t at = 0; at < ub_items.size();) {
+                const u32 b = unbwt_batch_size(ub_sizes.data() + at, (u32)(ub_items.size() - at), arena.cap - arena.used, unbwt_lanes);
+                const double t0 = now_ms();
+                bwt_inverse_batch(ub_items.data() + at, b, arena, s, unbwt_lanes);
+                HIP_CHECK(hipStreamSynchronize(s));
+                const float each = (float)(now_ms() - t0) / (float)b;
+                for (u32 j = 0; j < b; j++) sts[ub_owner[at + j]]->t[BZ3_HIP_T_BWT] = each;
+                at += b;
+            }
+            for (s32 i = w.w0; i < w.w1; i++) {
+                bz3_state * st = sts[i];
+                if (!w.alive[(size_t)(i - w.w0)]) continue;
                 if (st->model & 2) {
                     if (st->lzp_size < 4) {
                         st->last_error = BZ3_ERR_CRC;
diff --git a/bzip3_amd/csrc/api_hooks.hip b/bzip3_amd/csrc/api_hooks.hip
--- a/bzip3_amd/csrc/api_hooks.hip
+++ b/bzip3_amd/csrc/api_hooks.hip
@@ -164,6 +164,43 @@
         HIP_CHECK(hipStreamSynchronize(e.s));
         g_stage_ms.store(std::chrono::duration<float, std::milli>(std::chrono::steady_clock::now() - t0).count());
         e.down(out, o, (size_t)n);
+        return 0;
+    });
+}
+
+BZIP3_API int32_t bz3_hip_debug_unbwt_many(const uint8_t * const * in, uint8_t * const * out, const int32_t * n, const int32_t * idx, int32_t count) {
+    return stage_guard([&]() -> s32 {
+        if (count < 0 || (count > 0 && (!in || !out || !n || !idx))) return -1;
+        u64 largest = 0;
+        for (s32 k = 0; k < count; k++) {
+            if (n[k] < 0 || (n[k] <= 1 ? idx[k] != n[k] : (idx[k] <= 0 || idx[k] > n[k]))) return -1;
+            if ((u64)n[k] > largest) largest = (u64)n[k];
+        }
+        std::vector<UbBatchItem> items;
+        std::vector<u32> sizes;
+        std::vector<s32> owner;
+        StageEnv e;
+        for (s32 k = 0; k < count; k++) {
+            if (n[k] == 1) out[k][0] = in[k][0];
+            if (n[k] < 2) continue;
+            const u8 * d = e.dev((size_t)n[k] + 64, in[k], (size_t)n[k]);
+            items.push_back(UbBatchItem{d, e.dev((size_t)n[k] + 64), (u32)n[k], (u32)idx[k]});
+            sizes.push_back((u32)n[k]);
+            owner.push_back(k);
+        }
+        if (items.empty()) return 0;
+        const size_t plain = workspace_bytes_for(largest + 64), full = unbwt_batch_workspace_bytes(largest + 64, UB_MAX_BATCH);
+        Arena a = e.ctx->arena_for(plain > full ? plain : full);
+        HIP_CHECK(hipStreamSynchronize(e.s));
+        const auto t0 = std::chrono::steady_clock::now();
+        for (size_t at = 0; at < items.size();) {
+            const u32 b = unbwt_batch_size(sizes.data() + at, (u32)(items.size() - at), a.cap - a.used, 0u);
+            bwt_inverse_batch(items.data() + at, b, a, e.s);
+            HIP_CHECK(hipStreamSynchronize(e.s));
+            at += b;
+        }
+        g_stage_ms.store(std::chrono::duration<float, std::milli>(std::chrono::steady_clock::now() - t0).count());
+        for (size_t j = 0; j < items.size(); j++) e.down(out[owner[j]], items[j].out, (size_t)items[j].n);
         return 0;
     });
 }
diff --git a/bzip3_amd/csrc/sort.hip b/bzip3_amd/csrc/sort.hip
--- a/bzip3_amd/csrc/sort.hip
+++ b/bzip3_amd/csrc/sort.hip
@@ -23,22 +23,25 @@
     }
 }
 
-__global__ void __launch_bounds__(SC_BLOCK) k_scan_reduce(const u32 * __restrict__ data, u64 n, u32 * __restrict__ sums) {
+__device__ __forceinline__ void scan_reduce_body(const u32 * __restrict__ data, u64 n, u32 * __restrict__ sums, u32 bx) {
     __shared__ u32 lds[SC_BLOCK / WAVE + 1];
-    const u64 base = (u64)blockIdx.x * SC_TILE + (u64)threadIdx.x * SC_ITEMS;
+    const u64 base = (u64)bx * SC_TILE + (u64)threadIdx.x * SC_ITEMS;
     u32 v[SC_ITEMS];
     scan_load_items(data, n, base, v);
     u32 acc = 0;
 #pragma unroll
     for (int k = 0; k < SC_ITEMS; k++) acc += v[k];
     u32 tot = block_sum<SC_BLOCK>(acc, lds);
-    if (threadIdx.x == 0) sums[blockIdx.x] = tot;
-}
-
-__global__ void __launch_bounds__(SC_BLOCK) k_scan_apply(u32 * __restrict__ data, u64 n, const u32 * __restrict__ sums,
-                                                         u32 * __restrict__ total_out) {
+    if (threadIdx.x == 0) sums[bx] = tot;
+}
+__global__ void __launch_bounds__(SC_BLOCK) k_scan_reduce(const u32 * __restrict__ data, u64 n, u32 * __restrict__ sums) {
+    scan_reduce_body(data, n, sums, blockIdx.x);
+}
+
+__device__ __forceinline__ void scan_apply_body(u32 * __restrict__ data, u64 n, const u32 * __restrict__ sums, u32 * __restrict__ total_out, u32 bx,
+                                                bool one_tile) {
     __shared__ u32 lds[SC_BLOCK / WAVE + 1];
-    const u64 base = (u64)blockIdx.x * SC_TILE + (u64)threadIdx.x * SC_ITEMS;
+    const u64 base = (u64)bx * SC_TILE + (u64)threadIdx.x * SC_ITEMS;
     u32 v[SC_ITEMS];
     scan_load_items(data, n, base, v);
     u32 acc = 0;
@@ -46,7 +49,7 @@
     for (int k = 0; k < SC_ITEMS; k++) acc += v[k];
     u32 tot;
     u32 pre = block_excl_add<SC_BLOCK>(acc, lds, tot);
-    if (sums) pre += sums[blockIdx.x];
+    if (sums) pre += sums[bx];
     if (base + SC_ITEMS <= n && (reinterpret_cast<uintptr_t>(data) & 15u) == 0) {
         uint4 a, b;
         a.x = pre; a.y = a.x + v[0]; a.z = a.y + v[1]; a.w = a.z + v[2];
@@ -60,7 +63,11 @@
             pre += v[k];
         }
     }
-    if (total_out && gridDim.x == 1 && threadIdx.x == 0) *total_out = tot;
+    if (total_out && one_tile && threadIdx.x == 0) *total_out = tot;
+}
+__global__ void __launch_bounds__(SC_BLOCK) k_scan_apply(u32 * __restrict__ data, u64 n, const u32 * __restrict__ sums,
+                                                         u32 * __restrict__ total_out) {
+    scan_apply_body(data, n, sums, total_out, blockIdx.x, gridDim.x == 1);
 }
 
 __global__ void k_add_last(const u32 * __restrict__ sums_excl, const u32 * __restrict__ last_tile_total, u32 * out) {
@@ -69,7 +76,7 @@
 
 constexpr int SC1_BLOCK = 1024;
 constexpr u64 SC1_MAX = 262144;
-__global__ void __launch_bounds__(SC1_BLOCK) k_scan_single(u32 * __restrict__ data, u64 n, u32 * __restrict__ total_out) {
+__device__ __forceinline__ void scan_single_body(u32 * __restrict__ data, u64 n, u32 * __restrict__ total_out) {
     __shared__ u32 lds[SC1_BLOCK / WAVE + 1];
     const u64 quads = (n + 3) / 4;
     const u64 per = (quads + SC1_BLOCK - 1) / SC1_BLOCK;
@@ -108,6 +115,14 @@
     }
     if (total_out && threadIdx.x == 0) *total_out = tot;
 }
+__global__ void __launch_bounds__(SC1_BLOCK) k_scan_single(u32 * __restrict__ data, u64 n, u32 * __restrict__ total_out) {
+    scan_single_body(data, n, total_out);
+}
+
+static bool scan_no_single() {
+    static const bool v = getenv("BZ3_SCAN_NO_SINGLE") != nullptr;
+    return v;
+}
 
 static void scan_rec(u32 * d, u64 n, u32 * d_total, Arena & tmp, hipStream_t s) {
     if (n == 0) {
@@ -118,8 +133,7 @@
         launch(k_scan_apply, dim3(1), dim3(SC_BLOCK), 0, s, d, n, (const u32 *)nullptr, d_total);
         return;
     }
-    static const bool no_single = getenv("BZ3_SCAN_NO_SINGLE") != nullptr;
-    if (n <= SC1_MAX && !no_single) {
+    if (n <= SC1_MAX && !scan_no_single()) {
         launch(k_scan_single, dim3(1), dim3(SC1_BLOCK), 0, s, d, n, d_total);
         return;
     }
@@ -134,6 +148,71 @@
 
 void exclusive_scan_u32(u32 * d_data, u64 n, u32 * d_total, Arena & tmp, hipStream_t s) { scan_rec(d_data, n, d_total, tmp, s); }
 
+struct ScanBatch {
+    u32 count;
+    struct Job {
+        u32 * data;
+        u32 * sums;
+        u32 * total;
+        u64 n;
+    } job[SORT_MAX_BATCH];
+};
+__global__ void __launch_bounds__(SC_BLOCK) k_scan_reduce_many(ScanBatch b) {
+    const ScanBatch::Job & j = b.job[blockIdx.y];
+    if ((u64)blockIdx.x * SC_TILE >= j.n) return;
+    scan_reduce_body(j.data, j.n, j.sums, blockIdx.x);
+}
+__global__ void __launch_bounds__(SC_BLOCK) k_scan_apply_many(ScanBatch b) {
+    const ScanBatch::Job & j = b.job[blockIdx.y];
+    if ((u64)blockIdx.x * SC_TILE >= j.n) return;
+    scan_apply_body(j.data, j.n, j.sums, j.total, blockIdx.x, j.n <= (u64)SC_TILE);
+}
+__global__ void __launch_bounds__(SC1_BLOCK) k_scan_single_many(ScanBatch b) {
+    const ScanBatch::Job & j = b.job[blockIdx.y];
+    scan_single_body(j.data, j.n, j.total);
+}
+
+static void scan_rec_many(ScanBatch b, Arena & tmp, hipStream_t s) {
+    u64 longest = 0;
+    for (u32 k = 0; k < b.count; k++) longest = b.job[k].n > longest ? b.job[k].n : longest;
+    for (u32 k = 0; k < b.count; k++) b.job[k].sums = nullptr;
+    if (longest <= SC_TILE) {
+        launch(k_scan_apply_many, dim3(1, b.count), dim3(SC_BLOCK), 0, s, b);
+        return;
+    }
+    if (longest <= SC1_MAX && !scan_no_single()) {
+        launch(k_scan_single_many, dim3(1, b.count), dim3(SC1_BLOCK), 0, s, b);
+        return;
+    }
+    const u32 tiles = (u32)((longest + SC_TILE - 1) / SC_TILE);
+    size_t m = tmp.mark();
+    ScanBatch sub = b, top = b;
+    for (u32 k = 0; k < b.count; k++) {
+        const u64 t = (b.job[k].n + SC_TILE - 1) / SC_TILE;
+        u32 * sums = tmp.take<u32>(t + 1);
+        top.job[k].sums = sums;
+        top.job[k].total = nullptr;
+        sub.job[k].data = sums;
+        sub.job[k].n = t;
+    }
+    launch(k_scan_reduce_many, dim3(tiles, b.count), dim3(SC_BLOCK), 0, s, top);
+    scan_rec_many(sub, tmp, s);
+    launch(k_scan_apply_many, dim3(tiles, b.count), dim3(SC_BLOCK), 0, s, top);
+    tmp.release(m);
+}
+
+void exclusive_scan_u32_many(u32 * const * d_data, const u64 * n, u32 * const * d_totals, u32 count, Arena & tmp, hipStream_t s) {
+    if (count == 0 || count > SORT_MAX_BATCH) throw HipError{hipErrorUnknown, "scan batch of a size the job table does not hold", __FILE__, __LINE__};
+    ScanBatch b;
+    b.count = count;
+    for (u32 k = 0; k < SORT_MAX_BATCH; k++) {
+        const u32 j = k < count ? k : 0;
+        if (n[j] == 0) throw HipError{hipErrorUnknown, "scan batch with an empty table", __FILE__, __LINE__};
+        b.job[k] = ScanBatch::Job{d_data[j], nullptr, d_totals ? d_totals[j] : nullptr, n[j]};
+    }
+    scan_rec_many(b, tmp, s);
+}
+
 constexpr int RS_WAVES = RS_BLOCK / WAVE;
 constexpr int RS_ROUNDS = RS_TILE / RS_BLOCK;
 constexpr int RS_WAVE_SPAN = RS_TILE / RS_WAVES;
@@ -143,7 +222,7 @@
     const u32 per = (tiles + 7u) / 8u;
     return (b & 7u) * per + (b >> 3);
 }
-inline u32 rs_grid(u32 tiles, bool xcd) { return xcd ? 8u * ((tiles + 7u) / 8u) : tiles; }
+__host__ __device__ inline u32 rs_grid(u32 tiles, bool xcd) { return xcd ? 8u * ((tiles + 7u) / 8u) : tiles; }
 
 template <typename K, int BITS>
 __device__ __forceinline__ u32 rs_digit(K key, int shift) {
@@ -151,10 +230,10 @@
 }
 
 template <typename K, int BITS>
-__global__ void __launch_bounds__(RS_BLOCK) k_rs_hist(const K * __restrict__ keys, u64 n, int shift, u32 * __restrict__ hist, u32 tiles, u32 xcd) {
+__device__ __forceinline__ void rs_hist_body(const K * __restrict__ keys, u64 n, int shift, u32 * __restrict__ hist, u32 tiles, u32 xcd, u32 bx) {
     constexpr int RADIX = 1 << BITS;
     __shared__ u32 bins[RADIX];
-    const u32 tile = rs_tile_of_block(blockIdx.x, tiles, xcd != 0u);
+    const u32 tile = rs_tile_of_block(bx, tiles, xcd != 0u);
     if (tile >= tiles) return;
 #pragma unroll
     for (int d = threadIdx.x; d < RADIX; d += RS_BLOCK) bins[d] = 0;
@@ -177,151 +256,56 @@
 #pragma unroll
     for (int d = threadIdx.x; d < RADIX; d += RS_BLOCK) hist[(u64)d * tiles + tile] = bins[d];
 }
+template <typename K, int BITS>
+__global__ void __launch_bounds__(RS_BLOCK) k_rs_hist(const K * __restrict__ keys, u64 n, int shift, u32 * __restrict__ hist, u32 tiles, u32 xcd) {
+    rs_hist_body<K, BITS>(keys, n, shift, hist, tiles, xcd, blockIdx.x);
+}
 
 template <typename K, bool IOTA, bool WKEYS, int BITS, bool RAW>
 __global__ void __launch_bounds__(RS_BLOCK) k_rs_scatter(const K * __restrict__ kin, K * __restrict__ kout, const u32 * __restrict__ vin,
                                                                u32 * __restrict__ vout, u64 n, int shift, const u32 * __restrict__ offs, u32 tiles,
                                                                u32 iota_split, u32 out_base, u32 xcd) {
-    constexpr int RADIX = 1 << BITS;
-    constexpr int DPT = RADIX / RS_BLOCK;
-    static_assert(RADIX % RS_BLOCK == 0 && DPT >= 1, "a thread owns whole digits");
-    __shared__ u32 cnt[RS_WAVES][RADIX];
-    __shared__ u32 dstart[RADIX];
-    __shared__ u32 gdelta[RADIX];
-    __shared__ u32 scan_lds[RS_BLOCK / WAVE + 1];
-    __shared__ K skey[RS_TILE];
-    __shared__ u32 sval[RS_TILE];
-    const u32 tile = rs_tile_of_block(blockIdx.x, tiles, xcd != 0u);
-    if (tile >= tiles) return;
-    const int w = wave_id(), l = lane_id();
-#pragma unroll
-    for (int k = 0; k < RS_WAVES; k++)
-#pragma unroll
-        for (int d = threadIdx.x; d < RADIX; d += RS_BLOCK) cnt[k][d] = 0;
-    __syncthreads();
-
-    const u64 tile_base = (u64)tile * RS_TILE;
-    const u64 wbase = tile_base + (u64)w * RS_WAVE_SPAN + l;
-    K key[RS_ROUNDS];
-    u32 local[RS_ROUNDS];
-    const u64 lt = lanemask_lt();
-    const u64 last = n - 1;
-#pragma unroll
-    for (int r = 0; r < RS_ROUNDS; r++) {
-        const u64 i = wbase + (u64)r * WAVE;
-        key[r] = kin[i < n ? i : last];
-    }
-    u32 row_total[DPT], row_before[DPT];
-    if (RAW) {
-#pragma unroll
-        for (int j = 0; j < DPT; j++) {
-            const u32 * __restrict__ row = offs + (u64)(DPT * threadIdx.x + j) * tiles;
-            u32 tot = 0, bef = 0;
-#pragma unroll 4
-            for (u32 t = 0; t < tiles; t++) {
-                const u32 c = row[t];
-                tot += c;
-                bef += t < tile ? c : 0u;
-            }
-            row_total[j] = tot;
-            row_before[j] = bef;
-        }
-    }
-#pragma unroll
-    for (int r = 0; r < RS_ROUNDS; r++) {
-        const u64 i = wbase + (u64)r * WAVE;
-        const bool valid = i < n;
-        const u32 d = rs_digit<K, BITS>(key[r], shift);
-        u64 peers = __ballot(valid);
-#pragma unroll
-        for (int b = 0; b < BITS; b++) {
-            const bool bit = (d >> b) & 1u;
-            const u64 bal = __ballot(bit);
-            peers &= bit ? bal : ~bal;
-        }
-        const u32 below = (u32)__popcll(peers & lt);
-        const u32 pre = valid ? cnt[w][d] : 0u;
-        wave_sync();
-        if (valid && below == 0) cnt[w][d] = pre + (u32)__popcll(peers);
-        wave_sync();
-        local[r] = pre + below;
-    }
-    u32 val[RS_ROUNDS];
-#pragma unroll
-    for (int r = 0; r < RS_ROUNDS; r++) {
-        const u64 i = wbase + (u64)r * WAVE;
-        val[r] = IOTA ? (u32)i + ((u32)i >= iota_split ? 1u : 0u) : vin[i < n ? i : last];
-    }
-    __syncthreads();
-    {
-        u32 run[DPT];
-        u32 mine = 0;
-#pragma unroll
-        for (int j = 0; j < DPT; j++) {
-            const u32 d = DPT * threadIdx.x + j;
-            u32 acc = 0;
-#pragma unroll
-            for (int k = 0; k < RS_WAVES; k++) {
-                u32 c = cnt[k][d];
-                cnt[k][d] = acc;
-                acc += c;
-            }
-            run[j] = acc;
-            mine += acc;
-        }
-        u32 total;
-        u32 start = block_excl_add<RS_BLOCK>(mine, scan_lds, total);
-        u32 gbase = 0;
-        if (RAW) {
-            u32 rt = 0;
-#pragma unroll
-            for (int j = 0; j < DPT; j++) rt += row_total[j];
-            u32 all;
-            gbase = block_excl_add<RS_BLOCK>(rt, scan_lds, all);
-        }
-#pragma unroll
-        for (int j = 0; j < DPT; j++) {
-            const u32 d = DPT * threadIdx.x + j;
-            dstart[d] = start;
-            if (RAW) {
-                gdelta[d] = gbase + row_before[j] + out_base - start;
-                gbase += row_total[j];
-            } else {
-                gdelta[d] = offs[(u64)d * tiles + tile] + out_base - start;
-            }
-            start += run[j];
-        }
-    }
-    __syncthreads();
-#pragma unroll
-    for (int r = 0; r < RS_ROUNDS; r++) {
-        const u32 d = rs_digit<K, BITS>(key[r], shift);
-        local[r] += dstart[d] + cnt[w][d];
-    }
-#pragma unroll
-    for (int r = 0; r < RS_ROUNDS; r++) {
-        const u64 i = wbase + (u64)r * WAVE;
-        if (i < n) {
-            skey[local[r]] = key[r];
-            sval[local[r]] = val[r];
-        }
-    }
-    __syncthreads();
-    const u64 left = n - tile_base;
-    const u32 count = left < (u64)RS_TILE ? (u32)left : (u32)RS_TILE;
-#pragma unroll
-    for (int q = 0; q < RS_ROUNDS; q++) {
-        const u32 j = (u32)q * RS_BLOCK + threadIdx.x;
-        if (j < count) {
-            const K k = skey[j];
-            const u32 pos = gdelta[rs_digit<K, BITS>(k, shift)] + j;
-            if (WKEYS) kout[pos] = k;
-            vout[pos] = sval[j];
-        }
-    }
+#include "sort_scatter_body.hpp"
+}
+
+struct RsBatch8 {
+    u32 count;
+    struct Job {
+        const u8 * keys;
+        u32 * vout;
+        u32 * hist;
+        u64 n;
+        u32 tiles, iota_split;
+    } job[SORT_MAX_BATCH];
+};
+__global__ void __launch_bounds__(RS_BLOCK) k_rs_hist_many(RsBatch8 b, int shift, u32 xcd) {
+    const RsBatch8::Job & j = b.job[blockIdx.y];
+    if (blockIdx.x >= rs_grid(j.tiles, xcd != 0u)) return;
+    rs_hist_body<u8, 8>(j.keys, j.n, shift, j.hist, j.tiles, xcd, blockIdx.x);
+}
+template <bool RAW>
+__global__ void __launch_bounds__(RS_BLOCK) k_rs_scatter_many(RsBatch8 b, int shift, u32 out_base, u32 xcd) {
+    typedef u8 K;
+    constexpr bool IOTA = true, WKEYS = false;
+    constexpr int BITS = 8;
+    const RsBatch8::Job & j = b.job[blockIdx.y];
+    if (blockIdx.x >= rs_grid(j.tiles, xcd != 0u)) return;
+    const u8 * __restrict__ kin = j.keys;
+    u8 * __restrict__ kout = nullptr;
+    const u32 * __restrict__ vin = nullptr;
+    u32 * __restrict__ vout = j.vout;
+    const u32 * __restrict__ offs = j.hist;
+    const u64 n = j.n;
+    const u32 tiles = j.tiles, iota_split = j.iota_split;
+#include "sort_scatter_body.hpp"
 }
 
 constexpr u32 RS_RAW_TILES = 128;
+
+static bool rs_no_raw() {
+    static const bool v = getenv("BZ3_RS_NO_RAW") != nullptr;
+    return v;
+}
 
 template <typename K, int BITS>
 void radix_pass_bits(const K * kin, K * kout, const u32 * vin, u32 * vout, u64 n, int shift, u32 iota_split, u32 out_base, Arena & tmp,
@@ -334,8 +318,7 @@
     const u32 xcd = 1u;
     const dim3 sgrid(rs_grid(tiles, xcd != 0u));
     launch(k_rs_hist<K, BITS>, sgrid, dim3(RS_BLOCK), 0, s, kin, n, shift, hist, tiles, xcd);
-    static const bool no_raw = getenv("BZ3_RS_NO_RAW") != nullptr;
-    const bool raw = tiles <= RS_RAW_TILES && !no_raw;
+    const bool raw = tiles <= RS_RAW_TILES && !rs_no_raw();
     if (!raw) exclusive_scan_u32(hist, (u64)tiles * RADIX, nullptr, tmp, s);
     const bool iota = vin == nullptr, wkeys = kout != nullptr;
 #define BZ3_RS_LAUNCH(I, W, R) \
@@ -354,6 +337,33 @@
     tmp.release(m);
 }
 
+void radix_pass_iota_u8_many(const RadixIotaJob * jobs, u32 count, u32 out_base, Arena & tmp, hipStream_t s) {
+    if (count == 0 || count > SORT_MAX_BATCH) throw HipError{hipErrorUnknown, "radix batch of a size the job table does not hold", __FILE__, __LINE__};
+    RsBatch8 b;
+    b.count = count;
+    size_t m = tmp.mark();
+    u32 most = 0;
+    u32 * tables[SORT_MAX_BATCH];
+    u64 words[SORT_MAX_BATCH];
+    for (u32 k = 0; k < count; k++) {
+        if (jobs[k].n == 0) throw HipError{hipErrorUnknown, "radix batch with an empty array", __FILE__, __LINE__};
+        const u32 tiles = (u32)((jobs[k].n + RS_TILE - 1) / RS_TILE);
+        words[k] = (u64)tiles * RS_RADIX;
+        tables[k] = tmp.take<u32>((size_t)words[k]);
+        b.job[k] = RsBatch8::Job{jobs[k].keys, jobs[k].vout, tables[k], jobs[k].n, tiles, jobs[k].iota_split};
+        most = tiles > most ? tiles : most;
+    }
+    for (u32 k = count; k < SORT_MAX_BATCH; k++) b.job[k] = b.job[0];
+    const u32 xcd = 1u;
+    const dim3 grid(rs_grid(most, true), count);
+    launch(k_rs_hist_many, grid, dim3(RS_BLOCK), 0, s, b, 0, xcd);
+    const bool raw = most <= RS_RAW_TILES && !rs_no_raw();
+    if (!raw) exclusive_scan_u32_many(tables, words, nullptr, count, tmp, s);
+    if (raw) launch(k_rs_scatter_many<true>, grid, dim3(RS_BLOCK), 0, s, b, 0, out_base, xcd);
+    else launch(k_rs_scatter_many<false>, grid, dim3(RS_BLOCK), 0, s, b, 0, out_base, xcd);
+    tmp.release(m);
+}
+
 void radix_hist_bits9(const u32 * keys, u64 n, int shift, u32 * hist, u32 tiles, hipStream_t s) {
     launch(k_rs_hist<u32, 9>, dim3(rs_grid(tiles, true)), dim3(RS_BLOCK), 0, s, keys, n, shift, hist, tiles, 1u);
 }
diff --git a/bzip3_amd/csrc/sort.hpp b/bzip3_amd/csrc/sort.hpp
--- a/bzip3_amd/csrc/sort.hpp
+++ b/bzip3_amd/csrc/sort.hpp
@@ -38,6 +38,16 @@
 
 void exclusive_scan_u32(u32 * d_data, u64 n, u32 * d_total, Arena & tmp, hipStream_t s);
 
+constexpr u32 SORT_MAX_BATCH = 4;
+void exclusive_scan_u32_many(u32 * const * d_data, const u64 * n, u32 * const * d_totals, u32 count, Arena & tmp, hipStream_t s);
+struct RadixIotaJob {
+    const u8 * keys;
+    u32 * vout;
+    u64 n;
+    u32 iota_split;
+};
+void radix_pass_iota_u8_many(const RadixIotaJob * jobs, u32 count, u32 out_base, Arena & tmp, hipStream_t s);
+
 template <typename K>
 void radix_pass(const K * kin, K * kout, const u32 * vin, u32 * vout, u64 n, int shift, u32 iota_split, u32 out_base,
                 Arena & tmp, hipStream_t s);
diff --git a/bzip3_amd/csrc/sort_scatter_body.hpp b/bzip3_amd/csrc/sort_scatter_body.hpp
--- /dev/null
+++ b/bzip3_amd/csrc/sort_scatter_body.hpp
@@ -0,0 +1,137 @@
+    constexpr int RADIX = 1 << BITS;
+    constexpr int DPT = RADIX / RS_BLOCK;
+    static_assert(RADIX % RS_BLOCK == 0 && DPT >= 1, "a thread owns whole digits");
+    __shared__ u32 cnt[RS_WAVES][RADIX];
+    __shared__ u32 dstart[RADIX];
+    __shared__ u32 gdelta[RADIX];
+    __shared__ u32 scan_lds[RS_BLOCK / WAVE + 1];
+    __shared__ K skey[RS_TILE];
+    __shared__ u32 sval[RS_TILE];
+    const u32 tile = rs_tile_of_block(blockIdx.x, tiles, xcd != 0u);
+    if (tile >= tiles) return;
+    const int w = wave_id(), l = lane_id();
+#pragma unroll
+    for (int k = 0; k < RS_WAVES; k++)
+#pragma unroll
+        for (int d = threadIdx.x; d < RADIX; d += RS_BLOCK) cnt[k][d] = 0;
+    __syncthreads();
+
+    const u64 tile_base = (u64)tile * RS_TILE;
+    const u64 wbase = tile_base + (u64)w * RS_WAVE_SPAN + l;
+    K key[RS_ROUNDS];
+    u32 local[RS_ROUNDS];
+    const u64 lt = lanemask_lt();
+    const u64 last = n - 1;
+#pragma unroll
+    for (int r = 0; r < RS_ROUNDS; r++) {
+        const u64 i = wbase + (u64)r * WAVE;
+        key[r] = kin[i < n ? i : last];
+    }
+    u32 row_total[DPT], row_before[DPT];
+    if (RAW) {
+#pragma unroll
+        for (int j = 0; j < DPT; j++) {
+            const u32 * __restrict__ row = offs + (u64)(DPT * threadIdx.x + j) * tiles;
+            u32 tot = 0, bef = 0;
+#pragma unroll 4
+            for (u32 t = 0; t < tiles; t++) {
+                const u32 c = row[t];
+                tot += c;
+                bef += t < tile ? c : 0u;
+            }
+            row_total[j] = tot;
+            row_before[j] = bef;
+        }
+    }
+#pragma unroll
+    for (int r = 0; r < RS_ROUNDS; r++) {
+        const u64 i = wbase + (u64)r * WAVE;
+        const bool valid = i < n;
+        const u32 d = rs_digit<K, BITS>(key[r], shift);
+        u64 peers = __ballot(valid);
+#pragma unroll
+        for (int b = 0; b < BITS; b++) {
+            const bool bit = (d >> b) & 1u;
+            const u64 bal = __ballot(bit);
+            peers &= bit ? bal : ~bal;
+        }
+        const u32 below = (u32)__popcll(peers & lt);
+        const u32 pre = valid ? cnt[w][d] : 0u;
+        wave_sync();
+        if (valid && below == 0) cnt[w][d] = pre + (u32)__popcll(peers);
+        wave_sync();
+        local[r] = pre + below;
+    }
+    u32 val[RS_ROUNDS];
+#pragma unroll
+    for (int r = 0; r < RS_ROUNDS; r++) {
+        const u64 i = wbase + (u64)r * WAVE;
+        val[r] = IOTA ? (u32)i + ((u32)i >= iota_split ? 1u : 0u) : vin[i < n ? i : last];
+    }
+    __syncthreads();
+    {
+        u32 run[DPT];
+        u32 mine = 0;
+#pragma unroll
+        for (int j = 0; j < DPT; j++) {
+            const u32 d = DPT * threadIdx.x + j;
+            u32 acc = 0;
+#pragma unroll
+            for (int k = 0; k < RS_WAVES; k++) {
+                u32 c = cnt[k][d];
+                cnt[k][d] = acc;
+                acc += c;
+            }
+            run[j] = acc;
+            mine += acc;
+        }
+        u32 total;
+        u32 start = block_excl_add<RS_BLOCK>(mine, scan_lds, total);
+        u32 gbase = 0;
+        if (RAW) {
+            u32 rt = 0;
+#pragma unroll
+            for (int j = 0; j < DPT; j++) rt += row_total[j];
+            u32 all;
+            gbase = block_excl_add<RS_BLOCK>(rt, scan_lds, all);
+        }
+#pragma unroll
+        for (int j = 0; j < DPT; j++) {
+            const u32 d = DPT * threadIdx.x + j;
+            dstart[d] = start;
+            if (RAW) {
+                gdelta[d] = gbase + row_before[j] + out_base - start;
+                gbase += row_total[j];
+            } else {
+                gdelta[d] = offs[(u64)d * tiles + tile] + out_base - start;
+            }
+            start += run[j];
+        }
+    }
+    __syncthreads();
+#pragma unroll
+    for (int r = 0; r < RS_ROUNDS; r++) {
+        const u32 d = rs_digit<K, BITS>(key[r], shift);
+        local[r] += dstart[d] + cnt[w][d];
+    }
+#pragma unroll
+    for (int r = 0; r < RS_ROUNDS; r++) {
+        const u64 i = wbase + (u64)r * WAVE;
+        if (i < n) {
+            skey[local[r]] = key[r];
+            sval[local[r]] = val[r];
+        }
+    }
+    __syncthreads();
+    const u64 left = n - tile_base;
+    const u32 count = left < (u64)RS_TILE ? (u32)left : (u32)RS_TILE;
+#pragma unroll
+    for (int q = 0; q < RS_ROUNDS; q++) {
+        const u32 j = (u32)q * RS_BLOCK + threadIdx.x;
+        if (j < count) {
+            const K k = skey[j];
+            const u32 pos = gdelta[rs_digit<K, BITS>(k, shift)] + j;
+            if (WKEYS) kout[pos] = k;
+            vout[pos] = sval[j];
+        }
+    }
diff --git a/bzip3_amd/csrc/stages.hpp b/bzip3_amd/csrc/stages.hpp
--- a/bzip3_amd/csrc/stages.hpp
+++ b/bzip3_amd/csrc/stages.hpp
@@ -80,6 +80,15 @@
 
 constexpr u32 UNBWT_LANES_PER_CU = 2048;
 void bwt_inverse(const u8 * d_in, u32 n, u32 idx, u8 * d_out, Arena & tmp, hipStream_t s, u32 lanes = 0);
+constexpr u32 UB_MAX_BATCH = 4;
+struct UbBatchItem {
+    const u8 * in;
+    u8 * out;
+    u32 n, idx;
+};
+void bwt_inverse_batch(const UbBatchItem * items, u32 count, Arena & tmp, hipStream_t s, u32 lanes = 0);
+u32 unbwt_batch_size(const u32 * n, u32 count, size_t arena_free, u32 lanes);
+size_t unbwt_batch_workspace_bytes(u64 n, u32 b);
 size_t unbwt_workspace_bytes(u64 n);
 int unbwt_log_stride(u32 rows, u32 lanes);
 void unbwt_set_log_stride(int v);
diff --git a/bzip3_amd/csrc/unbwt.hip b/bzip3_amd/csrc/unbwt.hip
--- a/bzip3_amd/csrc/unbwt.hip
+++ b/bzip3_amd/csrc/unbwt.hip
@@ -30,7 +30,28 @@
     return v < bound ? v : bound - 1;
 }
 
-__global__ void __launch_bounds__(UB_BLOCK) k_ub_hist(const u8 * __restrict__ in, u32 n, u32 * __restrict__ hist) {
+struct UbJob {
+    const u8 * in;
+    u8 * out;
+    u32 n, idx, rows;
+    int log_stride;
+    u32 bound, cap;
+    u32 *psi, *sid, *hist, *cum, *d_total, *split_row, *seg_len, *resume;
+    u32 * succ[2];
+    u32 * dist[2];
+    u8 * slab;
+};
+struct UbBatch {
+    u32 count;
+    UbJob job[UB_MAX_BATCH];
+};
+
+__global__ void __launch_bounds__(UB_BLOCK) k_ub_hist(UbBatch b) {
+    const UbJob & J = b.job[blockIdx.y];
+    const u8 * __restrict__ in = J.in;
+    const u32 n = J.n;
+    u32 * __restrict__ hist = J.hist;
+    if ((u64)blockIdx.x * (UB_BLOCK * 64) >= n) return;
     __shared__ u32 bins[256];
     bins[threadIdx.x] = 0;
     __syncthreads();
@@ -53,7 +74,12 @@
     if (bins[threadIdx.x]) atomicAdd(&hist[threadIdx.x], bins[threadIdx.x]);
 }
 
-__global__ void __launch_bounds__(256) k_ub_cum(const u32 * __restrict__ hist, u32 * __restrict__ cum, u32 * __restrict__ psi, u32 idx) {
+__global__ void __launch_bounds__(256) k_ub_cum(UbBatch b) {
+    const UbJob & J = b.job[blockIdx.y];
+    const u32 * __restrict__ hist = J.hist;
+    u32 * __restrict__ cum = J.cum;
+    u32 * __restrict__ psi = J.psi;
+    const u32 idx = J.idx;
     __shared__ u32 lds[256 / WAVE + 1];
     u32 tot;
     u32 pre = block_excl_add<256>(hist[threadIdx.x], lds, tot);
@@ -64,16 +90,18 @@
     }
 }
 
-__global__ void __launch_bounds__(UB_BLOCK) k_ub_flags(u32 rows, u32 idx, int log_stride, u32 * __restrict__ flags) {
+__global__ void __launch_bounds__(UB_BLOCK) k_ub_flags(UbBatch b) {
+    const UbJob & J = b.job[blockIdx.y];
     const u32 r = blockIdx.x * UB_BLOCK + threadIdx.x;
-    if (r < rows) flags[r] = ub_is_splitter(r, idx, log_stride) ? 1u : 0u;
-}
-
-__global__ void __launch_bounds__(UB_BLOCK) k_ub_collect(u32 rows, u32 idx, int log_stride, const u32 * __restrict__ sid, u32 bound, u32 * __restrict__ split_row) {
+    if (r < J.rows) J.sid[r] = ub_is_splitter(r, J.idx, J.log_stride) ? 1u : 0u;
+}
+
+__global__ void __launch_bounds__(UB_BLOCK) k_ub_collect(UbBatch b) {
+    const UbJob & J = b.job[blockIdx.y];
     const u32 r = blockIdx.x * UB_BLOCK + threadIdx.x;
-    if (r < rows && ub_is_splitter(r, idx, log_stride)) {
-        const u32 j = sid[r];
-        if (j < bound) split_row[j] = r;
+    if (r < J.rows && ub_is_splitter(r, J.idx, J.log_stride)) {
+        const u32 j = J.sid[r];
+        if (j < J.bound) J.split_row[j] = r;
     }
 }
 
@@ -87,10 +115,22 @@
     return lo;
 }
 
-__global__ void __launch_bounds__(UB_BLOCK) k_ub_walk(const u32 * __restrict__ psi, const u32 * __restrict__ sid, const u32 * __restrict__ split_row,
-                                                     const u32 * __restrict__ d_total, u32 bound, u32 idx, int log_stride, u32 rows, const u32 * __restrict__ cum,
-                                                     u32 cap, u32 * __restrict__ succ, u32 * __restrict__ dist, u32 * __restrict__ seg_len, u8 * __restrict__ slab,
-                                                     u32 * __restrict__ resume) {
+__global__ void __launch_bounds__(UB_BLOCK) k_ub_walk(UbBatch b) {
+    const UbJob & J = b.job[blockIdx.y];
+    const u32 bound = J.bound;
+    if (blockIdx.x * UB_BLOCK >= bound) return;
+    const u32 * __restrict__ psi = J.psi;
+    const u32 * __restrict__ sid = J.sid;
+    const u32 * __restrict__ split_row = J.split_row;
+    const u32 * __restrict__ d_total = J.d_total;
+    const u32 * __restrict__ cum = J.cum;
+    const u32 idx = J.idx, rows = J.rows, cap = J.cap;
+    const int log_stride = J.log_stride;
+    u32 * __restrict__ succ = J.succ[0];
+    u32 * __restrict__ dist = J.dist[0];
+    u32 * __restrict__ seg_len = J.seg_len;
+    u8 * __restrict__ slab = J.slab;
+    u32 * __restrict__ resume = J.resume;
     __shared__ u32 c[257];
     for (int k = threadIdx.x; k < 257; k += UB_BLOCK) c[k] = cum[k];
     __syncthreads();
@@ -125,19 +165,30 @@
     seg_len[j] = len;
 }
 
-__global__ void __launch_bounds__(UB_BLOCK) k_ub_jump(const u32 * __restrict__ succ_in, const u32 * __restrict__ dist_in, const u32 * __restrict__ d_total, u32 bound,
-                                                     u32 * __restrict__ succ_out, u32 * __restrict__ dist_out) {
+__global__ void __launch_bounds__(UB_BLOCK) k_ub_jump(UbBatch b, int cur) {
+    const UbJob & J = b.job[blockIdx.y];
+    const u32 * __restrict__ succ_in = J.succ[cur];
+    const u32 * __restrict__ dist_in = J.dist[cur];
+    u32 * __restrict__ succ_out = J.succ[cur ^ 1];
+    u32 * __restrict__ dist_out = J.dist[cur ^ 1];
     const u32 j = blockIdx.x * UB_BLOCK + threadIdx.x;
-    if (j >= ub_count(d_total, bound)) return;
+    if (j >= ub_count(J.d_total, J.bound)) return;
     const u32 sj = succ_in[j];
     u64 d = (u64)dist_in[j] + dist_in[sj];
     dist_out[j] = d > 0xFFFFFFFFull ? 0xFFFFFFFFu : (u32)d;
     succ_out[j] = succ_in[sj];
 }
 
-__global__ void __launch_bounds__(UB_BLOCK) k_ub_place(const u8 * __restrict__ slab, const u32 * __restrict__ seg_len, const u32 * __restrict__ dist,
-                                                      const u32 * __restrict__ succ, const u32 * __restrict__ sid, u32 idx, u32 cap,
-                                                      const u32 * __restrict__ d_total, u32 bound, u32 n, u8 * __restrict__ out) {
+__global__ void __launch_bounds__(UB_BLOCK) k_ub_place(UbBatch b, int cur) {
+    const UbJob & J = b.job[blockIdx.y];
+    const u8 * __restrict__ slab = J.slab;
+    const u32 * __restrict__ seg_len = J.seg_len;
+    const u32 * __restrict__ dist = J.dist[cur];
+    const u32 * __restrict__ succ = J.succ[cur];
+    const u32 * __restrict__ sid = J.sid;
+    const u32 * __restrict__ d_total = J.d_total;
+    const u32 idx = J.idx, cap = J.cap, bound = J.bound, n = J.n;
+    u8 * __restrict__ out = J.out;
     const u32 t = blockIdx.x * UB_BLOCK + threadIdx.x;
     const u32 j = t >> 4, part = t & 15u;
     if (j >= ub_count(d_total, bound)) return;
@@ -163,10 +214,20 @@
     }
 }
 
-__global__ void __launch_bounds__(UB_BLOCK) k_ub_walk_long(const u32 * __restrict__ psi, const u32 * __restrict__ resume, const u32 * __restrict__ seg_len,
-                                                          const u32 * __restrict__ dist, const u32 * __restrict__ succ, const u32 * __restrict__ sid, u32 idx,
-                                                          const u32 * __restrict__ cum, u32 cap, const u32 * __restrict__ d_total, u32 bound, u32 n,
-                                                          u8 * __restrict__ out) {
+__global__ void __launch_bounds__(UB_BLOCK) k_ub_walk_long(UbBatch b, int cur) {
+    const UbJob & J = b.job[blockIdx.y];
+    const u32 bound = J.bound;
+    if (blockIdx.x * UB_BLOCK >= bound) return;
+    const u32 * __restrict__ psi = J.psi;
+    const u32 * __restrict__ resume = J.resume;
+    const u32 * __restrict__ seg_len = J.seg_len;
+    const u32 * __restrict__ dist = J.dist[cur];
+    const u32 * __restrict__ succ = J.succ[cur];
+    const u32 * __restrict__ sid = J.sid;
+    const u32 * __restrict__ cum = J.cum;
+    const u32 * __restrict__ d_total = J.d_total;
+    const u32 idx = J.idx, cap = J.cap, n = J.n;
+    u8 * __restrict__ out = J.out;
     __shared__ u32 c[257];
     for (int k = threadIdx.x; k < 257; k += UB_BLOCK) c[k] = cum[k];
     __syncthreads();
@@ -199,8 +260,15 @@
     return lo;
 }
 
-__global__ void __launch_bounds__(UB_BLOCK) k_ub_tail(const u8 * __restrict__ in, const u32 * __restrict__ psi, const u32 * __restrict__ cum,
-                                                     const u32 * __restrict__ dist, const u32 * __restrict__ sid, u32 idx, u32 bound, u32 n, u8 * __restrict__ out) {
+__global__ void __launch_bounds__(UB_BLOCK) k_ub_tail(UbBatch b, int cur) {
+    const UbJob & J = b.job[blockIdx.y];
+    const u8 * __restrict__ in = J.in;
+    const u32 * __restrict__ psi = J.psi;
+    const u32 * __restrict__ cum = J.cum;
+    const u32 * __restrict__ dist = J.dist[cur];
+    const u32 * __restrict__ sid = J.sid;
+    const u32 idx = J.idx, bound = J.bound, n = J.n;
+    u8 * __restrict__ out = J.out;
     const u32 D = dist[ub_sid(sid, idx, bound)];
     const u32 limit = n & ~1u;
     const u32 lastc = in[0];
@@ -265,53 +333,119 @@
     return log_stride;
 }
 
+static size_t ub_job_bytes(u64 n, int log_stride) {
+    const u64 rows = n + 1;
+    const u64 bound = ub_split_bound((u32)rows, log_stride);
+    return rows * 8 + radix_temp_bytes(n) + scan_temp_words(rows) * 4 + bound * 28 + bound * (4u << log_stride) + (1u << 16);
+}
+
+size_t unbwt_batch_workspace_bytes(u64 n, u32 b) {
+    size_t each = unbwt_workspace_bytes(n);
+    const int forced = g_ub_force_log_stride.load();
+    if (forced >= 0 && ub_job_bytes(n, forced) > each) each = ub_job_bytes(n, forced);
+    return each * b;
+}
+
+u32 unbwt_batch_size(const u32 * n, u32 count, size_t arena_free, u32 lanes) {
+    if (count <= 1) return count;
+    if (lanes == 0) lanes = ub_device_lanes();
+    u32 b = 1;
+    u64 largest = n[0];
+    while (b < count && b < UB_MAX_BATCH) {
+        const u64 big = n[b] > largest ? n[b] : largest;
+        if (unbwt_batch_workspace_bytes(big, b + 1) > arena_free || (u64)(b + 1) * ((big + 1) >> UB_MAX_LOG_STRIDE) > lanes) break;
+        largest = big;
+        b++;
+    }
+    return b;
+}
+
+void bwt_inverse_batch(const UbBatchItem * items, u32 count, Arena & tmp, hipStream_t s, u32 lanes) {
+    if (count == 0) return;
+    if (count > UB_MAX_BATCH) throw HipError{hipErrorUnknown, "inverse BWT batch of more blocks than the job table holds", __FILE__, __LINE__};
+    const size_t mk = tmp.mark();
+    if (lanes == 0) lanes = ub_device_lanes();
+    UbBatch b;
+    b.count = count;
+    u32 * hists = tmp.take<u32>((size_t)256 * count);
+    u32 most_n = 0, most_rows = 0, most_bound = 0;
+    RadixIotaJob rj[UB_MAX_BATCH];
+    u32 * sids[UB_MAX_BATCH];
+    u32 * totals[UB_MAX_BATCH];
+    u64 lens[UB_MAX_BATCH];
+    for (u32 k = 0; k < count; k++) {
+        UbJob & J = b.job[k];
+        if (items[k].n < 2) throw HipError{hipErrorUnknown, "inverse BWT batch with a block of fewer than 2 bytes", __FILE__, __LINE__};
+        J.in = items[k].in;
+        J.out = items[k].out;
+        J.n = items[k].n;
+        J.idx = items[k].idx;
+        J.rows = J.n + 1;
+        J.log_stride = unbwt_log_stride(J.rows, lanes);
+        J.bound = ub_split_bound(J.rows, J.log_stride);
+        J.cap = 4u << J.log_stride;
+        J.psi = tmp.take<u32>(J.rows);
+        J.sid = tmp.take<u32>(J.rows);
+        J.hist = hists + (size_t)256 * k;
+        J.cum = tmp.take<u32>(257);
+        J.d_total = tmp.take<u32>(1);
+        most_n = J.n > most_n ? J.n : most_n;
+        most_rows = J.rows > most_rows ? J.rows : most_rows;
+        most_bound = J.bound > most_bound ? J.bound : most_bound;
+        rj[k] = RadixIotaJob{J.in, J.psi, J.n, J.idx};
+        sids[k] = J.sid;
+        totals[k] = J.d_total;
+        lens[k] = J.rows;
+    }
+    HIP_CHECK(hipMemsetAsync(hists, 0, (size_t)256 * 4 * count, s));
+    for (u32 k = 0; k < UB_MAX_BATCH; k++) {
+        UbJob & J = b.job[k];
+        if (k >= count) J = b.job[0];
+        J.split_row = J.seg_len = J.resume = J.succ[0] = J.succ[1] = J.dist[0] = J.dist[1] = nullptr;
+        J.slab = nullptr;
+    }
+    launch(k_ub_hist, dim3((u32)(((u64)most_n + UB_BLOCK * 64 - 1) / (UB_BLOCK * 64)), count), dim3(UB_BLOCK), 0, s, b);
+    launch(k_ub_cum, dim3(1, count), dim3(256), 0, s, b);
+    radix_pass_iota_u8_many(rj, count, 1u, tmp, s);
+
+    const dim3 grows((most_rows + UB_BLOCK - 1) / UB_BLOCK, count);
+    launch(k_ub_flags, grows, dim3(UB_BLOCK), 0, s, b);
+    exclusive_scan_u32_many(sids, lens, totals, count, tmp, s);
+    for (u32 k = 0; k < count; k++) {
+        UbJob & J = b.job[k];
+        J.split_row = tmp.take<u32>(J.bound);
+        J.seg_len = tmp.take<u32>(J.bound);
+        J.resume = tmp.take<u32>(J.bound);
+        J.succ[0] = tmp.take<u32>(J.bound);
+        J.succ[1] = tmp.take<u32>(J.bound);
+        J.dist[0] = tmp.take<u32>(J.bound);
+        J.dist[1] = tmp.take<u32>(J.bound);
+        J.slab = tmp.take<u8>((size_t)J.bound * J.cap + 64);
+    }
+    for (u32 k = count; k < UB_MAX_BATCH; k++) b.job[k] = b.job[0];
+    const dim3 gs((most_bound + UB_BLOCK - 1) / UB_BLOCK, count);
+    launch(k_ub_collect, grows, dim3(UB_BLOCK), 0, s, b);
+    launch(k_ub_walk, gs, dim3(UB_BLOCK), 0, s, b);
+
+    int cur = 0;
+    for (u64 span = 1; span < most_bound; span <<= 1) {
+        launch(k_ub_jump, gs, dim3(UB_BLOCK), 0, s, b, cur);
+        cur ^= 1;
+    }
+    launch(k_ub_place, dim3((u32)(((u64)most_bound * 16 + UB_BLOCK - 1) / UB_BLOCK), count), dim3(UB_BLOCK), 0, s, b, cur);
+    launch(k_ub_walk_long, gs, dim3(UB_BLOCK), 0, s, b, cur);
+    launch(k_ub_tail, dim3(256, count), dim3(UB_BLOCK), 0, s, b, cur);
+    tmp.release(mk);
+}
+
 void bwt_inverse(const u8 * d_in, u32 n, u32 idx, u8 * d_out, Arena & tmp, hipStream_t s, u32 lanes) {
     if (n == 0) return;
     if (n == 1) {
         HIP_CHECK(hipMemcpyAsync(d_out, d_in, 1, hipMemcpyDeviceToDevice, s));
         return;
     }
-    const size_t mk = tmp.mark();
-    const u32 rows = n + 1;
-    u32 * psi = tmp.take<u32>(rows);
-    u32 * sid = tmp.take<u32>(rows);
-    u32 * hist = tmp.take<u32>(256);
-    u32 * cum = tmp.take<u32>(257);
-    u32 * d_total = tmp.take<u32>(1);
-
-    HIP_CHECK(hipMemsetAsync(hist, 0, 256 * 4, s));
-    launch(k_ub_hist, dim3((u32)(((u64)n + UB_BLOCK * 64 - 1) / (UB_BLOCK * 64))), dim3(UB_BLOCK), 0, s, d_in, n, hist);
-    launch(k_ub_cum, dim3(1), dim3(256), 0, s, (const u32 *)hist, cum, psi, idx);
-    radix_pass<u8>(d_in, (u8 *)nullptr, (const u32 *)nullptr, psi, n, 0, idx, 1u, tmp, s);
-
-    const int log_stride = unbwt_log_stride(rows, lanes ? lanes : ub_device_lanes());
-    const u32 bound = ub_split_bound(rows, log_stride);
-    const dim3 grows((rows + UB_BLOCK - 1) / UB_BLOCK);
-    launch(k_ub_flags, grows, dim3(UB_BLOCK), 0, s, rows, idx, log_stride, sid);
-    exclusive_scan_u32(sid, rows, d_total, tmp, s);
-    u32 * split_row = tmp.take<u32>(bound);
-    u32 * seg_len = tmp.take<u32>(bound);
-    u32 * resume = tmp.take<u32>(bound);
-    u32 * succ[2] = {tmp.take<u32>(bound), tmp.take<u32>(bound)};
-    u32 * dist[2] = {tmp.take<u32>(bound), tmp.take<u32>(bound)};
-    const u32 cap = 4u << log_stride;
-    u8 * slab = tmp.take<u8>((size_t)bound * cap + 64);
-    const dim3 gs((bound + UB_BLOCK - 1) / UB_BLOCK);
-    launch(k_ub_collect, grows, dim3(UB_BLOCK), 0, s, rows, idx, log_stride, (const u32 *)sid, bound, split_row);
-    launch(k_ub_walk, gs, dim3(UB_BLOCK), 0, s, (const u32 *)psi, (const u32 *)sid, (const u32 *)split_row, (const u32 *)d_total, bound, idx, log_stride, rows,
-           (const u32 *)cum, cap, succ[0], dist[0], seg_len, slab, resume);
-
-    int cur = 0;
-    for (u64 span = 1; span < bound; span <<= 1) {
-        launch(k_ub_jump, gs, dim3(UB_BLOCK), 0, s, (const u32 *)succ[cur], (const u32 *)dist[cur], (const u32 *)d_total, bound, succ[cur ^ 1], dist[cur ^ 1]);
-        cur ^= 1;
-    }
-    launch(k_ub_place, dim3((u32)(((u64)bound * 16 + UB_BLOCK - 1) / UB_BLOCK)), dim3(UB_BLOCK), 0, s, (const u8 *)slab, (const u32 *)seg_len, (const u32 *)dist[cur],
-           (const u32 *)succ[cur], (const u32 *)sid, idx, cap, (const u32 *)d_total, bound, n, d_out);
-    launch(k_ub_walk_long, gs, dim3(UB_BLOCK), 0, s, (const u32 *)psi, (const u32 *)resume, (const u32 *)seg_len, (const u32 *)dist[cur], (const u32 *)succ[cur],
-           (const u32 *)sid, idx, (const u32 *)cum, cap, (const u32 *)d_total, bound, n, d_out);
-    launch(k_ub_tail, dim3(256), dim3(UB_BLOCK), 0, s, d_in, (const u32 *)psi, (const u32 *)cum, (const u32 *)dist[cur], (const u32 *)sid, idx, bound, n, d_out);
-    tmp.release(mk);
-}
-
-}
+    const UbBatchItem one{d_in, d_out, n, idx};
+    bwt_inverse_batch(&one, 1, tmp, s, lanes);
+}
+
+}
diff --git a/include/bz3_hip.h b/include/bz3_hip.h
--- a/include/bz3_hip.h
+++ b/include/bz3_hip.h
@@ -137,6 +137,7 @@
 BZIP3_API int32_t bz3_hip_debug_cu_masks(int cus, int reserve, uint32_t * side, uint32_t * rest);
 BZIP3_API int32_t bz3_hip_debug_scan_u32(uint32_t * data, uint32_t n, uint32_t * total);
 BZIP3_API int32_t bz3_hip_debug_sort_u32(const uint32_t * keys, uint32_t n, int key_bits, int digit_bits, uint32_t * sorted_keys, uint32_t * sorted_index);
+BZIP3_API int32_t bz3_hip_debug_unbwt_many(const uint8_t * const * in, uint8_t * const * out, const int32_t * n, const int32_t * idx, int32_t count);
 BZIP3_API float bz3_hip_stage_last_ms(void);
 BZIP3_API int32_t bz3_hip_stage_cm_encode(const uint8_t * in, int32_t n, uint8_t * out);
 BZIP3_API void bz3_hip_stage_cm_decode(const uint8_t * in, int32_t in_size, uint8_t * out, int32_t n);
```

Result: faster. 654.4, median of 6 (+1.8%).
